# GrafikXxxxxxxYyyyyyyyyyy/StableDiffusion

Hardware: AMD Instinct MI355X
Metric: denoise-loop latents/s (512px, 50-step DDIM, batch 4) (higher is better)
Workload: dtype f16; 1 GPU; SD1.5 512x512, 50-step DDIM, batch 4/GPU, CFG on (UNet batch 8), UNet + VAE decode HIP kernels; global_batch=4, parallelism=dp1

## Files before the change

### include/sd_engine.h

```cpp
#ifndef SD_ENGINE_H
#define SD_ENGINE_H

#include <stdint.h>

#ifdef __cplusplus
extern "C" {
#endif

#define SD_OK 0
#define SD_ERR_INVALID 1
#define SD_ERR_STATE 2
#define SD_ERR_HIP 3
#define SD_ERR_UNSUPPORTED 4

#define SD_DTYPE_F16 0
#define SD_DTYPE_F32 1

#define SD_MAX_BLOCKS 4

typedef struct sd_unet_config {
    int32_t in_channels;
    int32_t out_channels;
    int32_t num_blocks;
    int32_t block_out_channels[SD_MAX_BLOCKS];
// ... 49 lines not shown
int sd_unet_destroy(sd_unet* u);
int sd_unet_num_weights(const sd_unet* u);
int sd_unet_weight_info(const sd_unet* u, int index, const char** key, int64_t* shape4, int* ndim);
int sd_unet_set_weight(sd_unet* u, const char* diffusers_key, const void* data,
                       const int64_t* shape, int ndim, int dtype);
int sd_unet_finalize(sd_unet* u);
int sd_unet_forward(sd_unet* u, const void* sample, const float* timesteps, const void* ehs,
                    int ehs_len, const void* add_text, const float* add_time_ids, void* out,
                    int B, int H, int W, void* stream);
int sd_unet_use_graph(sd_unet* u, int enable);
int sd_unet_text_kv_cache(sd_unet* u, int enable);
int sd_unet_forward_ex(sd_unet* u, const void* sample, const float* timesteps, const void* ehs, int ehs_len,
                       const void* add_text, const float* add_time_ids, const void* image_embeds, int n_img, void* out,
                       int B, int H, int W, void* stream);
int sd_unet_forward_tc(sd_unet* u, const void* sample, const float* timesteps, const void* ehs, int ehs_len,
                       const void* add_text, const float* add_time_ids, const void* image_embeds, int n_img,
                       const float* timestep_cond, int cond_dim, void* out, int B, int H, int W, void* stream);
int sd_unet_set_ip_adapter(sd_unet* u, sd_ip_adapter* adapter);
int sd_unet_set_ip_adapter_scale(sd_unet* u, float scale);
int sd_unet_set_controlnet(sd_unet* u, sd_controlnet* cn);
int sd_unet_forward_cn(sd_unet* u, const void* sample, const float* timesteps, const void* ehs, int ehs_len,
                       const void* add_text, const float* add_time_ids, const void* image_embeds, int n_img,
                       const void* control_image, int n_ctrl, float cond_scale, void* out, int B, int H, int W,
                       void* stream);
int sd_unet_forward_cfg(sd_unet* u, const void* latents, const float* timesteps, const void* ehs, int ehs_len,
                        const void* add_text, const float* add_time_ids, const void* image_embeds, int n_img,
                        float in_scale, int share, void* out, int B, int H, int W, void* stream);
int sd_unet_cfg_share(const sd_unet_config* cfg);
int sd_unet_set_freeu(sd_unet* u, int enable, float s1, float s2, float b1, float b2);
int sd_unet_memory(const sd_unet* u, int64_t* weight_bytes, int64_t* workspace_bytes);

int sd_ip_adapter_create(const sd_unet* u, int image_embed_dim, int num_tokens, sd_ip_adapter** out);
int sd_ip_adapter_destroy(sd_ip_adapter* a);
int sd_ip_adapter_num_weights(const sd_ip_adapter* a);
int sd_ip_adapter_weight_info(const sd_ip_adapter* a, int index, const char** key, int64_t* shape4, int* ndim);
int sd_ip_adapter_set_weight(sd_ip_adapter* a, const char* key, const void* data, const int64_t* shape, int ndim,
                             int dtype);
int sd_ip_adapter_finalize(sd_ip_adapter* a);

int sd_controlnet_create(const sd_unet* u, const sd_unet_config* cn_cfg, int conditioning_channels, sd_controlnet** out);
int sd_controlnet_destroy(sd_controlnet* cn);
int sd_controlnet_num_weights(const sd_controlnet* cn);
int sd_controlnet_weight_info(const sd_controlnet* cn, int index, const char** key, int64_t* shape4, int* ndim);
int sd_controlnet_set_weight(sd_controlnet* cn, const char* key, const void* data, const int64_t* shape, int ndim,
                             int dtype);
int sd_controlnet_finalize(sd_controlnet* cn);

int sd_vae_create(const sd_vae_config* cfg, sd_vae** out);
int sd_vae_destroy(sd_vae* v);
int sd_vae_num_weights(const sd_vae* v);
int sd_vae_weight_info(const sd_vae* v, int index, const char** key, int64_t* shape4, int* ndim);
int sd_vae_set_weight(sd_vae* v, const char* diffusers_key, const void* data,
                      const int64_t* shape, int ndim, int dtype);
int sd_vae_finalize(sd_vae* v);
int sd_vae_decode(sd_vae* v, const void* z, void* img, int B, int h, int w, void* stream);
int sd_vae_encode(sd_vae* v, const void* img, void* moments, int B, int H, int W, void* stream);
int sd_vae_encode_range_shift(sd_vae* v, int shift);
int sd_vae_memory(const sd_vae* v, int64_t* weight_bytes, int64_t* workspace_bytes);

int sd_clip_create(const sd_clip_config* cfg, sd_clip** out);
int sd_clip_destroy(sd_clip* c);
int sd_clip_num_weights(const sd_clip* c);
int sd_clip_weight_info(const sd_clip* c, int index, const char** key, int64_t* shape4, int* ndim);
int sd_clip_set_weight(sd_clip* c, const char* key, const void* data, const int64_t* shape, int ndim, int dtype);
int sd_clip_finalize(sd_clip* c);
int sd_clip_forward(sd_clip* c, const int32_t* input_ids, const int32_t* eos_index, void* hidden_states,
                    void* last_hidden, void* pooled, void* text_embeds, int B, int T, void* stream);
int sd_clip_final_layer_norm(sd_clip* c, const void* x, void* y, int64_t rows, void* stream);
int sd_clip_memory(const sd_clip* c, int64_t* weight_bytes, int64_t* workspace_bytes);

int sd_cfg_duplicate(const void* latents, void* out2b, int64_t n_per_batch, int B, float in_scale,
                     void* stream);
int sd_cfg_ddim_step(const void* noise_pred_2b, void* latents, int64_t n, float guidance_scale,
                     float c_x, float c_eps, void* stream);

int sd_cfg_linear_step(const void* noise_pred_2b, void* latents, float* hist_f32, int64_t n,
                       float guidance_scale, float c_x, float c_eps, float c_hist, float h_x, float h_eps,
                       void* stream);

int sd_cfg_rescale_linear_step(const void* noise_pred_2b, void* latents, float* hist_f32, int B, int64_t n_per_sample,
                               float guidance_scale, float guidance_rescale, float c_x, float c_eps, float c_hist,
                               float h_x, float h_eps, float* factors_out, void* stream);

int sd_lcm_step(const void* model_out, int rows, void* latents, const void* noise, void* denoised, int64_t n,
                float guidance_scale, float d_x, float d_out, float p_den, float p_noise, void* stream);

#define SD_STEP_MAX_SLOTS 4
#define SD_STEP_MAX_WRITES 2
typedef struct sd_step_plan {
    int32_t n_slots;
    int32_t n_writes;
    int32_t write_slot[SD_STEP_MAX_WRITES];
    double out[3+SD_STEP_MAX_SLOTS];
    double write[SD_STEP_MAX_WRITES][3+SD_STEP_MAX_SLOTS];
} sd_step_plan;
int sd_sched_affine_step(const void* model_out, int rows, void* latents, const void* noise, float* bank,
                         int64_t bank_stride, int64_t n, float guidance_scale, const sd_step_plan* plan, void* stream);

int sd_inpaint_blend(void* latents, const void* image_latents, const void* noise, const void* mask,
                     float a, float b, int B, int C, int H, int W, void* stream);

int sd_images_to_uint8(const void* images_nchw_f16, void* out_nhwc_u8, int B, int C, int H, int W, void* stream);

typedef struct sd_prof_entry {
    char kernel[64];
    double flops;
    double bytes;
    double ms;
    int64_t launches;
} sd_prof_entry;
int sd_prof_enable(int on);
int sd_prof_collect(sd_prof_entry* out, int max_entries, int* n_entries);

int sd_probe_mfma(int iters, float* tflops, void* stream);
int sd_probe_copy(int64_t bytes, int iters, float* gbs, void* stream);
int sd_probe_lds_dma(int64_t region_bytes, int passes, int depth, int shared, float* gbs, void* stream);

int sd_igemm_force(int variant, int splits);
int sd_igemm_plan(const int* geom, const int* flags, int64_t* out, char* name);

int sd_op_conv2d(const void* x_nhwc, const void* w_oihw, const void* bias, const void* rowadd,
                 const void* res_nhwc, void* y_nhwc, int N, int H, int W, int Cin, int Cout,
                 int ksize, int stride, int upsample2x, int geglu, void* stream);
int sd_op_conv2d_ex(const void* x_nhwc, const void* w_oihw, const void* bias, const void* rowadd,
                    const void* res_nhwc, void* y_nhwc, int N, int H, int W, int Cin, int Cout, int ksize,
                    int stride, int upsample2x, int geglu, int64_t ldx, int64_t ldres, int64_t ldy, int pad, int act,
                    float acc_scale, float bias_scale, int gn_groups, int* ran, void* stream);
int sd_op_conv3x3_small_cout(const void* x_nhwc, const void* w_oihw, const void* bias, void* y_nchw, int N, int H,
                             int W, int Cin, int Cout, void* stream);
int sd_op_conv2d_groupnorm(const void* x_nhwc, const void* w_oihw, const void* bias, const void* rowadd,
                           const void* res_nhwc, void* y_conv_nhwc, const void* gamma, const void* beta,
                           void* y_gn_nhwc, int N, int H, int W, int Cin, int Cout, int ksize, int stride,
                           int upsample2x, int groups, float eps, int silu, int* stats_from_epilogue, void* stream);
int sd_op_groupnorm_conv2d(const void* x_nhwc, const void* gamma, const void* beta, int groups, float eps, int silu,
                           const void* w_oihw, const void* bias, const void* rowadd, const void* res_nhwc, void* y_nhwc,
                           int N, int H, int W, int Cin, int Cout, int ksize, int iters, float* ms_per_launch, int* fused,
                           void* stream);
int sd_op_unet_conv_in(const void* x_nchw, const void* w_oihw, const void* bias, void* y_nhwc, float* gn_summaries, int groups,
                       int N, int Cin, int H, int W, int Cout, int iters, float* ms_per_launch, void* stream);
int sd_op_unet_conv_out(const void* x_nhwc, const void* gamma, const void* beta, int groups, float eps, int silu,
                        const void* w_oihw, const void* bias, void* y_nchw, int N, int H, int W, int C, int Cout, int iters,
                        float* ms_per_launch, void* stream);
int sd_op_ffn_geglu(const void* x, const void* ln_gamma, const void* ln_beta, float ln_eps, const void* w1, const void* b1,
                    const void* w2, const void* b2, void* y, int M, int C, int iters, float* ms_per_launch, int* fused,
                    void* stream);
int sd_op_linear_rowstats(const void* x, const void* w0, const void* b0, const void* res, void* y1, float* stat, int M,
                          int K, int C, int* parts, int* part_w, int* producer, void* stream);
int sd_op_ln_linear(const void* y1, const float* stat, int parts, int part_w, const void* gamma, const void* beta, float eps,
                    const void* w1, const void* b1, void* y2, int M, int C, int O, int geglu, int rows_scaled, float row_scale,
                    int* consumer, void* stream);
int sd_op_ln_ffn_geglu(const void* x, const float* stat, int parts, int part_w, const void* ln_gamma, const void* ln_beta,
                       float ln_eps, const void* w1, const void* b1, const void* w2, const void* b2, void* y, int M, int C,
                       int* fused, void* stream);
int sd_bench_conv2d(const void* x_nhwc, const void* w_oihw, void* y_nhwc, int N, int H, int W, int Cin,
                    int Cout, int ksize, int stride, int upsample2x, int geglu, int iters,
                    float* ms_per_launch, void* stream);
int sd_op_groupnorm(const void* x_nhwc, const void* gamma, const void* beta, void* y_nhwc,
                    int N, int HW, int C, int groups, float eps, int silu, void* stream);
int sd_op_groupnorm_concat(const void* x_nhwc, int Ca, int Cb, const void* gamma, const void* beta, void* y_nhwc, int N, int HW,
                           int groups, float eps, int silu, void* stream);
int sd_bench_groupnorm(const void* x_nhwc, const void* gamma, const void* beta, void* y_nhwc,
                       int N, int HW, int C, int groups, float eps, int silu, int iters,
                       float* ms_per_launch, void* stream);
int sd_op_timestep_sinusoid(const float* t, float* out, int count, int dim, int flip_sin_to_cos, float freq_shift,
                            void* stream);
int sd_op_timestep_cond_embedding(const float* t, const float* cond, const void* w_f16, float* out, int B, int dim,
                                  int cond_dim, int flip_sin_to_cos, float freq_shift, void* stream);
int sd_op_small_linear(const float* x, const void* w_f16, const float* bias, float* y, int B, int K, int n_out,
                       int silu_in, int silu_out, void* stream);
int sd_op_freeu(void* cat_nhwc, int N, int H, int W, int C1, int C2, float b, float s, void* stream);
int sd_op_layernorm(const void* x, const void* gamma, const void* beta, void* y, int rows, int C,
                    float eps, void* stream);
int sd_op_attention(const void* q, const void* k, const void* v, void* out, int B, int Tq, int Tk,
                    int heads, int d, int ldq, int ldk, int ldv, int ldo, void* stream);
int sd_op_attention_ex(const void* q, const void* k, const void* v, void* out, int B, int Tq, int Tk,
                       int heads, int d, int ldq, int ldk, int ldv, int ldo, int causal, int prescaled,
                       void* stream);
int sd_attention_plan(int B, int Tq, int Tk, int heads, int d, int causal, int prescaled, int* out5);
int sd_op_ip_cross_attention(const void* q, const void* k, const void* v, const void* k_ip, const void* v_ip, void* out,
                             int B, int Tq, int L, int T_ip, int heads, int d, int ldq, int ldk, int ldv, int ldk_ip,
                             int ldv_ip, int ldo, float ip_scale, int prescaled, int iters, float* ms_per_launch,
                             void* stream);

typedef struct sd_cn_problem {
    const void* x; int64_t ldx;
    const void* w;
    const float* bias;
    void* y; int64_t ldy;
    int M, C;
} sd_cn_problem;
int sd_op_controlnet_residuals(const sd_cn_problem* problems, int count, float scale, int mode, int iters,
                               float* ms_per_launch, void* stream);
int sd_op_controlnet_cond_embed(sd_controlnet* cn, const void* image, int n, int H, int W, void* out, int iters,
                                float* ms_per_launch, void* stream);

#ifdef __cplusplus
}
#endif
#endif
```

### stablediffusion_amd/_lib.py

```python
from __future__ import annotations

import ctypes as C
import os

_HERE = os.path.dirname(os.path.abspath(__file__))
LIB_PATH = os.path.join(_HERE, "libsd_engine.so")

SD_MAX_BLOCKS = 4
SD_STEP_MAX_SLOTS = 4
SD_STEP_MAX_WRITES = 2
SD_DTYPE_F16 = 0
SD_DTYPE_F32 = 1


class SdUNetConfig(C.Structure):
    _fields_ = [
        ("in_channels", C.c_int32),
        ("out_channels", C.c_int32),
        ("num_blocks", C.c_int32),
        ("block_out_channels", C.c_int32 * SD_MAX_BLOCKS),
        ("down_block_has_attn", C.c_int32 * SD_MAX_BLOCKS),
        ("up_block_has_attn", C.c_int32 * SD_MAX_BLOCKS),
        ("num_heads", C.c_int32 * SD_MAX_BLOCKS),
        ("transformer_layers", C.c_int32 * SD_MAX_BLOCKS),
# ... 1 lines not shown
        ("cross_attention_dim", C.c_int32),
        ("use_linear_projection", C.c_int32),
        ("norm_num_groups", C.c_int32),
        ("norm_eps", C.c_float),
        ("flip_sin_to_cos", C.c_int32),
        ("freq_shift", C.c_float),
        ("addition_time_embed_dim", C.c_int32),
        ("projection_class_embeddings_input_dim", C.c_int32),
        ("time_cond_proj_dim", C.c_int32),
    ]


class SdVAEConfig(C.Structure):
    _fields_ = [
        ("in_channels", C.c_int32),
        ("out_channels", C.c_int32),
        ("latent_channels", C.c_int32),
        ("num_blocks", C.c_int32),
        ("block_out_channels", C.c_int32 * SD_MAX_BLOCKS),
        ("layers_per_block", C.c_int32),
        ("norm_num_groups", C.c_int32),
    ]


class SdClipConfig(C.Structure):
    _fields_ = [
        ("vocab_size", C.c_int32),
        ("hidden_size", C.c_int32),
        ("intermediate_size", C.c_int32),
        ("num_layers", C.c_int32),
        ("num_heads", C.c_int32),
        ("max_positions", C.c_int32),
        ("hidden_act", C.c_int32),
        ("projection_dim", C.c_int32),
        ("layer_norm_eps", C.c_float),
    ]


class SdProfEntry(C.Structure):
    _fields_ = [("kernel", C.c_char * 64), ("flops", C.c_double), ("bytes", C.c_double),
                ("ms", C.c_double), ("launches", C.c_int64)]


class SdCnProblem(C.Structure):
    _fields_ = [("x", C.c_void_p), ("ldx", C.c_int64), ("w", C.c_void_p), ("bias", C.c_void_p),
                ("y", C.c_void_p), ("ldy", C.c_int64), ("M", C.c_int), ("C", C.c_int)]


class SdStepPlan(C.Structure):
    _fields_ = [("n_slots", C.c_int32), ("n_writes", C.c_int32), ("write_slot", C.c_int32 * SD_STEP_MAX_WRITES),
                ("out", C.c_double * (3 + SD_STEP_MAX_SLOTS)),
                ("write", C.c_double * (3 + SD_STEP_MAX_SLOTS) * SD_STEP_MAX_WRITES)]


def step_plan(plan) -> SdStepPlan:
    if len(plan.writes) > SD_STEP_MAX_WRITES or plan.n_slots > SD_STEP_MAX_SLOTS:
        raise ValueError(f"an affine step has at most {SD_STEP_MAX_WRITES} writes and {SD_STEP_MAX_SLOTS} slots")
    p = SdStepPlan(n_slots=plan.n_slots, n_writes=len(plan.writes))
    p.out[:] = plan.out
    for j, (slot, row) in enumerate(plan.writes):
        p.write_slot[j] = slot
        p.write[j][:] = row
    return p


_P = C.c_void_p
_I = C.c_int
_I64 = C.c_int64
_F = C.c_float
SIGNATURES = {
    "sd_last_error": (C.c_char_p, []),
    "sd_engine_version": (_I, []),
    "sd_engine_arch": (C.c_char_p, []),
    "sd_unet_create": (_I, [C.POINTER(SdUNetConfig), C.POINTER(_P)]),
    "sd_unet_destroy": (_I, [_P]),
    "sd_unet_num_weights": (_I, [_P]),
    "sd_unet_weight_info": (_I, [_P, _I, C.POINTER(C.c_char_p), C.POINTER(_I64), C.POINTER(_I)]),
    "sd_unet_set_weight": (_I, [_P, C.c_char_p, _P, C.POINTER(_I64), _I, _I]),
    "sd_unet_finalize": (_I, [_P]),
    "sd_unet_forward": (_I, [_P, _P, _P, _P, _I, _P, _P, _P, _I, _I, _I, _P]),
    "sd_unet_use_graph": (_I, [_P, _I]),
    "sd_unet_text_kv_cache": (_I, [_P, _I]),
    "sd_unet_memory": (_I, [_P, C.POINTER(_I64), C.POINTER(_I64)]),
    "sd_unet_forward_ex": (_I, [_P, _P, _P, _P, _I, _P, _P, _P, _I, _P, _I, _I, _I, _P]),
    "sd_unet_forward_tc": (_I, [_P, _P, _P, _P, _I, _P, _P, _P, _I, _P, _I, _P, _I, _I, _I, _P]),
    "sd_unet_forward_cfg": (_I, [_P, _P, _P, _P, _I, _P, _P, _P, _I, _F, _I, _P, _I, _I, _I, _P]),
    "sd_unet_cfg_share": (_I, [C.POINTER(SdUNetConfig)]),
    "sd_unet_set_ip_adapter": (_I, [_P, _P]),
    "sd_unet_set_ip_adapter_scale": (_I, [_P, _F]),
    "sd_unet_set_freeu": (_I, [_P, _I, _F, _F, _F, _F]),
    "sd_ip_adapter_create": (_I, [_P, _I, _I, C.POINTER(_P)]),
    "sd_ip_adapter_destroy": (_I, [_P]),
    "sd_ip_adapter_num_weights": (_I, [_P]),
    "sd_ip_adapter_weight_info": (_I, [_P, _I, C.POINTER(C.c_char_p), C.POINTER(_I64), C.POINTER(_I)]),
    "sd_ip_adapter_set_weight": (_I, [_P, C.c_char_p, _P, C.POINTER(_I64), _I, _I]),
    "sd_ip_adapter_finalize": (_I, [_P]),
    "sd_unet_set_controlnet": (_I, [_P, _P]),
    "sd_unet_forward_cn": (_I, [_P, _P, _P, _P, _I, _P, _P, _P, _I, _P, _I, _F, _P, _I, _I, _I, _P]),
    "sd_controlnet_create": (_I, [_P, C.POINTER(SdUNetConfig), _I, C.POINTER(_P)]),
    "sd_controlnet_destroy": (_I, [_P]),
    "sd_controlnet_num_weights": (_I, [_P]),
    "sd_controlnet_weight_info": (_I, [_P, _I, C.POINTER(C.c_char_p), C.POINTER(_I64), C.POINTER(_I)]),
    "sd_controlnet_set_weight": (_I, [_P, C.c_char_p, _P, C.POINTER(_I64), _I, _I]),
    "sd_controlnet_finalize": (_I, [_P]),
    "sd_vae_create": (_I, [C.POINTER(SdVAEConfig), C.POINTER(_P)]),
    "sd_vae_destroy": (_I, [_P]),
    "sd_vae_num_weights": (_I, [_P]),
    "sd_vae_weight_info": (_I, [_P, _I, C.POINTER(C.c_char_p), C.POINTER(_I64), C.POINTER(_I)]),
    "sd_vae_set_weight": (_I, [_P, C.c_char_p, _P, C.POINTER(_I64), _I, _I]),
    "sd_vae_finalize": (_I, [_P]),
    "sd_vae_decode": (_I, [_P, _P, _P, _I, _I, _I, _P]),
    "sd_vae_encode": (_I, [_P, _P, _P, _I, _I, _I, _P]),
    "sd_vae_encode_range_shift": (_I, [_P, _I]),
    "sd_vae_memory": (_I, [_P, C.POINTER(_I64), C.POINTER(_I64)]),
    "sd_clip_create": (_I, [C.POINTER(SdClipConfig), C.POINTER(_P)]),
    "sd_clip_destroy": (_I, [_P]),
    "sd_clip_num_weights": (_I, [_P]),
    "sd_clip_weight_info": (_I, [_P, _I, C.POINTER(C.c_char_p), C.POINTER(_I64), C.POINTER(_I)]),
    "sd_clip_set_weight": (_I, [_P, C.c_char_p, _P, C.POINTER(_I64), _I, _I]),
    "sd_clip_finalize": (_I, [_P]),
    "sd_clip_forward": (_I, [_P, _P, _P, _P, _P, _P, _P, _I, _I, _P]),
    "sd_clip_final_layer_norm": (_I, [_P, _P, _P, _I64, _P]),
    "sd_clip_memory": (_I, [_P, C.POINTER(_I64), C.POINTER(_I64)]),
    "sd_op_attention_ex": (_I, [_P, _P, _P, _P, _I, _I, _I, _I, _I, _I, _I, _I, _I, _I, _I, _P]),
    "sd_cfg_duplicate": (_I, [_P, _P, _I64, _I, _F, _P]),
    "sd_cfg_ddim_step": (_I, [_P, _P, _I64, _F, _F, _F, _P]),
    "sd_inpaint_blend": (_I, [_P, _P, _P, _P, _F, _F, _I, _I, _I, _I, _P]),
    "sd_images_to_uint8": (_I, [_P, _P, _I, _I, _I, _I, _P]),
    "sd_cfg_linear_step": (_I, [_P, _P, _P, _I64, _F, _F, _F, _F, _F, _F, _P]),
    "sd_cfg_rescale_linear_step": (_I, [_P, _P, _P, _I, _I64, _F, _F, _F, _F, _F, _F, _F, _P, _P]),
    "sd_lcm_step": (_I, [_P, _I, _P, _P, _P, _I64, _F, _F, _F, _F, _F, _P]),
    "sd_sched_affine_step": (_I, [_P, _I, _P, _P, _P, _I64, _I64, _F, C.POINTER(SdStepPlan), _P]),
    "sd_igemm_force": (_I, [_I, _I]),
    "sd_igemm_plan": (_I, [C.POINTER(_I), C.POINTER(_I), C.POINTER(_I64), C.c_char_p]),
    "sd_probe_mfma": (_I, [_I, C.POINTER(_F), _P]),
    "sd_probe_lds_dma": (_I, [_I64, _I, _I, _I, C.POINTER(_F), _P]),
    "sd_probe_copy": (_I, [_I64, _I, C.POINTER(_F), _P]),
    "sd_prof_enable": (_I, [_I]),
    "sd_prof_collect": (_I, [C.POINTER(SdProfEntry), _I, C.POINTER(_I)]),
    "sd_op_conv2d": (_I, [_P, _P, _P, _P, _P, _P, _I, _I, _I, _I, _I, _I, _I, _I, _I, _P]),
    "sd_op_conv2d_ex": (_I, [_P, _P, _P, _P, _P, _P, _I, _I, _I, _I, _I, _I, _I, _I, _I, _I64, _I64, _I64, _I, _I, _F, _F, _I,
                             C.POINTER(_I), _P]),
    "sd_op_conv3x3_small_cout": (_I, [_P, _P, _P, _P, _I, _I, _I, _I, _I, _P]),
    "sd_op_conv2d_groupnorm": (_I, [_P, _P, _P, _P, _P, _P, _P, _P, _P, _I, _I, _I, _I, _I, _I, _I, _I, _I, _F, _I,
                                    C.POINTER(_I), _P]),
    "sd_op_groupnorm_conv2d": (_I, [_P, _P, _P, _I, _F, _I, _P, _P, _P, _P, _P, _I, _I, _I, _I, _I, _I, _I, C.POINTER(_F),
                                    C.POINTER(_I), _P]),
    "sd_op_unet_conv_in": (_I, [_P, _P, _P, _P, _P, _I, _I, _I, _I, _I, _I, _I, C.POINTER(_F), _P]),
    "sd_op_unet_conv_out": (_I, [_P, _P, _P, _I, _F, _I, _P, _P, _P, _I, _I, _I, _I, _I, _I, C.POINTER(_F), _P]),
    "sd_op_ffn_geglu": (_I, [_P, _P, _P, _F, _P, _P, _P, _P, _P, _I, _I, _I, C.POINTER(_F), C.POINTER(_I), _P]),
    "sd_op_linear_rowstats": (_I, [_P, _P, _P, _P, _P, _P, _I, _I, _I, C.POINTER(_I), C.POINTER(_I), C.POINTER(_I), _P]),
    "sd_op_ln_linear": (_I, [_P, _P, _I, _I, _P, _P, _F, _P, _P, _P, _I, _I, _I, _I, _I, _F, C.POINTER(_I), _P]),
    "sd_op_ln_ffn_geglu": (_I, [_P, _P, _I, _I, _P, _P, _F, _P, _P, _P, _P, _P, _I, _I, C.POINTER(_I), _P]),
    "sd_bench_conv2d": (_I, [_P, _P, _P, _I, _I, _I, _I, _I, _I, _I, _I, _I, _I, C.POINTER(_F), _P]),
    "sd_op_groupnorm": (_I, [_P, _P, _P, _P, _I, _I, _I, _I, _F, _I, _P]),
    "sd_op_groupnorm_concat": (_I, [_P, _I, _I, _P, _P, _P, _I, _I, _I, _F, _I, _P]),
    "sd_bench_groupnorm": (_I, [_P, _P, _P, _P, _I, _I, _I, _I, _F, _I, _I, C.POINTER(_F), _P]),
    "sd_op_timestep_sinusoid": (_I, [_P, _P, _I, _I, _I, _F, _P]),
    "sd_op_timestep_cond_embedding": (_I, [_P, _P, _P, _P, _I, _I, _I, _I, _F, _P]),
    "sd_op_small_linear": (_I, [_P, _P, _P, _P, _I, _I, _I, _I, _I, _P]),
    "sd_op_freeu": (_I, [_P, _I, _I, _I, _I, _I, _F, _F, _P]),
    "sd_op_layernorm": (_I, [_P, _P, _P, _P, _I, _I, _F, _P]),
    "sd_op_attention": (_I, [_P, _P, _P, _P, _I, _I, _I, _I, _I, _I, _I, _I, _I, _P]),
    "sd_attention_plan": (_I, [_I, _I, _I, _I, _I, _I, _I, C.POINTER(_I)]),
    "sd_op_ip_cross_attention": (_I, [_P, _P, _P, _P, _P, _P, _I, _I, _I, _I, _I, _I, _I, _I, _I, _I, _I, _I, _F, _I, _I,
                                      C.POINTER(_F), _P]),
    "sd_op_controlnet_residuals": (_I, [C.POINTER(SdCnProblem), _I, _F, _I, _I, C.POINTER(_F), _P]),
    "sd_op_controlnet_cond_embed": (_I, [_P, _P, _I, _I, _I, _P, _I, C.POINTER(_F), _P]),
}

_lib = None


class EngineError(RuntimeError):
    pass


def load():
    global _lib
    if _lib is not None:
        return _lib
    if not os.path.exists(LIB_PATH):
        raise EngineError(
            f"{LIB_PATH} not found: build it with `python -m stablediffusion_amd.build` "
            "(hipcc --offload-arch=gfx950). The HIP engine is mandatory; there is no CPU fallback.")
    import torch
    lib = C.CDLL(LIB_PATH)
    for name, (res, args) in SIGNATURES.items():
        fn = getattr(lib, name)
        fn.restype = res
        fn.argtypes = args
    _lib = lib
    return lib


def check(rc: int, what: str = ""):
    if rc != 0:
        msg = load().sd_last_error()
        raise EngineError(f"{what}: error {rc}: {msg.decode() if msg else '?'}")


def require_gpu():
    import torch
    if not torch.cuda.is_available():
        raise EngineError("no HIP device visible: the gfx950 engine cannot run (and nothing else will run in its place)")
```

### stablediffusion_amd/csrc/capi.cpp

```cpp
#include <cmath>
#include <cstdio>
#include <new>

#include "model.h"
#include <cstdlib>

using namespace sd;

struct sd_unet { UNet impl; explicit sd_unet(const sd_unet_config& c) : impl(c) {} };
struct sd_vae { VAE impl; explicit sd_vae(const sd_vae_config& c) : impl(c) {} };
struct sd_clip { CLIP impl; explicit sd_clip(const sd_clip_config& c) : impl(c) {} };
struct sd_controlnet {
    ControlNet impl;
    sd_controlnet(const sd_unet_config& c, int cc) : impl(c, cc) {}
};
struct sd_ip_adapter {
    IPAdapter impl;
    sd_ip_adapter(const sd_unet_config& c, int d, int n) : impl(c, d, n) {}
    ~sd_ip_adapter() { if (impl.attached) impl.attached->set_ip_adapter(nullptr); }
};

namespace {

int weight_info(const WeightStore& ws, int index, const char** key, int64_t* shape4, int* ndim) {
// ... 1227 lines not shown
    auto fused = [&]() {
        return launch_ip_attention(qh, kh, vh, kih, vih, oh, B, Tq, L, T_ip, heads, d, ldq, ldk, ldv, ldk_ip, ldv_ip, ldo,
                                   ip_scale, prescaled, s);
    };
    int rc = fused();
    if (rc || iters <= 0) return rc;
    if (!ms_per_launch) { set_error("sd_op_ip_cross_attention: ms_per_launch required with iters > 0"); return SD_ERR_INVALID; }
    if (!attention_supported(d)) { set_error("sd_op_ip_cross_attention: timing needs a head dim of the text kernel"); return SD_ERR_UNSUPPORTED; }
    half_t* tmp = nullptr;
    SD_HIP_CHECK(hipMalloc(reinterpret_cast<void**>(&tmp), (size_t)B * Tq * heads * d * sizeof(half_t)));
    const long ldt = (long)heads * d;
    auto text = [&]() {
        return launch_attention(qh, kh, vh, oh, B, Tq, L, heads, d, ldq, ldk, ldv, ldo, s, 0, prescaled);
    };
    auto unfused = [&]() {
        int r = text();
        if (!r) r = launch_attention(qh, kih, vih, tmp, B, Tq, T_ip, heads, d, ldq, ldk_ip, ldv_ip, ldt, s, 0, prescaled);
        if (!r) r = launch_axpy_f16(oh, ldo, tmp, ldt, (long)B * Tq, heads * d, ip_scale, s);
        return r;
    };
    hipEvent_t e0 = nullptr, e1 = nullptr;
    if (hipEventCreate(&e0) != hipSuccess || hipEventCreate(&e1) != hipSuccess) rc = SD_ERR_HIP;
    for (int variant = 0; variant < 3 && !rc; ++variant) {
        auto one = [&]() { return variant == 0 ? fused() : variant == 1 ? text() : unfused(); };
        for (int it = 0; it < 2 && !rc; ++it) rc = one();
        if (rc) break;
        (void)hipEventRecord(e0, s);
        for (int it = 0; it < iters && !rc; ++it) rc = one();
        (void)hipEventRecord(e1, s);
        float ms = 0.f;
        hipError_t e = hipEventSynchronize(e1);
        if (e == hipSuccess) e = hipEventElapsedTime(&ms, e0, e1);
        if (e != hipSuccess) { set_error(hipGetErrorString(e)); rc = SD_ERR_HIP; }
        ms_per_launch[variant] = ms / (float)iters;
    }
    if (!rc) rc = fused();
    if (!rc && hipStreamSynchronize(s) != hipSuccess) rc = SD_ERR_HIP;
    if (e0) (void)hipEventDestroy(e0);
    if (e1) (void)hipEventDestroy(e1);
    (void)hipFree(tmp);
    return rc;
}

}

namespace {
template <class F>
int run_op_on_arena(hipStream_t s, int iters, float* ms, F body) {
    Arena arena;
    Ctx dry{&arena, s, true};
    arena.begin(true);
    body(dry);
    if (dry.err) return dry.err;
    if (int rc = arena.reserve(arena.peak() > 0 ? arena.peak() : 256)) return rc;
    auto live = [&]() {
        Ctx c{&arena, s, false};
        arena.begin(false);
        body(c);
        return c.err;
    };
    int rc = live();
    if (!rc && iters > 0) {
        if (!ms) { set_error("ms_per_launch required with iters > 0"); return SD_ERR_INVALID; }
        hipEvent_t e0 = nullptr, e1 = nullptr;
        if (hipEventCreate(&e0) != hipSuccess || hipEventCreate(&e1) != hipSuccess) rc = SD_ERR_HIP;
        if (!rc) rc = live();
        if (!rc) (void)hipEventRecord(e0, s);
        for (int it = 0; it < iters && !rc; ++it) rc = live();
        if (!rc) {
            (void)hipEventRecord(e1, s);
            float t = 0.f;
            hipError_t e = hipEventSynchronize(e1);
            if (e == hipSuccess) e = hipEventElapsedTime(&t, e0, e1);
            if (e != hipSuccess) { set_error(hipGetErrorString(e)); rc = SD_ERR_HIP; }
            *ms = t / (float)iters;
        }
        if (e0) (void)hipEventDestroy(e0);
        if (e1) (void)hipEventDestroy(e1);
    }
    const hipError_t e = hipStreamSynchronize(s);
    if (!rc && e != hipSuccess) { set_error(hipGetErrorString(e)); rc = SD_ERR_HIP; }
    return rc;
}
}

extern "C" {

int sd_op_controlnet_residuals(const sd_cn_problem* problems, int count, float scale, int mode, int iters,
                               float* ms_per_launch, void* stream) {
    if (!problems || count < 1 || count > kCnMaxProblems) { set_error("sd_op_controlnet_residuals: 1..16 problems"); return SD_ERR_INVALID; }
    if (mode != 0 && mode != 1) { set_error("sd_op_controlnet_residuals: mode must be 0 (grouped) or 1 (unfused)"); return SD_ERR_INVALID; }
    hipStream_t s = static_cast<hipStream_t>(stream);
    CnResParams rp;
    rp.scale = scale;
    for (int i = 0; i < count; ++i) {
        const sd_cn_problem& q = problems[i];
        CnResProblem& d = rp.p[rp.count++];
        d.x = static_cast<const half_t*>(q.x); d.ldx = q.ldx; d.w = static_cast<const half_t*>(q.w); d.bias = q.bias;
        d.y = static_cast<half_t*>(q.y); d.ldy = q.ldy; d.M = q.M; d.C = q.C; d.first = rp.total;
        if (q.C <= 0 || q.C % 64 != 0 || q.M <= 0) { set_error("sd_op_controlnet_residuals: C % 64 == 0 and M >= 1 required"); return SD_ERR_UNSUPPORTED; }
        rp.total += cn_residual_tiles(q.M, q.C);
    }
    if (!cn_residual_supported(rp)) { set_error("sd_op_controlnet_residuals: unsupported strides or alignment"); return SD_ERR_UNSUPPORTED; }
    if (mode == 0) return run_op_on_arena(s, iters, ms_per_launch, [&](Ctx& c) { if (!c.dry) c.err = launch_cn_residual(rp, s); });
    std::vector<ConvW> ws((size_t)count);
    std::vector<void*> owned;
    int rc = 0;
    for (int i = 0; i < count && !rc; ++i) {
        const sd_cn_problem& q = problems[i];
        const long rows = ((long)q.C + kWeightRowPad - 1) / kWeightRowPad * kWeightRowPad;
        void *w = nullptr, *b = nullptr;
        if (hipMalloc(&w, (size_t)rows * q.C * sizeof(half_t)) != hipSuccess || hipMalloc(&b, (size_t)rows * sizeof(float)) != hipSuccess) {
            set_error("sd_op_controlnet_residuals: out of device memory"); rc = SD_ERR_HIP;
        }
        if (w) owned.push_back(w);
        if (b) owned.push_back(b);
        if (rc) break;
        if (hipMemsetAsync(w, 0, (size_t)rows * q.C * sizeof(half_t), s) != hipSuccess ||
            hipMemsetAsync(b, 0, (size_t)rows * sizeof(float), s) != hipSuccess ||
            hipMemcpyAsync(w, q.w, (size_t)q.C * q.C * sizeof(half_t), hipMemcpyDeviceToDevice, s) != hipSuccess ||
            hipMemcpyAsync(b, q.bias, (size_t)q.C * sizeof(float), hipMemcpyDeviceToDevice, s) != hipSuccess) {
            set_error("sd_op_controlnet_residuals: copy failed"); rc = SD_ERR_HIP;
        }
        ConvW& cw = ws[(size_t)i];
        cw.w = static_cast<half_t*>(w); cw.bias = static_cast<float*>(b); cw.cin = q.C; cw.cout = q.C; cw.ks = 1; cw.K = q.C;
    }
    if (!rc && scale != 0.f)
        rc = run_op_on_arena(s, iters, ms_per_launch, [&](Ctx& c) {
            for (int i = 0; i < count; ++i) {
                const sd_cn_problem& q = problems[i];
                View y(static_cast<half_t*>(q.y), q.ldy, q.C);
                ConvFuse f;
                f.acc_scale = scale; f.bias_scale = scale;
                op_conv(c, ws[(size_t)i], View(const_cast<half_t*>(static_cast<const half_t*>(q.x)), q.ldx, q.C), 1, q.M, 1,
                        y, 1, 0, nullptr, 0, &y, 0, -1, 0, &f);
            }
        });
    (void)hipStreamSynchronize(s);
    for (void* p : owned) (void)hipFree(p);
    return rc;
}

int sd_op_controlnet_cond_embed(sd_controlnet* cn, const void* image, int n, int H, int W, void* out, int iters,
                                float* ms_per_launch, void* stream) {
    if (!cn || !image || !out) { set_error("null argument"); return SD_ERR_INVALID; }
    if (!cn->impl.finalized) { set_error("sd_op_controlnet_cond_embed: ControlNet not finalized"); return SD_ERR_STATE; }
    if (n < 1 || H < 1 || W < 1) { set_error("sd_op_controlnet_cond_embed: bad shape"); return SD_ERR_INVALID; }
    const int C0 = cn->impl.cfg.block_out_channels[0];
    return run_op_on_arena(static_cast<hipStream_t>(stream), iters, ms_per_launch, [&](Ctx& c) {
        cn->impl.run_cond_embed(c, static_cast<const half_t*>(image), n, H, W, View(static_cast<half_t*>(out), C0, C0));
    });
}

}
```

### stablediffusion_amd/csrc/engine.h

```cpp
#pragma once
#include <map>
#include <string>
#include <unordered_map>
#include <vector>

#include "kernels.h"

namespace sd {

struct View {
    half_t* p = nullptr;
    long ld = 0;
    int C = 0;
    View() {}
    View(half_t* p_, long ld_, int C_) : p(p_), ld(ld_), C(C_) {}
    View slice(int c0, int c) const { return View(p + c0, ld, c); }
};

class Arena {
  public:
    ~Arena();
    int reserve(size_t bytes);
    void begin(bool dry) { dry_ = dry; off_ = 0; if (dry) peak_ = 0; }
    void* alloc(size_t bytes);
    half_t* alloc_h(long n) { return static_cast<half_t*>(alloc((size_t)n * sizeof(half_t))); }
    float* alloc_f(long n) { return static_cast<float*>(alloc((size_t)n * sizeof(float))); }
    size_t mark() const { return off_; }
    void release(size_t m) { off_ = m; }
    size_t peak() const { return peak_; }
    size_t capacity() const { return cap_; }
    bool dry() const { return dry_; }
    bool overflow() const { return overflow_; }

  private:
    char* base_ = nullptr;
    size_t cap_ = 0, off_ = 0, peak_ = 0;
    bool dry_ = false, overflow_ = false;
};

struct ConvW {
    half_t* w = nullptr;
    float* bias = nullptr;
    int cin = 0, cout = 0, ks = 1;
    long K = 0;
    float* wsum = nullptr;
};
struct RowStat {
    float* p = nullptr;
    int parts = 0;
    int width = 0;
};
struct GnStatBuf {
    float* buf = nullptr;
    GnStats st;
};
struct ConvFuse {
    const RowStat* ln_in = nullptr;
    float ln_eps = 0.f;
    RowStat* stat_out = nullptr;
    GnStatBuf* gn_out = nullptr;
    int gn_groups = 0;
    const struct NormW* gn_in = nullptr;
    GnStats gn_in_stats;
    int gn_in_groups = 0;
    float gn_in_eps = 0.f;
    int gn_in_silu = 0;
    float acc_scale = 1.f, bias_scale = 1.f;
};
struct NormW {
    float* gamma = nullptr;
    float* beta = nullptr;
    float* gb = nullptr;
    int C = 0;
};

struct RawTensor {
    std::vector<int64_t> shape;
    half_t* dev = nullptr;
    long numel = 0;
};

class WeightStore {
  public:
    ~WeightStore();
    void declare(const std::string& key, std::vector<int64_t> shape);
    int set(const std::string& key, const void* data, const int64_t* shape, int ndim, int dtype);
    bool complete(std::string* missing) const;
    const RawTensor* raw(const std::string& key) const;
    int pack_conv(const std::string& prefix, ConvW* out, bool has_bias = true);
    int pack_rows(const std::vector<std::string>& weight_keys, const std::vector<std::string>& bias_keys,
                  ConvW* out);
    int pack_geglu(const std::string& prefix, ConvW* out);
    int pack_norm(const std::string& prefix, NormW* out);
    int fold_ln(ConvW* w, const NormW& ln, int rows_scaled, float row_scale);
    void free_raw();
    void* dmalloc(size_t bytes);
    int64_t packed_bytes() const { return packed_bytes_; }

    std::vector<std::string> order;
    std::unordered_map<std::string, RawTensor> tensors;

  private:
    int host_floats(const std::string& key, std::vector<float>* out) const;
    std::vector<void*> owned_;
    int64_t packed_bytes_ = 0;
};

struct Ctx {
    Arena* arena;
    hipStream_t stream;
    bool dry;
    int err = 0;
    static constexpr int kGnPool = 4;
    GnStatBuf gnpool[kGnPool];
    int gn_next = 0;
    int gn_groups = 0;
    View ip_kv;
    int ip_T = 0;
    float ip_scale = 1.f;
};
void ctx_gnpool_init(Ctx& c, int N, long HW_max, int G);
GnStatBuf* ctx_gnbuf(Ctx& c);

struct ProfAgg { double flops = 0, bytes = 0, ms = 0; long launches = 0; };
void prof_enable(bool on);
bool prof_enabled();
void prof_open(hipStream_t s, const char* kernel, double flops, double bytes);
void prof_close(hipStream_t s);
int prof_collect(std::map<std::string, ProfAgg>* out);

void op_conv(Ctx& c, const ConvW& w, View x, int N, int H, int W, View y, int stride = 1, int up = 0,
             const float* rowadd = nullptr, int rowadd_ld = 0, const View* res = nullptr, int geglu = 0,
             int pad = -1, int act = 0, const ConvFuse* fuse = nullptr);
inline long rowstat_floats(long M, int C) { return M * ((C + 63) / 64) * 2; }
inline long gnstat_floats(int N, long HW, int G) { const long t = (HW + 63) / 64; return (long)N * (t > 64 ? t : 64) * G * 2; }
void op_groupnorm(Ctx& c, const NormW& n, View x, View y, int N, long HW, int G, float eps, int silu,
                  const GnStatBuf* pre = nullptr);
void op_gn_conv(Ctx& c, const NormW& n, const ConvW& w, View x, int N, int H, int W, View y, int G, float eps, int silu,
                const GnStatBuf* pre, const float* rowadd = nullptr, int rowadd_ld = 0, const View* res = nullptr,
                const ConvFuse* fuse = nullptr);
void op_layernorm(Ctx& c, const NormW& n, View x, View y, long rows, float eps);
bool op_ffn_fused(Ctx& c, const ConvW& ff1, const ConvW& ff2, View x, const RowStat& x_stat, float ln_eps, long M, View y);
void op_attention(Ctx& c, View q, View k, View v, View out, int B, int Tq, int Tk, int heads, int d, int causal = 0,
                  int prescaled = 0);
void op_ip_attention(Ctx& c, View q, View k, View v, View k_ip, View v_ip, View out, int B, int Tq, int L, int T_ip,
                     int heads, int d, float ip_scale);

}
```

### stablediffusion_amd/csrc/ffn.hip

```cpp
#include <cstdlib>

#include "kernels.h"

namespace sd {
namespace {

constexpr int FF_C = 320, FF_BM = 128, FF_NKS = FF_C / 64, FF_NOS = 2, FF_STAGES = 7;
constexpr int kFfMaxLnParts = 20;

template <int N>
__device__ __forceinline__ void ff_wait_vmcnt() {
    asm volatile("s_waitcnt vmcnt(%0)" ::"n"(N) : "memory");
}

struct FfLds {
    static constexpr int STAGE = 160 * 64 * 2;
    static constexpr int RING = FF_STAGES * STAGE;
    static constexpr int H = FF_BM * 64 * 2;
    static constexpr int AUX = 2 * 256 * 4;
    static constexpr int STAT = FF_BM * 2 * 4;
    static constexpr int TOTAL = RING + H + AUX + STAT;
};

__global__ __launch_bounds__(512) void ffn_fused_kernel(FfnParams p) {
// ... 38 lines not shown
    __amdgpu_buffer_rsrc_t rw2 = __builtin_amdgcn_make_buffer_rsrc(const_cast<half_t*>(p.w2), 0, (int)((long)p.w2_rows * p.hidden * 2), 0x00020000);
    __amdgpu_buffer_rsrc_t raux = __builtin_amdgcn_make_buffer_rsrc(const_cast<float*>(wave == 0 ? p.b1 : p.wsum1), 0, p.w1_rows * 4, 0x00020000);
    const int lrow = lane >> 3;
    const int chunk = (lane & 7) ^ (lrow & 7);
    auto gperm = [](int r) { return r < 32 || r >= 96 ? r : (r < 64 ? r + 32 : r - 32); };
    unsigned w1_off[2], w2_off[3];
#pragma unroll
    for (int j = 0; j < 2; ++j) {
        const int r = (wave * 2 + j) * 8 + lrow;
        w1_off[j] = (unsigned)((((long)gperm(r)) * C + chunk * 8) * 2);
    }
#pragma unroll
    for (int j = 0; j < 3; ++j) {
        const int r = (wave + NW * j) * 8 + lrow;
        const int oc = 160 * (r / 80) + (r % 80);
        w2_off[j] = (unsigned)((((long)oc) * p.hidden + chunk * 8) * 2);
    }

    int s_it = 0, s_q = 0, s_slot = 0;
    auto issue = [&]() {
        half_t* dst = ring + s_slot * STAGE_HALVES;
        const bool live = s_it < NSTEP;
        if (s_q < NKS) {
            if (s_q == 0 && wave < 2 && live && lane < 32)
                __builtin_amdgcn_raw_ptr_buffer_load_lds(raux, (__attribute__((address_space(3))) void*)(sAux + (s_it & 1) * 256 + wave * 128),
                                                         16, (unsigned)((s_it * 128 + lane * 4) * 4), 0, 0, 0);
#pragma unroll
            for (int j = 0; j < 2; ++j)
                __builtin_amdgcn_raw_ptr_buffer_load_lds(rw1, (__attribute__((address_space(3))) void*)(dst + (wave * 2 + j) * 512), 16,
                                                         live ? w1_off[j] + (unsigned)((s_it * 128 * C + s_q * 64) * 2) : kOOB, 0, 0, 0);
        } else {
            const unsigned sb = (unsigned)((((long)(s_q - NKS) * 80) * p.hidden + s_it * 64) * 2);
#pragma unroll
            for (int j = 0; j < 3; ++j)
                if (wave + NW * j < 20)
                    __builtin_amdgcn_raw_ptr_buffer_load_lds(rw2, (__attribute__((address_space(3))) void*)(dst + (wave + NW * j) * 512), 16,
                                                             live ? w2_off[j] + sb : kOOB, 0, 0, 0);
        }
        if (++s_q == NKS + NOS) { s_q = 0; ++s_it; }
        if (++s_slot == STAGES) s_slot = 0;
    };
#pragma unroll
    for (int s = 0; s < LA; ++s) issue();

    f4 acc1[TM][4], acc2[NOS][TM][5];
#pragma unroll
    for (int i = 0; i < TM; ++i) {
#pragma unroll
        for (int j = 0; j < 4; ++j) acc1[i][j] = f4{0.f, 0.f, 0.f, 0.f};
#pragma unroll
        for (int s = 0; s < NOS; ++s)
#pragma unroll
            for (int j = 0; j < 5; ++j) acc2[s][i][j] = f4{0.f, 0.f, 0.f, 0.f};
    }

    int lb[2];
#pragma unroll
    for (int ks = 0; ks < 2; ++ks) lb[ks] = fr * 64 + (((ks * 4 + fq) ^ (fr & 7)) << 3);
    const int rowH = wm * 32 * 64, rowB1 = wn * 64 * 64, rowB2 = wn * 80 * 64;
    int c_slot = 0;
    auto slab_begin = [&]() -> const half_t* {
        ff_wait_vmcnt<2 * (LA - 1)>();
        asm volatile("s_waitcnt lgkmcnt(0)" ::: "memory");
        __builtin_amdgcn_s_barrier();
        issue();
        const half_t* cB = ring + c_slot * STAGE_HALVES;
        if (++c_slot == STAGES) c_slot = 0;
        return cB;
    };

    for (int it = 0; it < NSTEP; ++it) {
        {
#pragma unroll
            for (int q = 0; q < NKS; ++q) {
                const half_t* cB = slab_begin();
#pragma unroll
                for (int ks = 0; ks < 2; ++ks) {
                    h8 fb[4];
#pragma unroll
                    for (int j = 0; j < 4; ++j) fb[j] = *reinterpret_cast<const h8*>(cB + rowB1 + j * 1024 + lb[ks]);
#pragma unroll
                    for (int i = 0; i < TM; ++i)
#pragma unroll
                        for (int j = 0; j < 4; ++j)
                            acc1[i][j] = __builtin_amdgcn_mfma_f32_16x16x32_f16(fb[j], xf[i][q * 2 + ks], acc1[i][j], 0, 0, 0);
                }
            }
            const float* ax = sAux + (it & 1) * 256 + wn * 32 + fq * 4;
#pragma unroll
            for (int jh = 0; jh < 2; ++jh) {
                const f4 bh = *reinterpret_cast<const f4*>(ax + jh * 16), bg = *reinterpret_cast<const f4*>(ax + 64 + jh * 16);
                const f4 wh = *reinterpret_cast<const f4*>(ax + 128 + jh * 16), wg = *reinterpret_cast<const f4*>(ax + 192 + jh * 16);
#pragma unroll
                for (int i = 0; i < TM; ++i) {
                    const float2 mr = *reinterpret_cast<const float2*>(sStat + (wm * 32 + i * 16 + fr) * 2);
                    const f4 hv = (acc1[i][jh] - mr.x * wh) * mr.y + bh;
                    const f4 gv = (acc1[i][jh + 2] - mr.x * wg) * mr.y + bg;
                    h4 o;
#pragma unroll
                    for (int e = 0; e < 4; ++e) o[e] = (half_t)(hv[e] * gelu_erf_f(gv[e]));
                    const int pr = wm * 32 + i * 16 + fr;
                    const int k = wn * 32 + jh * 16 + fq * 4;
                    *reinterpret_cast<h4*>(sH + pr * 64 + (((k >> 3) ^ (pr & 7)) << 3) + (k & 7)) = o;
                    acc1[i][jh] = f4{0.f, 0.f, 0.f, 0.f};
                    acc1[i][jh + 2] = f4{0.f, 0.f, 0.f, 0.f};
                }
            }
        }
        {
#pragma unroll
            for (int s = 0; s < NOS; ++s) {
                const half_t* cB = slab_begin();
#pragma unroll
                for (int ks = 0; ks < 2; ++ks) {
                    h8 fa[TM], fb[5];
#pragma unroll
                    for (int i = 0; i < TM; ++i) fa[i] = *reinterpret_cast<const h8*>(sH + rowH + i * 1024 + lb[ks]);
#pragma unroll
                    for (int j = 0; j < 5; ++j) fb[j] = *reinterpret_cast<const h8*>(cB + rowB2 + j * 1024 + lb[ks]);
#pragma unroll
                    for (int i = 0; i < TM; ++i)
#pragma unroll
                        for (int j = 0; j < 5; ++j)
                            acc2[s][i][j] = __builtin_amdgcn_mfma_f32_16x16x32_f16(fb[j], fa[i], acc2[s][i][j], 0, 0, 0);
                }
            }
        }
    }
    ff_wait_vmcnt<0>();

#pragma unroll
    for (int s = 0; s < NOS; ++s) {
#pragma unroll
        for (int j = 0; j < 5; ++j) {
            const int col = 160 * wn + 80 * s + j * 16 + fq * 4;
            const f4 b2 = *reinterpret_cast<const f4*>(p.b2 + col);
#pragma unroll
            for (int i = 0; i < TM; ++i) {
                const long m = m0 + wm * 32 + i * 16 + fr;
                const f4 v = acc2[s][i][j] + b2;
                const h4 xr = *reinterpret_cast<const h4*>(p.x + m * p.ldx + col);
                h4 o;
#pragma unroll
                for (int e = 0; e < 4; ++e) o[e] = (half_t)((float)(half_t)v[e] + (float)xr[e]);
                *reinterpret_cast<h4*>(p.y + m * p.ldy + col) = o;
            }
        }
    }
#endif
}

}

bool ffn_fused_supported(const FfnParams& p) {
    static const bool off = getenv("SD_NO_FFN_FUSE") != nullptr;
    return !off && p.C == FF_C && p.hidden == 4 * FF_C && p.M % FF_BM == 0 && p.M / FF_BM >= 64 && p.ln_stat && p.ln_parts >= 1 &&
           p.ln_parts <= kFfMaxLnParts && p.w1_rows >= 2 * p.hidden && p.w2_rows >= FF_C &&
           (long)p.M * p.ldx * 2 < (1L << 31) && p.b1 && p.b2 && p.wsum1;
}

int launch_ffn_fused(const FfnParams& p, hipStream_t s) {
    if (!ffn_fused_supported(p)) { set_error("ffn_fused: unsupported problem"); return 1; }
    static_assert(FfLds::TOTAL <= 160 * 1024, "LDS budget");
    static PerDeviceOnce attr_once;
    if (attr_once.first()) {
        SD_HIP_CHECK(hipFuncSetAttribute(reinterpret_cast<const void*>(&ffn_fused_kernel),
                                         hipFuncAttributeMaxDynamicSharedMemorySize, FfLds::TOTAL));
    }
    hipLaunchKernelGGL(ffn_fused_kernel, dim3(p.M / FF_BM), dim3(512), FfLds::TOTAL, s, p);
    SD_HIP_CHECK(hipGetLastError());
    return 0;
}

}
```

### stablediffusion_amd/csrc/igemm2.hip

```cpp
#include <atomic>
#include <cstdlib>
#include <mutex>

#include "kernels.h"

namespace sd {
namespace {

constexpr int BK = 64;
constexpr int kMaxLnParts = 20;
template <int N>
__device__ __forceinline__ void wait_vmcnt() {
    static_assert(N >= 0 && N <= 63, "vmcnt is a 6-bit field");
    asm volatile("s_waitcnt vmcnt(%0)" ::"n"(N) : "memory");
}
template <int PER, int YMAX>
__device__ __forceinline__ void wait_stages(int y) {
    if constexpr (YMAX == 0) {
        wait_vmcnt<0>();
    } else {
        if (y >= YMAX) wait_vmcnt<PER * YMAX>();
        else wait_stages<PER, YMAX - 1>(y);
    }
}
// ... 924 lines not shown
    }
    if constexpr (GN) {
        if (p.gnstat_out) {
            float* sG = reinterpret_cast<float*>(smem + ((BM * LDC * 2 + 15) & ~15));
            gn_part_finish(gsplit, gnv, gp0, gp1, gm0, gq0, gm1, gq1);
            gn_tile_stats<BM, BN, NT>(sG, tid, gm0, gq0, gm1, gq1, n0, p.Cout, cpg, p.gn_groups,
                                      p.gnstat_out + ((long)img * patches + pidx) * p.gn_groups * 2);
        }
    }
#endif
}

bool halo_supported(const IGemmParams& p) {
    return p.KS == 3 && p.stride == 1 && (p.up == 0 || p.up == 1) && p.pad == 1 && !p.geglu && !p.act && p.Cin % 64 == 0 &&
           p.Cout % 8 == 0 && halo_patch_width(p.OH, p.OW) > 0 && p.OH == p.H << p.up && p.OW == p.W << p.up &&
           p.K == 9 * p.Cin;
}

template <int BN, bool GNF, bool KHU>
int launch_halo_t(const IGemmParams& p, float* partial, int splits, hipStream_t s) {
    const int Wt = halo_patch_width(p.OH, p.OW), R = 256 / Wt;
    size_t lds = (size_t)2 * (R + 2) * (Wt + 2) * 128 + (size_t)3 * BN * 128 + (GNF ? 768 : 0);
    const size_t epi = (size_t)256 * (BN + 8) * 2 + 16 + 512 * 16;
    if (lds < epi) lds = epi;
    if (lds > 160 * 1024) { set_error("conv3x3_halo_kernel: LDS budget"); return 1; }
    static size_t attr_by_dev[64] = {};
    static std::mutex attr_mu;
    int dev = 0;
    (void)hipGetDevice(&dev);
    std::lock_guard<std::mutex> attr_lock(attr_mu);
    size_t& attr = attr_by_dev[dev & 63];
    if (lds > attr) {
        SD_HIP_CHECK(hipFuncSetAttribute(reinterpret_cast<const void*>(&conv3x3_halo_kernel<BN, GNF, KHU>),
                                         hipFuncAttributeMaxDynamicSharedMemorySize, (int)lds));
        attr = lds;
    }
    const int tiles = (p.M / 256) * cdiv(p.Cout, BN);
    const int nslab = p.Cin / 64;
    const int per = cdiv(nslab, splits);
    const int eff_splits = cdiv(nslab, per);
    note_splits(eff_splits);
    IGemmParams q = p;
    q.mfast = weights_outweigh_activations(p);
    if (eff_splits > 1) q.gnstat_out = nullptr;
    hipLaunchKernelGGL((conv3x3_halo_kernel<BN, GNF, KHU>), dim3(tiles, eff_splits), dim3(512), lds, s, q, eff_splits > 1 ? partial : nullptr,
                       per);
    SD_HIP_CHECK(hipGetLastError());
    if (eff_splits > 1) return launch_splitk_epilogue(p, partial, eff_splits, s);
    return 0;
}

template <int BN>
int launch_halo(const IGemmParams& p, float* partial, int splits, hipStream_t s) {
    if (p.gni_part) {
        if (p.gni_groups < 1 || p.gni_groups > 32 || 512 % p.gni_groups != 0 || p.Cin % p.gni_groups != 0 || !p.gni_gb) {
            set_error("conv3x3_halo_kernel: fused GroupNorm needs 1..32 groups dividing 512 and the packed affine");
            return 1;
        }
        return launch_halo_t<BN, true, false>(p, partial, splits, s);
    }
    if constexpr (BN == 160) {
        if (p.gnstat_out && splits <= 1) return launch_halo_t<BN, false, false>(p, partial, splits, s);
    }
    return launch_halo_t<BN, false, true>(p, partial, splits, s);
}

template <int BM, int BN, int WM, int WN, int STAGES, bool PW, bool STAG, int BKT>
int launch_v2p(const IGemmParams& p, float* partial, int splits, hipStream_t s) {
    constexpr size_t lds = IGemm2Lds<BM, BN, STAGES, BKT>::TOTAL;
    static_assert(lds <= 160 * 1024, "LDS budget");
    static PerDeviceOnce attr_once;
    if (attr_once.first()) {
        SD_HIP_CHECK(hipFuncSetAttribute(reinterpret_cast<const void*>(&igemm2_kernel<BM, BN, WM, WN, STAGES, PW, STAG, BKT>),
                                         hipFuncAttributeMaxDynamicSharedMemorySize, (int)lds));
    }
    const int tiles = cdiv(p.M, BM) * cdiv(p.Cout, BN);
    const int nk = p.K / BKT;
    const int per = cdiv(nk, splits);
    const int eff_splits = cdiv(nk, per);
    note_splits(eff_splits);
    IGemmParams q = p;
    q.mfast = weights_outweigh_activations(p);
    q.rowstat_parts = cdiv(p.Cout, BN);
    if (p.geglu && !(BN == 128 && WN == 2)) { set_error("igemm2: GEGLU needs a 128-column tile over two wave columns"); return 1; }
    if (eff_splits > 1 && (p.rowstat_out || p.ln_stat)) { set_error("igemm2: row statistics / LayerNorm fold need splits == 1"); return 1; }
    hipLaunchKernelGGL((igemm2_kernel<BM, BN, WM, WN, STAGES, PW, STAG, BKT>), dim3(tiles, eff_splits), dim3(64 * WM * WN), lds, s,
                       q, eff_splits > 1 ? partial : nullptr, per);
    SD_HIP_CHECK(hipGetLastError());
    if (eff_splits > 1) return launch_splitk_epilogue(p, partial, eff_splits, s);
    return 0;
}

template <int BM, int BN, int WM, int WN, int STAGES, bool STAG = false, int BKT = 64>
int launch_v2(const IGemmParams& p, float* partial, int splits, hipStream_t s) {
    if (p.KS == 1 && p.stride == 1 && p.up == 0)
        return launch_v2p<BM, BN, WM, WN, STAGES, true, STAG, BKT>(p, partial, splits, s);
    return launch_v2p<BM, BN, WM, WN, STAGES, false, STAG, BKT>(p, partial, splits, s);
}

std::atomic<int> g_force_variant{-1};
std::atomic<int> g_force_splits{0};

enum class Family { Tile, Halo, Ws, Reg };
struct Variant {
    int id, bm, bn;
    Family family;
    bool geglu;
    bool reg_alt;
    const char* name;
    int (*launch)(const IGemmParams&, float* partial, int splits, hipStream_t);
};
int launch_ws(const IGemmParams& p, float*, int, hipStream_t s) { return launch_wsgemm(p, s); }
int launch_reg(const IGemmParams& p, float*, int, hipStream_t s) { return launch_igemm3(p, weights_outweigh_activations(p), s); }
const Variant kVariants[] = {
    {0, 256, 128, Family::Tile, true, false, "igemm2_kernel<256,128,4,2,3,%s,false,64>", &launch_v2<256, 128, 4, 2, 3>},
    {1, 128, 128, Family::Tile, true, false, "igemm2_kernel<128,128,2,2,2,%s,false,64>", &launch_v2<128, 128, 2, 2, 2>},
    {2, 128, 160, Family::Tile, false, false, "igemm2_kernel<128,160,2,2,2,%s,false,64>", &launch_v2<128, 160, 2, 2, 2>},
    {3, 128, 64, Family::Tile, false, false, "igemm2_kernel<128,64,2,2,2,%s,false,64>", &launch_v2<128, 64, 2, 2, 2>},
    {4, 64, 64, Family::Tile, false, false, "igemm2_kernel<64,64,2,2,2,%s,false,64>", &launch_v2<64, 64, 2, 2, 2>},
    {5, 256, 160, Family::Tile, false, false, "igemm2_kernel<256,160,4,1,3,%s,false,64>", &launch_v2<256, 160, 4, 1, 3>},
    {6, 256, 128, Family::Tile, true, false, "igemm2_kernel<256,128,4,2,3,%s,true,64>", &launch_v2<256, 128, 4, 2, 3, true>},
    {7, 256, 160, Family::Tile, false, false, "igemm2_kernel<256,160,4,2,3,%s,true,64>", &launch_v2<256, 160, 4, 2, 3, true>},
    {8, 128, 64, Family::Tile, false, false, "igemm2_kernel<128,64,2,2,3,%s,false,64>", &launch_v2<128, 64, 2, 2, 3>},
    {9, 128, 160, Family::Tile, false, false, "igemm2_kernel<128,160,2,2,3,%s,false,64>", &launch_v2<128, 160, 2, 2, 3>},
    {10, 256, 160, Family::Halo, false, false, "conv3x3_halo_kernel<160>", &launch_halo<160>},
    {11, 128, 80, Family::Tile, false, true, "igemm2_kernel<128,80,4,1,2,%s,false,64>", &launch_v2<128, 80, 4, 1, 2>},
    {12, 128, 80, Family::Tile, false, true, "igemm2_kernel<128,80,4,1,3,%s,false,64>", &launch_v2<128, 80, 4, 1, 3>},
    {13, 128, 160, Family::Ws, true, false, "wsgemm_kernel<160,false,...>", &launch_ws},
    {14, 128, 128, Family::Ws, true, false, "wsgemm_kernel<128,true,...>", &launch_ws},
    {15, 256, 128, Family::Halo, false, false, "conv3x3_halo_kernel<128>", &launch_halo<128>},
    {16, 128, 80, Family::Tile, false, false, "igemm2_kernel<128,80,4,1,4,%s,false,64>", &launch_v2<128, 80, 4, 1, 4>},
    {17, 128, 80, Family::Tile, false, false, "igemm2_kernel<128,80,4,1,5,%s,false,64>", &launch_v2<128, 80, 4, 1, 5>},
    {18, 128, 80, Family::Reg, false, false, "igemm3_kernel", &launch_reg},
};
constexpr int kNumVariants = sizeof(kVariants) / sizeof(kVariants[0]);
enum : int {
    kT256x128 = 0, kT128x128 = 1, kT128x160 = 2, kT128x64 = 3, kT64x64 = 4,
    kHalo160 = 10, kHalo128 = 15,
    kWsPlain = 13, kWsGeglu = 14,
    kHaloFallback = 7,
    kGegluFallback = kT128x128,
    kWsFallbackGeglu = kT128x128, kWsFallbackPlain = kT128x160,
    kReg = 18, kRegFallback = 12,
};
bool valid_id(int v) { return v >= 0 && v < kNumVariants && kVariants[v].id == v; }
bool is_halo(int v) { return kVariants[v].family == Family::Halo; }
bool is_ws(int v) { return kVariants[v].family == Family::Ws; }

struct TunedEntry { int M, N, K, ks, stride, up, geglu, variant, splits; float us; int alt_variant; float alt_us; };
const TunedEntry kTuned[] = {
#include "igemm2_table.inc"
};

void pick_tile(const IGemmParams& p, int* variant, int* splits) {
    if (g_force_variant.load() >= 0) {
        int v = g_force_variant.load();
        *splits = g_force_splits.load() > 0 ? g_force_splits.load() : 1;
        if (p.geglu && !(valid_id(v) && kVariants[v].geglu)) v = kGegluFallback;
        if (p.geglu || p.act) *splits = 1;
        if (valid_id(v) && is_halo(v) && !halo_supported(p)) v = kHaloFallback;
        *variant = v;
        return;
    }
    for (const TunedEntry& e : kTuned)
        if (!p.act && e.M == p.M && e.N == p.Cout && e.K == p.K && e.ks == p.KS && e.stride == p.stride && e.up == p.up &&
            e.geglu == p.geglu) {
            *variant = is_halo(e.variant) && !halo_supported(p) ? kHaloFallback : e.variant;
            *splits = e.splits;
            return;
        }
    auto tiles_of = [&](int v) { return (long)cdiv(p.M, kVariants[v].bm) * cdiv(p.Cout, kVariants[v].bn); };
    const int narrow = tiles_of(kT128x64) >= 256 ? kT128x64 : kT64x64;
    *splits = 1;
    if (p.act) {
        *variant = tiles_of(kT128x128) >= 256 ? kT128x128 : narrow;
        return;
    }
    const int nk = p.K / BK;
    int v;
    if (p.geglu) v = tiles_of(kT256x128) >= 512 ? kT256x128 : kT128x128;
    else v = p.Cout % 160 == 0 ? kT128x160 : kT128x128;
    if (!p.geglu && tiles_of(v) < 256 && nk <= 40) v = narrow;
    const long tiles = tiles_of(v);
    if (!p.geglu && tiles < 384 && nk >= 24) {
        int sp = (int)((512 + tiles / 2) / tiles);
        if (sp > 8) sp = 8;
        while (sp > 1 && nk / sp < 12) --sp;
        *splits = sp;
    }
    *variant = v;
}

}

void igemm2_force(int variant, int splits) { g_force_variant = variant; g_force_splits = splits; }

bool igemm2_supported(const IGemmParams& p) {
    const long x_bytes = (long)p.N * p.H * p.W * p.ldx * 2;
    const long wrows = ((long)p.Cout + kWeightRowPad - 1) / kWeightRowPad * kWeightRowPad;
    return p.K % BK == 0 && p.Cin % BK == 0 && (p.Cout % 8) == 0 && x_bytes < (1L << 31) &&
           wrows * p.K * 2 < (1L << 31) && (!p.geglu || p.Cout % 128 == 0) && !(p.geglu && p.act);
}

bool igemm2_gn_fusable(const IGemmParams& p, int groups) {
    return igemm2_supported(p) && halo_supported(p) && p.up == 0 && groups >= 1 && groups <= 32 && 512 % groups == 0 &&
           p.Cin % groups == 0;
}

IGemmPlan igemm2_plan(IGemmParams& p, const IGemmRequest& rq) {
    IGemmPlan pl;
    pl.rs_part_w = p.Cout;
    if (!igemm2_supported(p)) {
        snprintf(pl.name, sizeof(pl.name), "%s", igemm_variant(p));
        return pl;
    }
    static const bool ws_on = getenv("SD_NO_WSGEMM") == nullptr;
    static const bool pg_k320 = getenv("SD_PGEMM_K320") != nullptr;
    static const bool g3_auto = getenv("SD_IGEMM3") != nullptr;
    const bool forced = g_force_variant.load() >= 0;
    int v0, sp0;
    pick_tile(p, &v0, &sp0);
    if (!valid_id(v0)) { set_error("igemm2: bad variant"); pl.kind = kKindBadVariant; return pl; }
    int v, sp;
    auto route = [&]() {
        v = v0; sp = sp0;
        if (p.gni_part && !is_halo(v)) {
            v = p.Cout % 160 == 0 ? kHalo160 : kHalo128;
            const long tiles = (long)(p.M / kVariants[v].bm) * cdiv(p.Cout, kVariants[v].bn);
            const int nslab = p.Cin / 64;
            sp = 1;
            while (tiles * sp < 192 && nslab / (sp + 1) >= 4 && sp < 8) ++sp;
        }
        if (p.ln_stat) sp = 1;
        const bool ws_ok = wsgemm_supported(p);
        if (is_ws(v) && !ws_ok) { v = p.geglu ? kWsFallbackGeglu : kWsFallbackPlain; sp = 1; }
        if (!forced && ws_ok && !p.res && ws_on) { v = kWsPlain; sp = 1; }
        if (is_ws(v)) v = p.geglu ? kWsGeglu : kWsPlain;
        if (rq.no_workspace) sp = 1;
    };
    route();
    pl.scales_ok = !p.geglu && !is_ws(v);
    const int G = rq.gn_groups, cpg = G > 0 && p.Cout % G == 0 ? p.Cout / G : 0;
    if (rq.gnstat && !p.geglu && (cpg >= 8 || cpg == 4)) {
        p.gnstat_out = rq.gnstat; p.gn_groups = G;
        route();
        const Variant& t = kVariants[is_halo(v) && !halo_supported(p) ? kHaloFallback : v];
        if (is_ws(v)) pl.gn_rows = 0;
        else if (sp > 1) pl.gn_rows = splitk_gs_rows(p, G);
        else pl.gn_rows = (p.OH * p.OW) % t.bm == 0 && (t.bn % cpg == 0 || p.Cout <= t.bn) ? t.bm : 0;
        pl.gnstats = pl.gn_rows > 0;
        if (!pl.gnstats) { p.gnstat_out = nullptr; p.gn_groups = 0; }
    }
    if (rq.rowstat && !p.geglu) {
        p.rowstat_out = rq.rowstat;
        route();
        const int parts = is_ws(v) ? wsgemm_rowstat_parts(p) : cdiv(p.Cout, kVariants[v].bn);
        pl.rowstats = sp <= 1 && !is_halo(v) && parts <= kMaxLnParts;
        if (pl.rowstats) { pl.rs_parts = parts; pl.rs_part_w = is_ws(v) ? p.Cout / parts : kVariants[v].bn; }
        else p.rowstat_out = nullptr;
    }
    route();
    pl.variant = v;
    pl.splits = sp;
    pl.partial_floats = sp > 1 ? (long)sp * p.M * p.Cout : 0;
    if (p.geglu && (!is_ws(v) || pg_k320) && !forced && pgemm_geglu_supported(p)) pl.kind = kKindPgemmGeglu;
    else if ((v == kReg || (kVariants[v].reg_alt && g3_auto && !forced)) && sp <= 1 && igemm3_supported(p)) pl.kind = kReg;
    else pl.kind = v == kReg ? kRegFallback : v;
    const Variant& t = kVariants[pl.kind == kKindPgemmGeglu ? v : pl.kind];
    pl.bm = t.bm; pl.bn = t.bn;
    if (pl.kind == kKindPgemmGeglu) snprintf(pl.name, sizeof(pl.name), "geglu_persist_kernel");
    else snprintf(pl.name, sizeof(pl.name), t.name, p.KS == 1 && p.stride == 1 && p.up == 0 ? "true" : "false");
    return pl;
}

IGemmLaunchNote igemm2_last_launch() { return t_note; }

int launch_igemm2(const IGemmParams& p, float* partial, hipStream_t s, const IGemmPlan* plan) {
    t_note = IGemmLaunchNote();
    IGemmParams q = p;
    IGemmPlan own;
    if (!plan || (plan->splits > 1 && !partial)) {
        q.rowstat_out = nullptr; q.gnstat_out = nullptr;
        own = igemm2_plan(q, IGemmRequest{p.rowstat_out, p.gnstat_out, p.gn_groups, partial == nullptr});
        plan = &own;
    }
    if (plan->kind == kKindIgemm1) return launch_igemm(q, s);
    if (plan->kind == kKindPgemmGeglu) return launch_pgemm_geglu(q, s);
    if (plan->kind == kKindBadVariant) { set_error("igemm2: bad variant"); return 1; }
    return kVariants[plan->kind].launch(q, partial, plan->splits, s);
}

}
```

### stablediffusion_amd/csrc/kernels.h

```cpp
#pragma once
#include "common.h"

namespace sd {

struct IGemmParams {
    const half_t* x; long ldx;
    const half_t* w;
    const float* bias;
    const float* rowadd; int rowadd_ld;
    const half_t* res; long ldres;
    half_t* y; long ldy;
    int N, H, W, Cin;
    int OH, OW, Cout;
    int KS, stride, pad, up;
    int M, K;
    int geglu;
    int mfast = 0;
    int act = 0;
    float* rowstat_out = nullptr;
    int rowstat_parts = 0;
    const float* ln_stat = nullptr;
    int ln_parts = 0, ln_C = 0, ln_part_w = 0;
    float ln_eps = 0.f;
    const float* ln_wsum = nullptr;
    float* gnstat_out = nullptr;
    int gn_groups = 0;
    const float* gni_part = nullptr;
    int gni_S = 0;
    long gni_rows = 0;
    int gni_groups = 0;
    float gni_eps = 0.f;
    int gni_silu = 0;
    const float* gni_gb = nullptr;
    int dbg_unchecked = 0;
    float acc_scale = 1.f, bias_scale = 1.f;
};
bool igemm2_gn_fusable(const IGemmParams& p, int groups);
int launch_igemm(const IGemmParams& p, hipStream_t s);
const char* igemm_variant(const IGemmParams& p);
bool igemm2_supported(const IGemmParams& p);
void igemm2_force(int variant, int splits);
struct IGemmRequest {
    float* rowstat = nullptr;
    float* gnstat = nullptr;
    int gn_groups = 0;
    bool no_workspace = false;
};
constexpr int kKindPgemmGeglu = 100;
constexpr int kKindIgemm1 = -1;
constexpr int kKindBadVariant = -2;
struct IGemmPlan {
    int kind = kKindIgemm1;
    int variant = -1;
    int splits = 1;
    long partial_floats = 0;
    int bm = 0, bn = 0;
    bool rowstats = false;
    int rs_parts = 1, rs_part_w = 0;
    bool gnstats = false;
    int gn_rows = 0;
    bool scales_ok = false;
    char name[64] = "";
};
IGemmPlan igemm2_plan(IGemmParams& p, const IGemmRequest& rq = IGemmRequest());
int launch_igemm2(const IGemmParams& p, float* partial, hipStream_t s, const IGemmPlan* plan = nullptr);
struct IGemmLaunchNote {
    int splits = 1;
    int reducer = 0;
};
IGemmLaunchNote igemm2_last_launch();
bool igemm3_supported(const IGemmParams& p);
int launch_igemm3(const IGemmParams& p, int mfast, hipStream_t s);
constexpr int kWeightRowPad = 256;
bool wsgemm_supported(const IGemmParams& p);
int wsgemm_rowstat_parts(const IGemmParams& p);
int launch_wsgemm(const IGemmParams& p, hipStream_t s);
bool pgemm_geglu_supported(const IGemmParams& p);
int launch_pgemm_geglu(const IGemmParams& p, hipStream_t s);

struct FfnParams {
    const half_t* x; long ldx;
    half_t* y; long ldy;
    const half_t* w1; const float* b1; const float* wsum1; int w1_rows;
    const half_t* w2; const float* b2; int w2_rows;
    const float* ln_stat; int ln_parts; float ln_eps;
    int M, C, hidden;
    int ln_part_w;
};
bool ffn_fused_supported(const FfnParams& p);
int launch_ffn_fused(const FfnParams& p, hipStream_t s);

long gn_scratch_floats(int N, long HW, int C, int G);
struct GnStats {
    const float* part = nullptr;
    int S = 0;
    long rows = 0;
};
bool gn_wants_stats(long HW, int C, int G);
int launch_groupnorm(const half_t* x, long ldx, const float* gamma, const float* beta,
                     half_t* y, long ldy, int N, long HW, int C, int G, float eps, int silu,
                     float* scratch, hipStream_t s, const GnStats* pre = nullptr);
int launch_gn_stats(const half_t* x, long ldx, int N, long HW, int C, int G, float* scratch, GnStats* st, hipStream_t s);
int launch_gn_finalize(GnStats* st, float* out, int N, long HW, int C, int G, hipStream_t s);
int gn_cat_unit(int Ca, int Cb, int G);
int launch_gn_cat_finalize(const GnStats& sa, int Ga, int Ca, const GnStats& sb, int Gb, int Cb, float* out, int N, long HW, int G,
                           hipStream_t s);
int launch_layernorm(const half_t* x, long ldx, const float* gamma, const float* beta,
                     half_t* y, long ldy, long rows, int C, float eps, hipStream_t s);
int launch_row_stats(const half_t* x, long ldx, float* stat, long rows, int C, hipStream_t s);
int launch_ln_fold(half_t* w, long K, int rows, const float* gamma, const float* beta, const float* bias_in,
                   float* bias, float* wsum, int rows_scaled, float row_scale, hipStream_t s);

int launch_attention(const half_t* q, const half_t* k, const half_t* v, half_t* out,
                     int B, int Tq, int Tk, int heads, int d,
                     long ldq, long ldk, long ldv, long ldo, hipStream_t s, int causal = 0, int prescaled = 0);
bool attention_supported(int d);
struct AttnPlan { int D, QT, KT, PRESC, NWV; };
AttnPlan attention_plan(int B, int Tq, int Tk, int heads, int d, int causal, int prescaled);
int launch_ip_attention(const half_t* q, const half_t* k, const half_t* v, const half_t* kip, const half_t* vip,
                        half_t* out, int B, int Tq, int L, int Tip, int heads, int d, long ldq, long ldk, long ldv,
                        long ldki, long ldvi, long ldo, float ip_scale, int prescaled, hipStream_t s);
bool ip_attention_supported(int d);
int launch_axpy_f16(half_t* y, long ldy, const half_t* x, long ldx, long rows, int cols, float a, hipStream_t s);

constexpr int kCnMaxProblems = 16;
struct CnResProblem {
    const half_t* x = nullptr; long ldx = 0;
    const half_t* w = nullptr;
    const float* bias = nullptr;
    half_t* y = nullptr; long ldy = 0;
    int M = 0, C = 0;
    int first = 0;
};
struct CnResParams {
    CnResProblem p[kCnMaxProblems];
    int count = 0, total = 0;
    float scale = 1.f;
};
int cn_residual_tiles(int M, int C);
bool cn_residual_supported(const CnResParams& p);
int launch_cn_residual(const CnResParams& p, hipStream_t s);
struct CnCondConvParams {
    const half_t* x = nullptr; int nchw = 0;
    const float* w = nullptr; const float* bias = nullptr;
    half_t* y = nullptr;
    int N = 0, IH = 0, IW = 0, Cin = 0, OH = 0, OW = 0, Cout = 0, stride = 1, silu = 1;
};
bool cn_cond_conv_supported(const CnCondConvParams& p);
int launch_cn_cond_conv(const CnCondConvParams& p, hipStream_t s);
int launch_cn_pack_cond(const half_t* w_oihw, float* out, int O, int I, hipStream_t s);

int launch_freeu(half_t* x, long ld, int N, int H, int W, int C1, int C2, float b, float s, hipStream_t st);

int launch_timestep_sinusoid(const float* t, int t_stride, float* out, int count, int dim, int flip, float shift,
                             long out_ld, hipStream_t s);
int launch_timestep_cond(const float* t, const float* cond, const half_t* w, long ldw, float* out, int count, int dim,
                         int cond_dim, int flip, float shift, hipStream_t s);
int launch_small_linear(const float* x, long ldx, const half_t* w, const float* bias, float* y,
                        long ldy, int B, int K, int Nout, int silu_in, int silu_out, hipStream_t s);
int launch_add_f32(float* y, const float* x, long n, int silu, hipStream_t s);
int launch_f16_to_f32(const half_t* x, float* y, long n, hipStream_t s);
int launch_f32_to_f16(const float* x, half_t* y, long n, hipStream_t s);
int launch_im2col_nchw3x3(const half_t* x, half_t* col, int N, int C, int H, int W, int Kpad,
                          hipStream_t s);
int launch_nhwc_to_nchw(const half_t* x, long ldx, half_t* y, int N, long HW, int C, hipStream_t s);
int launch_nchw_to_nhwc(const half_t* x, half_t* y, long ldy, int N, long HW, int C, hipStream_t s);
int launch_pointwise_nchw(const half_t* x, const half_t* w, const float* bias, half_t* y, int N,
                          int Cin, int Cout, long HW, hipStream_t s);
constexpr long kSmallCoutMinPixels = 131072;
int launch_conv3x3_small_cout(const half_t* x, long ldx, const half_t* w, long K, const float* bias, half_t* y_nchw,
                              int N, int H, int W, int Cin, int Cout, hipStream_t s);
struct HeadParams {
    const half_t* x_nchw = nullptr;
    const half_t* w = nullptr; long K = 0;
    const float* bias = nullptr;
    half_t* y = nullptr; long ldy = 0;
    float* gnstat_out = nullptr; int G = 0;
    int N = 0, Cin = 0, H = 0, W = 0, Cout = 0;
};
bool conv_head_supported(const HeadParams& p);
int launch_conv_head(const HeadParams& p, hipStream_t s);
struct TailParams {
    const half_t* x = nullptr; long ldx = 0;
    const float* gn_part = nullptr; int gn_S = 0; long gn_rows = 0;
    int G = 0; float eps = 0.f; const float* gamma = nullptr; const float* beta = nullptr; int silu = 0;
    const half_t* w = nullptr; long K = 0; const float* bias = nullptr;
    half_t* y = nullptr;
    int N = 0, H = 0, W = 0, C = 0, Cout = 0;
};
bool conv_tail_supported(const TailParams& p);
int launch_conv_tail(const TailParams& p, hipStream_t s);
int launch_pack_conv(const half_t* w_oihw, half_t* wp, int O, int I, int KH, int KW, long Kpad,
                     hipStream_t s);
int launch_cfg_duplicate(const half_t* lat, half_t* out, long n_total, float scale, hipStream_t s);
constexpr int kRowDupMax = 8;
struct RowDupSeg {
    const void* src = nullptr;
    void* dst = nullptr;
    long ld_bytes = 0, row_bytes = 0, rows = 0;
};
int launch_row_dup(const RowDupSeg* segs, int count, hipStream_t s);
int launch_scale_copy_f16(const half_t* x, half_t* out, long n, float scale, hipStream_t s);
int launch_dup_f32(const float* x, float* out, long n, hipStream_t s);
int launch_clip_embed(const int* ids, const half_t* tok, const half_t* pos, half_t* out, int B, int T, int H, int vocab,
                      hipStream_t s);
int launch_gather_rows(const half_t* x, long ldx, const int* idx, half_t* out16, float* out32, int B, int T, int H,
                       hipStream_t s);
int launch_inpaint_blend(half_t* lat, const half_t* img, const half_t* noise, const half_t* mask, float a, float b, int B,
                         int C, long HW, hipStream_t s);
int launch_scale_f16(half_t* x, long n, float scale, hipStream_t s);
int launch_image_to_uint8(const half_t* img, unsigned char* out, int B, int C, long HW, hipStream_t s);
int launch_cfg_linear(const half_t* eps2b, half_t* lat, float* hist, long n, float g, float cx, float ce, float ch,
                      float hx, float he, hipStream_t s);
int launch_cfg_ddim(const half_t* eps2b, half_t* lat, long n, float g, float cx, float ce,
                    hipStream_t s);
int launch_lcm_step(const half_t* model_out, int rows, half_t* lat, const half_t* noise, half_t* denoised, long n, float g,
                    float dx, float dout, float pden, float pnoise, hipStream_t s);
constexpr int STEP_SLOTS = 4, STEP_WRITES = 2, STEP_COLS = 3 + STEP_SLOTS;
struct StepRows {
    double out[STEP_COLS];
    double write[STEP_WRITES][STEP_COLS];
    int n_writes;
    int write_slot[STEP_WRITES];
};
int launch_sched_affine_step(const half_t* model_out, int rows, half_t* lat, const half_t* noise, float* bank, long stride,
                             long n, float g, const StepRows& p, hipStream_t s);
int launch_cfg_rescale_linear(const half_t* eps2b, half_t* lat, float* hist, int B, long n, float g, float phi, float cx,
                              float ce, float ch, float hx, float he, float* factors, hipStream_t s);

int probe_mfma(int iters, float* tflops, hipStream_t s);
int probe_copy(long bytes, int iters, float* gbs, hipStream_t s);
int probe_dma(long region_bytes, int passes, int depth, int shared, float* gbs, hipStream_t s);

}
```

### stablediffusion_amd/csrc/misc.hip

```cpp
#include <cstdint>
#include <cstdlib>
#include <map>
#include <mutex>
#include <utility>

#include "kernels.h"

namespace sd {
namespace {

__global__ void sinusoid_kernel(const float* __restrict__ t, int t_stride, float* __restrict__ out, int count,
                                int dim, int flip, float shift, long out_ld) {
    const int half = dim >> 1;
    const int i = blockIdx.x * blockDim.x + threadIdx.x;
    if (i >= count * half) return;
    const int b = i / half, f = i - b * half;
    const float freq = __expf(-9.210340371976184f * (float)f / ((float)half - shift));
    const float ang = t[(long)b * t_stride] * freq;
    float sn, cs;
    sincosf(ang, &sn, &cs);
    float* o = out + (long)b * out_ld;
    if (flip) { o[f] = cs; o[half + f] = sn; } else { o[f] = sn; o[half + f] = cs; }
}

// ... 472 lines not shown
__global__ __launch_bounds__(256) void rs_apply_kernel(const half_t* __restrict__ eps2b, half_t* __restrict__ lat,
                                                       float* __restrict__ hist, const RsStat* __restrict__ part, int parts,
                                                       long n, long total, float g, float phi, float cx, float ce, float ch,
                                                       float hx, float he, float* __restrict__ factors) {
    const int b = blockIdx.y, lane = threadIdx.x & 63;
    RsStat st = {0.f, 0.f, 0.f}, se = {0.f, 0.f, 0.f};
    if (lane < parts) {
        const RsStat* q = part + ((long)b * parts + lane) * 2;
        st = q[0];
        se = q[1];
    }
    st = rs_wave_merge(st);
    se = rs_wave_merge(se);
    const float k = 1.f + phi * (sqrtf(st.m2 / se.m2) - 1.f);
    if (factors && blockIdx.x == 0 && threadIdx.x == 0) factors[b] = k;
    const long base = (long)b * n;
    const half_t* u = eps2b + base;
    const half_t* t = u + total;
    half_t* x = lat + base;
    float* h = hist ? hist + base : nullptr;
    if (VEC) {
        const long i = ((long)blockIdx.x * 256 + threadIdx.x) * 8;
        if (i >= n) return;
        const h8 vu = *reinterpret_cast<const h8*>(u + i);
        const h8 vt = *reinterpret_cast<const h8*>(t + i);
        const h8 vx = *reinterpret_cast<const h8*>(x + i);
        float hv[8], x0[8];
        if (h) {
            const f4 h0 = *reinterpret_cast<const f4*>(h + i), h1 = *reinterpret_cast<const f4*>(h + i + 4);
#pragma unroll
            for (int j = 0; j < 4; ++j) { hv[j] = h0[j]; hv[j + 4] = h1[j]; }
        }
        h8 o;
#pragma unroll
        for (int j = 0; j < 8; ++j) {
            const float e = k * rs_cfg((float)vu[j], (float)vt[j], g);
            const float xf = (float)vx[j];
            float out = rs_axpby(cx, xf, ce, e);
            if (h) {
                out = __builtin_fmaf(ch, hv[j], out);
                x0[j] = rs_axpby(hx, xf, he, e);
            }
            o[j] = (half_t)out;
        }
        *reinterpret_cast<h8*>(x + i) = o;
        if (h) {
            f4 h0, h1;
#pragma unroll
            for (int j = 0; j < 4; ++j) { h0[j] = x0[j]; h1[j] = x0[j + 4]; }
            *reinterpret_cast<f4*>(h + i) = h0;
            *reinterpret_cast<f4*>(h + i + 4) = h1;
        }
    } else {
        const long i = (long)blockIdx.x * 256 + threadIdx.x;
        if (i >= n) return;
        const float e = k * rs_cfg((float)u[i], (float)t[i], g);
        const float xf = (float)x[i];
        float out = rs_axpby(cx, xf, ce, e);
        if (h) {
            out = __builtin_fmaf(ch, h[i], out);
            h[i] = rs_axpby(hx, xf, he, e);
        }
        x[i] = (half_t)out;
    }
}

__global__ void image_to_uint8_kernel(const half_t* __restrict__ img, unsigned char* __restrict__ out, int C, long HW,
                                      long total_px) {
    const long i = (long)blockIdx.x * blockDim.x + threadIdx.x;
    if (i >= total_px) return;
    const long b = i / HW, px = i - b * HW;
    const half_t* src = img + b * C * HW + px;
    unsigned char* dst = out + i * C;
    for (int c = 0; c < C; ++c) {
        half_t v = src[(long)c * HW] * (half_t)0.5f;
        v = v + (half_t)0.5f;
        v = v < (half_t)0.f ? (half_t)0.f : (v > (half_t)1.f ? (half_t)1.f : v);
        v = v * (half_t)255.f;
        dst[c] = (unsigned char)(int)(float)v;
    }
}

__global__ void clip_embed_kernel(const int* __restrict__ ids, const half_t* __restrict__ tok,
                                  const half_t* __restrict__ pos, half_t* __restrict__ out, long rows, int T, int H8,
                                  int vocab) {
    const long i = (long)blockIdx.x * blockDim.x + threadIdx.x;
    if (i >= rows * H8) return;
    const long r = i / H8;
    const int c = (int)(i - r * H8) * 8;
    int id = ids[r];
    id = id < 0 ? 0 : (id >= vocab ? vocab - 1 : id);
    const int t = (int)(r % T);
    const h8 a = *reinterpret_cast<const h8*>(tok + (long)id * H8 * 8 + c);
    const h8 b = *reinterpret_cast<const h8*>(pos + (long)t * H8 * 8 + c);
    h8 o;
#pragma unroll
    for (int e = 0; e < 8; ++e) o[e] = (half_t)((float)a[e] + (float)b[e]);
    *reinterpret_cast<h8*>(out + r * H8 * 8 + c) = o;
}
__global__ void gather_rows_kernel(const half_t* __restrict__ x, long ldx, const int* __restrict__ idx,
                                   half_t* __restrict__ out16, float* __restrict__ out32, int B, int T, int H) {
    const long i = (long)blockIdx.x * blockDim.x + threadIdx.x;
    if (i >= (long)B * H) return;
    const int b = (int)(i / H), c = (int)(i - (long)b * H);
    int t = idx[b];
    t = t < 0 ? 0 : (t >= T ? T - 1 : t);
    const half_t v = x[((long)b * T + t) * ldx + c];
    if (out16) out16[i] = v;
    if (out32) out32[i] = (float)v;
}

__global__ void inpaint_blend_kernel(half_t* __restrict__ lat, const half_t* __restrict__ img,
                                     const half_t* __restrict__ noise, const half_t* __restrict__ mask, float a,
                                     float b, int C, long HW, long n) {
    const long i = (long)blockIdx.x * blockDim.x + threadIdx.x;
    if (i >= n) return;
    const long bc = i / HW, px = i - bc * HW;
    const float m = (float)mask[(bc / C) * HW + px];
    float keep = a * (float)img[i];
    if (noise) keep += b * (float)noise[i];
    lat[i] = (half_t)(m * (float)lat[i] + (1.f - m) * keep);
}

__global__ void scale_f16_kernel(half_t* __restrict__ x, long n, float scale) {
    const long i = (long)blockIdx.x * blockDim.x + threadIdx.x;
    if (i < n) x[i] = (half_t)((float)x[i] * scale);
}

__global__ __launch_bounds__(256) void ln_fold_kernel(half_t* __restrict__ w, long K, int rows,
                                                      const float* __restrict__ gamma, const float* __restrict__ beta,
                                                      const float* __restrict__ bias_in, float* __restrict__ bias,
                                                      float* __restrict__ wsum, int rows_scaled, float row_scale) {
    const int lane = threadIdx.x & 63;
    const int n = blockIdx.x * 4 + (threadIdx.x >> 6);
    if (n >= rows) return;
    const float sc = n < rows_scaled ? row_scale : 1.0f;
    half_t* row = w + (long)n * K;
    float ws = 0.f, wb = 0.f;
    for (long k = lane; k < K; k += 64) {
        const float old = (float)row[k];
        const half_t nw = (half_t)(old * gamma[k] * sc);
        row[k] = nw;
        ws += (float)nw;
        wb += old * beta[k];
    }
#pragma unroll
    for (int off = 32; off > 0; off >>= 1) { ws += __shfl_xor(ws, off); wb += __shfl_xor(wb, off); }
    if (lane == 0) {
        wsum[n] = ws;
        bias[n] = sc * ((bias_in ? bias_in[n] : 0.f) + wb);
    }
}


constexpr int CO_TH = 8, CO_TW = 64;
constexpr int CO_CS = 32;
constexpr int CO_PSTR = CO_CS + 8;
template <int COUT>
__global__ __launch_bounds__(256) void conv3x3_small_cout_kernel(const half_t* __restrict__ x, long ldx,
                                                                 const half_t* __restrict__ w, long K,
                                                                 const float* __restrict__ bias,
                                                                 half_t* __restrict__ y, int N, int H, int W, int Cin,
                                                                 int cout_real) {
    constexpr int HP = (CO_TH + 2) * (CO_TW + 2);
    __shared__ __attribute__((aligned(16))) half_t halo[HP * CO_PSTR];
    __shared__ __attribute__((aligned(16))) half_t wl[9 * (CO_CS / 8) * COUT * 8];
    const int tid = threadIdx.x;
    const int tiles_w = (W + CO_TW - 1) / CO_TW, tiles_h = (H + CO_TH - 1) / CO_TH;
    int b = blockIdx.x;
    const int tw = b % tiles_w; b /= tiles_w;
    const int th = b % tiles_h;
    const int n = b / tiles_h;
    const int oh0 = th * CO_TH, ow0 = tw * CO_TW;
    const int lr = tid / (CO_TW / 2), lc = (tid % (CO_TW / 2)) * 2;
    float acc[2][COUT];
#pragma unroll
    for (int co = 0; co < COUT; ++co) { acc[0][co] = 0.f; acc[1][co] = 0.f; }
    const half_t* xn = x + (long)n * H * W * ldx;
    for (int c0 = 0; c0 < Cin; c0 += CO_CS) {
        __syncthreads();
        for (int i = tid; i < HP * (CO_CS / 8); i += 256) {
            const int hp = i / (CO_CS / 8), ch = i % (CO_CS / 8);
            const int hr = hp / (CO_TW + 2), hc = hp - hr * (CO_TW + 2);
            const int ih = oh0 - 1 + hr, iw = ow0 - 1 + hc;
            h8 v = {0, 0, 0, 0, 0, 0, 0, 0};
            if ((unsigned)ih < (unsigned)H && (unsigned)iw < (unsigned)W)
                v = *reinterpret_cast<const h8*>(xn + ((long)ih * W + iw) * ldx + c0 + ch * 8);
            *reinterpret_cast<h8*>(halo + hp * CO_PSTR + ch * 8) = v;
        }
        for (int i = tid; i < 9 * (CO_CS / 8) * COUT; i += 256) {
            const int co = i % COUT, ch = (i / COUT) % (CO_CS / 8), tap = i / (COUT * (CO_CS / 8));
            *reinterpret_cast<h8*>(wl + i * 8) =
                *reinterpret_cast<const h8*>(w + (long)co * K + ((long)(c0 / 64) * 9 + tap) * 64 + (c0 % 64) + ch * 8);
        }
        __syncthreads();
#pragma unroll
        for (int tap = 0; tap < 9; ++tap) {
            const half_t* px = halo + ((lr + tap / 3) * (CO_TW + 2) + lc + tap % 3) * CO_PSTR;
#pragma unroll
            for (int ch = 0; ch < CO_CS / 8; ++ch) {
                const h8 x0 = *reinterpret_cast<const h8*>(px + ch * 8);
                const h8 x1 = *reinterpret_cast<const h8*>(px + CO_PSTR + ch * 8);
#pragma unroll
                for (int co = 0; co < COUT; ++co) {
                    const h8 wv = *reinterpret_cast<const h8*>(wl + ((tap * (CO_CS / 8) + ch) * COUT + co) * 8);
#pragma unroll
                    for (int e = 0; e < 4; ++e) {
                        const h2 wp = {wv[2 * e], wv[2 * e + 1]};
                        acc[0][co] = __builtin_amdgcn_fdot2(h2{x0[2 * e], x0[2 * e + 1]}, wp, acc[0][co], false);
                        acc[1][co] = __builtin_amdgcn_fdot2(h2{x1[2 * e], x1[2 * e + 1]}, wp, acc[1][co], false);
                    }
                }
            }
        }
    }
    const int oh = oh0 + lr;
#pragma unroll
    for (int p2 = 0; p2 < 2; ++p2) {
        const int ow = ow0 + lc + p2;
        if (oh < H && ow < W) {
#pragma unroll
            for (int co = 0; co < COUT; ++co)
                if (co < cout_real)
                    y[(((long)n * cout_real + co) * H + oh) * W + ow] = (half_t)(acc[p2][co] + (bias ? bias[co] : 0.f));
        }
    }
}

inline dim3 grid1d(long n, int block = 256) { return dim3((unsigned)((n + block - 1) / block)); }

}

int launch_timestep_sinusoid(const float* t, int t_stride, float* out, int count, int dim, int flip, float shift,
                             long out_ld, hipStream_t s) {
    hipLaunchKernelGGL(sinusoid_kernel, grid1d((long)count * (dim / 2)), dim3(256), 0, s, t, t_stride, out, count,
                       dim, flip, shift, out_ld);
    SD_HIP_CHECK(hipGetLastError());
    return 0;
}

int launch_timestep_cond(const float* t, const float* cond, const half_t* w, long ldw, float* out, int count, int dim,
                         int cond_dim, int flip, float shift, hipStream_t s) {
    const long waves = (long)count * (dim / 2);
    if (waves <= 0) return 0;
    const bool vec = ldw % 8 == 0 && (reinterpret_cast<uintptr_t>(w) & 15) == 0;
    const dim3 grid((unsigned)((waves + 3) / 4));
    if (vec)
        hipLaunchKernelGGL(temb_cond_kernel<true>, grid, dim3(256), 0, s, t, cond, w, ldw, out, count, dim, cond_dim, flip, shift);
    else
        hipLaunchKernelGGL(temb_cond_kernel<false>, grid, dim3(256), 0, s, t, cond, w, ldw, out, count, dim, cond_dim, flip, shift);
    SD_HIP_CHECK(hipGetLastError());
    return 0;
}

constexpr int SK_MAXKS = 10;
__global__ __launch_bounds__(256) void skinny_linear_kernel(const float* __restrict__ x, long ldx, const half_t* __restrict__ w,
                                                            const float* __restrict__ bias, float* __restrict__ y, long ldy,
                                                            int B, int K, int Nout, int silu_in, int silu_out) {
    __shared__ float red[2][4][256];
    const int tid = threadIdx.x, lane = tid & 63, wave = tid >> 6;
    const int fr = lane & 15, fq = lane >> 4;
    const int KS = K / 32;
    const int tiles = Nout / 16;
    h8 xh[SK_MAXKS], xl[SK_MAXKS];
#pragma unroll
    for (int j = 0; j < SK_MAXKS; ++j) {
        const int ks = wave + 4 * j;
        h8 hi = {0, 0, 0, 0, 0, 0, 0, 0}, lo = {0, 0, 0, 0, 0, 0, 0, 0};
        if (ks < KS && fr < B) {
            const float* xr = x + (long)fr * ldx + ks * 32 + fq * 8;
            const f4 a = *reinterpret_cast<const f4*>(xr), b = *reinterpret_cast<const f4*>(xr + 4);
#pragma unroll
            for (int e = 0; e < 8; ++e) {
                float v = e < 4 ? a[e] : b[e - 4];
                if (silu_in) v = silu_f(v);
                hi[e] = (half_t)v;
                lo[e] = (half_t)(v - (float)hi[e]);
            }
        }
        xh[j] = hi; xl[j] = lo;
    }
    auto fetch = [&](int t, h8* wf) {
        const int tt = t < tiles ? t : tiles - 1;
        const half_t* wr = w + ((long)tt * 16 + fr) * K + fq * 8;
#pragma unroll
        for (int j = 0; j < SK_MAXKS; ++j) {
            const int ks = wave + 4 * j;
            wf[j] = *reinterpret_cast<const h8*>(wr + (ks < KS ? ks : KS - 1) * 32);
        }
    };
    h8 wcur[SK_MAXKS], wnext[SK_MAXKS];
    int t = blockIdx.x;
    fetch(t, wcur);
    int par = 0;
    for (; t < tiles; t += gridDim.x, par ^= 1) {
        fetch(t + gridDim.x, wnext);
        f4 acc = {0.f, 0.f, 0.f, 0.f};
#pragma unroll
        for (int j = 0; j < SK_MAXKS; ++j) {
            if (wave + 4 * j < KS) {
                acc = __builtin_amdgcn_mfma_f32_16x16x32_f16(wcur[j], xh[j], acc, 0, 0, 0);
                acc = __builtin_amdgcn_mfma_f32_16x16x32_f16(wcur[j], xl[j], acc, 0, 0, 0);
            }
        }
#pragma unroll
        for (int e = 0; e < 4; ++e) red[par][wave][(fq * 4 + e) * 16 + fr] = acc[e];
// ... 101 lines not shown
        }
        p.src[k] = static_cast<const uint4*>(g.src);
        p.dst[k] = static_cast<uint4*>(g.dst);
        p.ld16[k] = g.ld_bytes / 16;
        p.w16[k] = g.row_bytes / 16;
        p.units[k] = g.rows * p.w16[k];
        p.first[k] = blocks;
        const long nb = (p.units[k] + RD_UNITS - 1) / RD_UNITS;
        if (nb + blocks > 0x7fffffffL) { set_error("row_dup: too large"); return 1; }
        blocks += (int)nb;
        ++k;
    }
    if (k == 0) return 0;
    p.first[k] = blocks;
    p.count = k;
    hipLaunchKernelGGL(row_dup_kernel, dim3((unsigned)blocks), dim3(256), 0, s, p);
    SD_HIP_CHECK(hipGetLastError());
    return 0;
}
int launch_scale_copy_f16(const half_t* x, half_t* out, long n, float scale, hipStream_t s) {
    if (n <= 0) return 0;
    hipLaunchKernelGGL(scale_copy_f16_kernel, grid1d(n), dim3(256), 0, s, x, out, n, scale);
    SD_HIP_CHECK(hipGetLastError());
    return 0;
}
int launch_dup_f32(const float* x, float* out, long n, hipStream_t s) {
    if (n <= 0) return 0;
    hipLaunchKernelGGL(dup_f32_kernel, grid1d(n), dim3(256), 0, s, x, out, n);
    SD_HIP_CHECK(hipGetLastError());
    return 0;
}
int launch_cfg_ddim(const half_t* eps2b, half_t* lat, long n, float g, float cx, float ce, hipStream_t s) {
    hipLaunchKernelGGL(cfg_ddim_kernel, grid1d(n), dim3(256), 0, s, eps2b, lat, n, g, cx, ce);
    SD_HIP_CHECK(hipGetLastError());
    return 0;
}
int launch_cfg_linear(const half_t* eps2b, half_t* lat, float* hist, long n, float g, float cx, float ce, float ch,
                      float hx, float he, hipStream_t s) {
    hipLaunchKernelGGL(cfg_linear_kernel, grid1d(n), dim3(256), 0, s, eps2b, lat, hist, n, g, cx, ce, ch, hx, he);
    SD_HIP_CHECK(hipGetLastError());
    return 0;
}
int launch_lcm_step(const half_t* model_out, int rows, half_t* lat, const half_t* noise, half_t* denoised, long n, float g,
                    float dx, float dout, float pden, float pnoise, hipStream_t s) {
    const bool vec = n % 8 == 0 && ((reinterpret_cast<uintptr_t>(model_out) | reinterpret_cast<uintptr_t>(lat) |
                                     reinterpret_cast<uintptr_t>(noise) | reinterpret_cast<uintptr_t>(denoised)) & 15) == 0;
    const dim3 grid = grid1d(vec ? n / 8 : n);
#define SD_LCM_LAUNCH(R, V) \
    hipLaunchKernelGGL((lcm_step_kernel<R, V>), grid, dim3(256), 0, s, model_out, lat, noise, denoised, n, g, dx, dout, pden, pnoise)
    if (rows == 2) { if (vec) SD_LCM_LAUNCH(2, true); else SD_LCM_LAUNCH(2, false); }
    else { if (vec) SD_LCM_LAUNCH(1, true); else SD_LCM_LAUNCH(1, false); }
#undef SD_LCM_LAUNCH
    SD_HIP_CHECK(hipGetLastError());
    return 0;
}
int launch_sched_affine_step(const half_t* model_out, int rows, half_t* lat, const half_t* noise, float* bank, long stride,
                             long n, float g, const StepRows& p, hipStream_t s) {
    unsigned use = 0;
    for (int k = 0; k < STEP_COLS; ++k) {
        bool any = p.out[k] != 0.0;
        for (int w = 0; w < p.n_writes; ++w) any = any || p.write[w][k] != 0.0;
        if (any) use |= 1u << k;
    }
    const bool vec = n % 8 == 0 && stride % 4 == 0 &&
                     ((reinterpret_cast<uintptr_t>(model_out) | reinterpret_cast<uintptr_t>(lat) |
                       reinterpret_cast<uintptr_t>(noise) | reinterpret_cast<uintptr_t>(bank)) & 15) == 0;
    const dim3 grid = grid1d(vec ? n / 8 : n);
#define SD_STEP_LAUNCH(R, V) \
    hipLaunchKernelGGL((sched_affine_kernel<R, V>), grid, dim3(256), 0, s, model_out, lat, noise, bank, stride, n, g, p, use)
    if (rows == 2) { if (vec) SD_STEP_LAUNCH(2, true); else SD_STEP_LAUNCH(2, false); }
    else { if (vec) SD_STEP_LAUNCH(1, true); else SD_STEP_LAUNCH(1, false); }
#undef SD_STEP_LAUNCH
    SD_HIP_CHECK(hipGetLastError());
    return 0;
}
static RsStat* rs_workspace(int B, hipStream_t s) {
    struct Buf { RsStat* p = nullptr; int B = 0; };
    static std::mutex mu;
    static std::map<std::pair<int, hipStream_t>, Buf> bufs;
    int dev = 0;
    if (hipGetDevice(&dev) != hipSuccess) return nullptr;
    std::lock_guard<std::mutex> lock(mu);
    Buf& b = bufs[{dev, s}];
    if (b.B < B) {
        if (b.p) (void)hipFree(b.p);
        b.p = nullptr;
        b.B = 0;
        if (hipMalloc(reinterpret_cast<void**>(&b.p), (size_t)B * RS_MAX_PARTS * 2 * sizeof(RsStat)) != hipSuccess) {
            b.p = nullptr;
            return nullptr;
        }
        b.B = B;
    }
    return b.p;
}
int launch_cfg_rescale_linear(const half_t* eps2b, half_t* lat, float* hist, int B, long n, float g, float phi, float cx,
                              float ce, float ch, float hx, float he, float* factors, hipStream_t s) {
    RsStat* part = rs_workspace(B, s);
    if (!part) { set_error("cfg_rescale_linear: no device memory for the chunk summaries"); return 1; }
    const long total = (long)B * n;
    const bool vec = n % 8 == 0 && ((reinterpret_cast<uintptr_t>(eps2b) | reinterpret_cast<uintptr_t>(lat) |
                                     reinterpret_cast<uintptr_t>(hist)) & 15) == 0;
    long parts = (n + RS_MIN_CHUNK - 1) / RS_MIN_CHUNK;
    if (parts > RS_MAX_PARTS) parts = RS_MAX_PARTS;
    long chunk = (n + parts - 1) / parts;
    chunk = (chunk + 7) / 8 * 8;
    parts = (n + chunk - 1) / chunk;
    const long per_block = vec ? 256 * 8 : 256;
    const long blocks = (n + per_block - 1) / per_block;
    if (blocks > 0x7fffffffL) { set_error("cfg_rescale_linear: sample too large"); return 1; }
    const dim3 gs((unsigned)parts, (unsigned)B), ga((unsigned)blocks, (unsigned)B);
    if (vec) {
        hipLaunchKernelGGL(rs_stats_kernel<true>, gs, dim3(256), 0, s, eps2b, part, n, chunk, total, g);
        hipLaunchKernelGGL(rs_apply_kernel<true>, ga, dim3(256), 0, s, eps2b, lat, hist, part, (int)parts, n, total, g, phi, cx,
                           ce, ch, hx, he, factors);
    } else {
        hipLaunchKernelGGL(rs_stats_kernel<false>, gs, dim3(256), 0, s, eps2b, part, n, chunk, total, g);
        hipLaunchKernelGGL(rs_apply_kernel<false>, ga, dim3(256), 0, s, eps2b, lat, hist, part, (int)parts, n, total, g, phi, cx,
                           ce, ch, hx, he, factors);
    }
    SD_HIP_CHECK(hipGetLastError());
    return 0;
}
int launch_clip_embed(const int* ids, const half_t* tok, const half_t* pos, half_t* out, int B, int T, int H, int vocab,
                      hipStream_t s) {
    if (H % 8 != 0) { set_error("clip_embed: hidden size must be a multiple of 8"); return 1; }
    const long n = (long)B * T * (H / 8);
    hipLaunchKernelGGL(clip_embed_kernel, grid1d(n), dim3(256), 0, s, ids, tok, pos, out, (long)B * T, T, H / 8, vocab);
    SD_HIP_CHECK(hipGetLastError());
    return 0;
}
int launch_gather_rows(const half_t* x, long ldx, const int* idx, half_t* out16, float* out32, int B, int T, int H,
                       hipStream_t s) {
    hipLaunchKernelGGL(gather_rows_kernel, grid1d((long)B * H), dim3(256), 0, s, x, ldx, idx, out16, out32, B, T, H);
    SD_HIP_CHECK(hipGetLastError());
    return 0;
}
int launch_inpaint_blend(half_t* lat, const half_t* img, const half_t* noise, const half_t* mask, float a, float b, int B,
                         int C, long HW, hipStream_t s) {
    const long n = (long)B * C * HW;
    if (n == 0) return 0;
    hipLaunchKernelGGL(inpaint_blend_kernel, grid1d(n), dim3(256), 0, s, lat, img, noise, mask, a, b, C, HW, n);
    SD_HIP_CHECK(hipGetLastError());
    return 0;
}
int launch_ln_fold(half_t* w, long K, int rows, const float* gamma, const float* beta, const float* bias_in,
                   float* bias, float* wsum, int rows_scaled, float row_scale, hipStream_t s) {
    if (rows <= 0) return 0;
    hipLaunchKernelGGL(ln_fold_kernel, dim3((rows + 3) / 4), dim3(256), 0, s, w, K, rows, gamma, beta, bias_in, bias, wsum,
                       rows_scaled, row_scale);
    SD_HIP_CHECK(hipGetLastError());
    return 0;
}
int launch_scale_f16(half_t* x, long n, float scale, hipStream_t s) {
    if (n <= 0) return 0;
    hipLaunchKernelGGL(scale_f16_kernel, grid1d(n), dim3(256), 0, s, x, n, scale);
    SD_HIP_CHECK(hipGetLastError());
    return 0;
}
int launch_image_to_uint8(const half_t* img, unsigned char* out, int B, int C, long HW, hipStream_t s) {
    const long total = (long)B * HW;
    if (total == 0) return 0;
    hipLaunchKernelGGL(image_to_uint8_kernel, grid1d(total), dim3(256), 0, s, img, out, C, HW, total);
    SD_HIP_CHECK(hipGetLastError());
    return 0;
}

}
```

### stablediffusion_amd/csrc/model.h

```cpp
#pragma once
#include "../../include/sd_engine.h"
#include "engine.h"

#include <functional>

namespace sd {

const std::string& last_error();

struct Resnet {
    NormW n1, n2;
    ConvW c1, c2, sc;
    bool has_sc = false;
    int temb_off = -1;
    int cin = 0, cout = 0;
};
struct TBlock {
    NormW ln1, ln2, ln3;
    ConvW qkv, out1, q2, out2, ff1, ff2;
    int kv_off = 0;
    int ip_kv_off = 0;
    bool fold = false;
};
struct Xformer {
    NormW gn;
    ConvW pin, pout;
    std::vector<TBlock> blocks;
    int C = 0, heads = 1;
};
struct VaeAttn {
    NormW gn;
    ConvW qkv, out;
    int C = 0;
};

struct CfgShare {
    std::vector<RowDupSeg> segs;
};

void run_resnet(Ctx& c, const Resnet& r, View x, int N, int H, int W, View out, int G, float eps,
                const float* tproj, int tproj_ld, const GnStatBuf* x_stats = nullptr, GnStatBuf** out_stats = nullptr,
                float stream_scale = 1.f, GnStatBuf* out_buf = nullptr, int out_groups = 0);
void run_xformer(Ctx& c, const Xformer& t, View x, int N, int H, int W, View out, int G, View text_kv, int L,
                 const GnStatBuf* x_stats = nullptr, GnStatBuf** out_stats = nullptr, GnStatBuf* out_buf = nullptr,
                 int out_groups = 0, const CfgShare* share = nullptr);

struct UNet;

std::vector<std::pair<std::string, int>> unet_xattn_sites(const sd_unet_config& cfg, bool mid_last);

struct IPAdapter {
    IPAdapter(const sd_unet_config& c, int image_embed_dim, int num_tokens);
    int finalize();

    sd_unet_config cfg;
    int d_img = 0, n_tok = 0;
    WeightStore ws;
    bool finalized = false;
    ConvW proj;
    NormW norm;
    ConvW kv_all;
    int kv_total = 0;
    UNet* attached = nullptr;
};

struct Encoder {
    explicit Encoder(const sd_unet_config& c) : cfg(c) {}

    sd_unet_config cfg;
    WeightStore ws;
    ConvW conv_in, te1, te2, ae1, ae2, temb_stack;
    ConvW tcp;
    ConvW kv_all;
    std::vector<std::string> kv_keys;
    std::vector<std::vector<Resnet>> down_res;
    std::vector<std::vector<Xformer>> down_att;
    std::vector<ConvW> down_ds;
    Resnet mid_r0, mid_r1;
    Xformer mid_att;
    int temb_total = 0;
    int kv_total = 0;

    int num_skips() const;
    using SkipDst = std::function<View(int si)>;
    using SkipStat = std::function<GnStatBuf*(int si, long HW, int C)>;

  protected:
    void declare_encoder();
    int pack_encoder(std::vector<std::string>* tw, std::vector<std::string>* tb);
    int pack_resnet(const std::string& p, Resnet* r, std::vector<std::string>* tw, std::vector<std::string>* tb);
    int pack_xformer(const std::string& p, Xformer* x, int heads, int depth);
    int run_temb(Ctx& c, const float* timesteps, const half_t* add_text, const float* add_time_ids, int B, float** tproj,
                 int rows_alloc = 0, const float* tcond = nullptr);
    void run_conv_in(Ctx& c, const half_t* sample, int B, int H, int W, View y0, GnStatBuf* gb, const View* res,
                     GnStatBuf** xs);
    View run_down(Ctx& c, View x, GnStatBuf*& xs, int B, int& h, int& w, View text_kv, int L, const float* tproj,
                  const SkipDst& dst, const SkipStat& stat, const CfgShare* share = nullptr);
    void run_mid(Ctx& c, View x, GnStatBuf* xs, int B, int h, int w, View text_kv, int L, const float* tproj, View dst);
};

struct ControlNet : Encoder {
    ControlNet(const sd_unet_config& c, int conditioning_channels);
    ~ControlNet();
    int finalize();

    int cond_channels = 3;
    bool finalized = false;
    static constexpr int kCondLayers = 7;
    float* cond_w[kCondLayers] = {};
    float* cond_b[kCondLayers] = {};
    int cond_cin[kCondLayers] = {}, cond_cout[kCondLayers] = {}, cond_stride[kCondLayers] = {};
    ConvW cond_out;
    std::vector<ConvW> zero;
    ConvW zero_mid;
    UNet* attached = nullptr;

    void run_cond_embed(Ctx& c, const half_t* image, int n, int H, int W, View out);
    int run(Ctx& c, const half_t* sample, const float* timesteps, View text_kv, int L, const half_t* add_text,
            const float* add_time_ids, int B, int H, int W, View emb, const std::vector<View>& sites, View mid);
};

bool unet_cfg_share_eligible(const sd_unet_config& cfg);

struct CfgIn {
    const half_t* latents = nullptr;
    float in_scale = 1.f;
};

struct UNet : Encoder {
    explicit UNet(const sd_unet_config& c);
    int finalize();
    int forward_cfg(const half_t* latents, const float* timesteps, const half_t* ehs, int L, const half_t* add_text,
                    const float* add_time_ids, const half_t* image_embeds, int n_img, float in_scale, bool share,
                    half_t* out, int B, int H, int W, hipStream_t stream);
    bool cfg_share_active(bool share) const;
    char* cfg_slab = nullptr;
    size_t cfg_cap = 0;
    int forward(const half_t* sample, const float* timesteps, const half_t* ehs, int L,
                const half_t* add_text, const float* add_time_ids, half_t* out, int B, int H, int W,
                hipStream_t stream, const half_t* image_embeds = nullptr, int n_img = 0,
                const half_t* control = nullptr, int n_ctrl = 0, float cn_scale = 0.f, const CfgIn* cfg_in = nullptr,
                const float* tcond = nullptr);
    void set_ip_adapter(IPAdapter* a);
    void set_controlnet(ControlNet* n);

    Arena arena;
    bool finalized = false;
    long planned_key = -1;
    long planned_cn = -1;

    bool graph_enabled = false;
    hipStream_t gstream = nullptr;
    hipEvent_t ev_in = nullptr, ev_out = nullptr;
    hipGraphExec_t gexec = nullptr;
    long graph_key = -1;
    char* io_slab = nullptr;
    size_t io_cap = 0;
    int forward_graph(const half_t* sample, const float* timesteps, const half_t* ehs, int L, const half_t* add_text,
                      const float* add_time_ids, half_t* out, int B, int H, int W, hipStream_t stream,
                      const float* tcond = nullptr);
    ~UNet();

    bool kv_cache_on = false, kv_valid = false;
    half_t* kv_cache = nullptr;
    size_t kv_cap = 0;
    const half_t* kv_src = nullptr;
    int kv_B = 0, kv_L = 0;

    IPAdapter* ip = nullptr;
    float ip_scale = 1.f;
    bool ipkv_valid = false;
    half_t* ipkv_cache = nullptr;
    size_t ipkv_cap = 0;
    const half_t* ipkv_src = nullptr;
    int ipkv_B = 0, ipkv_n = 0;

    ControlNet* cn = nullptr;
    bool cond_valid = false, cnkv_valid = false;
    half_t* cond_cache = nullptr;
    size_t cond_cap = 0;
    const half_t* cond_src = nullptr;
    int cond_B = 0, cond_n = 0, cond_H = 0, cond_W = 0;
    half_t* cnkv_cache = nullptr;
    size_t cnkv_cap = 0;
    const half_t* cnkv_src = nullptr;
    int cnkv_B = 0, cnkv_L = 0;

    bool freeu_on = false;
    float freeu_s1 = 1.f, freeu_s2 = 1.f, freeu_b1 = 1.f, freeu_b2 = 1.f;

    ConvW conv_out;
    NormW norm_out;
    std::vector<std::vector<Resnet>> up_res;
    std::vector<std::vector<Xformer>> up_att;
    std::vector<ConvW> up_us;

  private:
    int run(Ctx& c, const half_t* sample, const float* timesteps, const half_t* ehs, int L,
// ... 75 lines not shown
```

### stablediffusion_amd/csrc/runtime.cpp

```cpp
#include "engine.h"

#include <atomic>
#include <cstdio>
#include <mutex>
#include <cstdlib>
#include <cstring>

namespace sd {

static thread_local std::string g_last_error;
void set_error(const std::string& msg) { g_last_error = msg; }
const std::string& last_error() { return g_last_error; }

Arena::~Arena() {
    if (base_) (void)hipFree(base_);
}

int Arena::reserve(size_t bytes) {
    if (bytes <= cap_) return 0;
    if (base_) { (void)hipFree(base_); base_ = nullptr; cap_ = 0; }
    SD_HIP_CHECK(hipMalloc(reinterpret_cast<void**>(&base_), bytes));
    cap_ = bytes;
    return 0;
}
// ... 88 lines not shown
    if (!t) { set_error("missing weight: " + key); return 2; }
    std::vector<half_t> h((size_t)t->numel);
    SD_HIP_CHECK(hipMemcpy(h.data(), t->dev, (size_t)t->numel * sizeof(half_t), hipMemcpyDeviceToHost));
    out->resize((size_t)t->numel);
    for (long i = 0; i < t->numel; ++i) (*out)[(size_t)i] = (float)h[(size_t)i];
    return 0;
}

static long round_up(long a, long b) { return (a + b - 1) / b * b; }

static int upload_bias(WeightStore* ws, const std::vector<float>& host, int cout, float** dst) {
    const long padded = round_up(cout, kWeightRowPad);
    std::vector<float> buf((size_t)padded, 0.f);
    std::memcpy(buf.data(), host.data(), (size_t)cout * sizeof(float));
    *dst = static_cast<float*>(ws->dmalloc((size_t)padded * sizeof(float)));
    if (!*dst) { set_error("hipMalloc failed (bias)"); return 3; }
    SD_HIP_CHECK(hipMemcpy(*dst, buf.data(), (size_t)padded * sizeof(float), hipMemcpyHostToDevice));
    return 0;
}

int WeightStore::pack_conv(const std::string& prefix, ConvW* out, bool has_bias) {
    const RawTensor* w = raw(prefix + ".weight");
    if (!w) { set_error("missing weight: " + prefix + ".weight"); return 2; }
    const int O = (int)w->shape[0], I = (int)w->shape[1];
    const int KH = w->shape.size() == 4 ? (int)w->shape[2] : 1;
    const int KW = w->shape.size() == 4 ? (int)w->shape[3] : 1;
    const long K = round_up((long)KH * KW * I, 64);
    const long rows = round_up(O, kWeightRowPad);
    out->cin = I; out->cout = O; out->ks = KH; out->K = K;
    out->w = static_cast<half_t*>(dmalloc((size_t)rows * K * sizeof(half_t)));
    if (!out->w) { set_error("hipMalloc failed (weights)"); return 3; }
    SD_HIP_CHECK(hipMemsetAsync(out->w, 0, (size_t)rows * K * sizeof(half_t), 0));
    int rc = launch_pack_conv(w->dev, out->w, O, I, KH, KW, K, 0);
    if (rc) return rc;
    out->bias = nullptr;
    if (has_bias) {
        std::vector<float> b;
        rc = host_floats(prefix + ".bias", &b);
        if (rc) return rc;
        rc = upload_bias(this, b, O, &out->bias);
        if (rc) return rc;
    }
    return 0;
}

int WeightStore::pack_rows(const std::vector<std::string>& wkeys, const std::vector<std::string>& bkeys,
                           ConvW* out) {
    long total = 0;
    int I = -1;
    for (const auto& k : wkeys) {
        const RawTensor* w = raw(k);
        if (!w) { set_error("missing weight: " + k); return 2; }
        if (I < 0) I = (int)w->shape[1];
        if ((int)w->shape[1] != I) { set_error("pack_rows: inner dims differ at " + k); return 1; }
        total += w->shape[0];
    }
    if (I % 64 != 0) { set_error("pack_rows: inner dim must be a multiple of 64"); return 1; }
    const long rows = round_up(total, kWeightRowPad);
    out->cin = I; out->cout = (int)total; out->ks = 1; out->K = I;
    out->w = static_cast<half_t*>(dmalloc((size_t)rows * I * sizeof(half_t)));
    if (!out->w) { set_error("hipMalloc failed (weights)"); return 3; }
    SD_HIP_CHECK(hipMemsetAsync(out->w, 0, (size_t)rows * I * sizeof(half_t), 0));
    long r = 0;
    for (const auto& k : wkeys) {
        const RawTensor* w = raw(k);
        SD_HIP_CHECK(hipMemcpyAsync(out->w + r * I, w->dev, (size_t)w->numel * sizeof(half_t),
                                    hipMemcpyDeviceToDevice, 0));
        r += w->shape[0];
    }
    out->bias = nullptr;
    if (!bkeys.empty()) {
        std::vector<float> all;
        for (const auto& k : bkeys) {
            std::vector<float> b;
            int rc = host_floats(k, &b);
            if (rc) return rc;
            all.insert(all.end(), b.begin(), b.end());
        }
        if ((long)all.size() != total) { set_error("pack_rows: bias length mismatch"); return 1; }
        int rc = upload_bias(this, all, (int)total, &out->bias);
        if (rc) return rc;
    }
    return 0;
}

int WeightStore::pack_geglu(const std::string& prefix, ConvW* out) {
    const RawTensor* w = raw(prefix + ".weight");
    if (!w) { set_error("missing weight: " + prefix + ".weight"); return 2; }
    const long O = w->shape[0], I = w->shape[1];
    const long half_rows = O / 2;
    if (half_rows % 64 != 0 || I % 64 != 0) { set_error("pack_geglu: dims must be multiples of 64"); return 1; }
    const long rows = round_up(O, kWeightRowPad);
    out->cin = (int)I; out->cout = (int)O; out->ks = 1; out->K = I;
    out->w = static_cast<half_t*>(dmalloc((size_t)rows * I * sizeof(half_t)));
    if (!out->w) { set_error("hipMalloc failed (weights)"); return 3; }
    SD_HIP_CHECK(hipMemsetAsync(out->w, 0, (size_t)rows * I * sizeof(half_t), 0));
    std::vector<float> b, bp((size_t)O);
    int rc = host_floats(prefix + ".bias", &b);
    if (rc) return rc;
    for (long blk = 0; blk < half_rows / 64; ++blk) {
        SD_HIP_CHECK(hipMemcpyAsync(out->w + (blk * 128) * I, w->dev + (blk * 64) * I,
                                    (size_t)64 * I * sizeof(half_t), hipMemcpyDeviceToDevice, 0));
        SD_HIP_CHECK(hipMemcpyAsync(out->w + (blk * 128 + 64) * I, w->dev + (half_rows + blk * 64) * I,
                                    (size_t)64 * I * sizeof(half_t), hipMemcpyDeviceToDevice, 0));
        for (int e = 0; e < 64; ++e) {
            bp[(size_t)(blk * 128 + e)] = b[(size_t)(blk * 64 + e)];
            bp[(size_t)(blk * 128 + 64 + e)] = b[(size_t)(half_rows + blk * 64 + e)];
        }
    }
    return upload_bias(this, bp, (int)O, &out->bias);
}

int WeightStore::pack_norm(const std::string& prefix, NormW* out) {
    std::vector<float> g, b;
    int rc = host_floats(prefix + ".weight", &g);
    if (rc) return rc;
    rc = host_floats(prefix + ".bias", &b);
    if (rc) return rc;
    out->C = (int)g.size();
    out->gamma = static_cast<float*>(dmalloc(g.size() * sizeof(float)));
    out->beta = static_cast<float*>(dmalloc(b.size() * sizeof(float)));
    if (!out->gamma || !out->beta) { set_error("hipMalloc failed (norm)"); return 3; }
    SD_HIP_CHECK(hipMemcpy(out->gamma, g.data(), g.size() * sizeof(float), hipMemcpyHostToDevice));
    SD_HIP_CHECK(hipMemcpy(out->beta, b.data(), b.size() * sizeof(float), hipMemcpyHostToDevice));
    out->gb = nullptr;
    if (g.size() % 64 == 0) {
        std::vector<float> gb(2 * g.size());
        for (size_t blk = 0; blk < g.size() / 64; ++blk)
            for (int e = 0; e < 64; ++e) {
                gb[blk * 128 + e] = g[blk * 64 + e];
                gb[blk * 128 + 64 + e] = b[blk * 64 + e];
            }
        out->gb = static_cast<float*>(dmalloc(gb.size() * sizeof(float)));
        if (!out->gb) { set_error("hipMalloc failed (norm)"); return 3; }
        SD_HIP_CHECK(hipMemcpy(out->gb, gb.data(), gb.size() * sizeof(float), hipMemcpyHostToDevice));
    }
    return 0;
}

int WeightStore::fold_ln(ConvW* w, const NormW& ln, int rows_scaled, float row_scale) {
    if (ln.C != w->K || w->ks != 1) { set_error("fold_ln: LayerNorm width must equal the linear's K"); return 1; }
    const long padded = round_up(w->cout, kWeightRowPad);
    float* nb = static_cast<float*>(dmalloc((size_t)padded * sizeof(float)));
    w->wsum = static_cast<float*>(dmalloc((size_t)padded * sizeof(float)));
    if (!nb || !w->wsum) { set_error("hipMalloc failed (fold_ln)"); return 3; }
    SD_HIP_CHECK(hipMemsetAsync(nb, 0, (size_t)padded * sizeof(float), 0));
    SD_HIP_CHECK(hipMemsetAsync(w->wsum, 0, (size_t)padded * sizeof(float), 0));
    int rc = launch_ln_fold(w->w, w->K, w->cout, ln.gamma, ln.beta, w->bias, nb, w->wsum, rows_scaled, row_scale, 0);
    if (rc) return rc;
    w->bias = nb;
    return 0;
}

namespace {
struct ProfRec { std::string name; double flops, bytes; hipEvent_t a, b; };
std::atomic<bool> g_prof_on{false};
std::mutex g_prof_mu;
std::vector<ProfRec> g_prof;
}
void prof_enable(bool on) { g_prof_on = on; }
bool prof_enabled() { return g_prof_on; }
void prof_open(hipStream_t s, const char* kernel, double flops, double bytes) {
    if (!g_prof_on) return;
    ProfRec r{kernel, flops, bytes, nullptr, nullptr};
    if (hipEventCreate(&r.a) != hipSuccess || hipEventCreate(&r.b) != hipSuccess) return;
    (void)hipEventRecord(r.a, s);
    std::lock_guard<std::mutex> lk(g_prof_mu);
    g_prof.push_back(r);
}
void prof_close(hipStream_t s) {
    if (!g_prof_on) return;
    std::lock_guard<std::mutex> lk(g_prof_mu);
    if (g_prof.empty()) return;
    (void)hipEventRecord(g_prof.back().b, s);
}
int prof_collect(std::map<std::string, ProfAgg>* out) {
    SD_HIP_CHECK(hipDeviceSynchronize());
    std::lock_guard<std::mutex> lk(g_prof_mu);
    for (auto& r : g_prof) {
        float ms = 0.f;
        if (hipEventElapsedTime(&ms, r.a, r.b) == hipSuccess) {
            ProfAgg& a = (*out)[r.name];
            a.flops += r.flops; a.bytes += r.bytes; a.ms += ms; a.launches += 1;
        }
        (void)hipEventDestroy(r.a); (void)hipEventDestroy(r.b);
    }
    g_prof.clear();
    return 0;
}

void ctx_gnpool_init(Ctx& c, int N, long HW_max, int G) {
    static const bool off = getenv("SD_NO_GN_EPILOGUE") != nullptr;
    c.gn_groups = G;
    c.gn_next = 0;
    for (int i = 0; i < Ctx::kGnPool; ++i) {
        c.gnpool[i].buf = off ? nullptr : c.arena->alloc_f(gnstat_floats(N, HW_max, G));
        c.gnpool[i].st = GnStats();
    }
}

GnStatBuf* ctx_gnbuf(Ctx& c) {
    if (!c.gnpool[0].buf) return nullptr;
    GnStatBuf* b = &c.gnpool[c.gn_next];
    c.gn_next = (c.gn_next + 1) % Ctx::kGnPool;
    b->st = GnStats();
    return b;
}

void op_conv(Ctx& c, const ConvW& w, View x, int N, int H, int W, View y, int stride, int up,
             const float* rowadd, int rowadd_ld, const View* res, int geglu, int pad, int act, const ConvFuse* fuse) {
    const RowStat* ln_in = fuse ? fuse->ln_in : nullptr;
    const float ln_eps = fuse ? fuse->ln_eps : 0.f;
    RowStat* stat_out = fuse ? fuse->stat_out : nullptr;
    GnStatBuf* gn_out = fuse ? fuse->gn_out : nullptr;
    IGemmParams p;
    p.x = x.p; p.ldx = x.ld;
    p.w = w.w; p.bias = w.bias;
    p.rowadd = rowadd; p.rowadd_ld = rowadd_ld;
    p.res = res ? res->p : nullptr; p.ldres = res ? res->ld : 0;
    p.y = y.p; p.ldy = y.ld;
    p.N = N; p.H = H; p.W = W; p.Cin = (w.ks == 1) ? (int)w.K : w.cin;
    p.KS = w.ks; p.stride = stride; p.up = up;
    p.pad = pad >= 0 ? pad : (w.ks == 3 ? 1 : 0);
    const int IH = H << up, IW = W << up;
    if (stride == 1) {
        p.OH = IH; p.OW = IW;
    } else if (p.pad == 0) {
        p.OH = (IH + 1 - w.ks) / stride + 1; p.OW = (IW + 1 - w.ks) / stride + 1;
    } else {
        p.OH = (IH + 2 * p.pad - w.ks) / stride + 1; p.OW = (IW + 2 * p.pad - w.ks) / stride + 1;
    }
    p.Cout = w.cout;
    p.M = N * p.OH * p.OW;
    p.K = (int)w.K;
    p.geglu = geglu;
    p.act = act;
    if (ln_in) {
        if (!w.wsum) { set_error("op_conv: LayerNorm statistics passed to a linear without folded weights"); c.err = 1; return; }
        p.ln_stat = ln_in->p; p.ln_parts = ln_in->parts; p.ln_part_w = ln_in->width; p.ln_C = (int)w.K; p.ln_eps = ln_eps; p.ln_wsum = w.wsum;
    }
    if (fuse && fuse->gn_in) {
        p.gni_part = fuse->gn_in_stats.part; p.gni_S = fuse->gn_in_stats.S; p.gni_rows = fuse->gn_in_stats.rows;
        p.gni_groups = fuse->gn_in_groups; p.gni_eps = fuse->gn_in_eps; p.gni_silu = fuse->gn_in_silu;
        p.gni_gb = fuse->gn_in->gb;
        if (c.dry) p.gni_part = reinterpret_cast<const float*>(8);
    }
    if (fuse && (fuse->acc_scale != 1.f || fuse->bias_scale != 1.f)) { p.acc_scale = fuse->acc_scale; p.bias_scale = fuse->bias_scale; }
    const IGemmPlan plan = igemm2_plan(p, IGemmRequest{stat_out ? stat_out->p : nullptr, gn_out ? gn_out->buf : nullptr,
                                                       fuse ? fuse->gn_groups : 0});
    const bool v2 = plan.kind != kKindIgemm1;
    if ((p.acc_scale != 1.f || p.bias_scale != 1.f) && !plan.scales_ok) { set_error("op_conv: output scaling needs the LDS-DMA kernels (not GEGLU / weight-stationary)"); c.err = 1; return; }
    if (ln_in && !v2) { set_error("op_conv: the LayerNorm fold needs the LDS-DMA kernel"); c.err = 1; return; }
    if (act && !v2) { set_error("op_conv: activation epilogue needs the LDS-DMA kernel (Cin % 64, Cout % 8)"); c.err = 1; return; }
    if (gn_out) {
        gn_out->st = GnStats();
        if (plan.gnstats) { gn_out->st.part = gn_out->buf; gn_out->st.rows = plan.gn_rows; gn_out->st.S = p.OH * p.OW / plan.gn_rows; }
    }
    const bool own_stats = plan.rowstats;
    if (stat_out) { stat_out->parts = plan.rs_parts; stat_out->width = plan.rs_part_w; }
    float* partial = plan.partial_floats > 0 ? c.arena->alloc_f(plan.partial_floats) : nullptr;
    if (c.dry || c.err) return;
    if (prof_enabled()) {
        const double kreal = (double)w.ks * w.ks * w.cin;
        const double in_px = (double)N * H * W;
        const char* name = plan.name;
        static const bool by_shape = getenv("SD_PROF_SHAPES") != nullptr;
        char nbuf[64];
        if (v2 && by_shape) {
            snprintf(nbuf, sizeof(nbuf), "%s%d/k%d %dx%dx%d ks%d%s%s%s%s%s%s", plan.kind == kKindPgemmGeglu ? "pg" : "v", plan.variant,
                     plan.splits, p.M, p.Cout, p.K, p.KS, res ? " res" : "", geglu ? " geglu" : "", p.ln_stat ? " ln" : "",
                     p.rowstat_out ? " rs" : "", p.gnstat_out ? " gs" : "", p.gni_part ? " gn" : "");
            name = nbuf;
        }
        prof_open(c.stream, name, 2.0 * p.M * w.cout * kreal,
                  2.0 * (in_px * (w.ks == 1 ? (double)w.K : w.cin) + (double)w.cout * w.K +
                         (double)p.M * (geglu ? w.cout / 2 : w.cout) * (res ? 2 : 1)));
    }
    c.err = launch_igemm2(p, partial, c.stream, &plan);
    prof_close(c.stream);
    if (stat_out && !own_stats && !c.err) {
        prof_open(c.stream, "row_stats_kernel", 0.0, 2.0 * p.M * w.cout);
        c.err = launch_row_stats(y.p, y.ld, stat_out->p, p.M, w.cout, c.stream);
        prof_close(c.stream);
    }
}

void op_groupnorm(Ctx& c, const NormW& n, View x, View y, int N, long HW, int G, float eps, int silu,
                  const GnStatBuf* pre) {
    float* scratch = c.arena->alloc_f(gn_scratch_floats(N, HW, n.C, G));
    if (c.dry || c.err) return;
    const GnStats* st = (pre && pre->st.part && gn_wants_stats(HW, n.C, G)) ? &pre->st : nullptr;
    const bool own_pass = gn_wants_stats(HW, n.C, G) && !st;
    const char* gname = own_pass ? "groupnorm(stats+apply)" : "groupnorm(apply)";
    static thread_local char gbuf[64];
    static const bool gn_by_shape = getenv("SD_PROF_SHAPES") != nullptr;
    if (gn_by_shape && prof_enabled()) {
        snprintf(gbuf, sizeof(gbuf), "gn%s %ldx%d%s", own_pass ? "(stats+apply)" : (st ? "(apply)" : "(fused)"), (long)N * HW, n.C, silu ? " silu" : "");
        gname = gbuf;
    }
    prof_open(c.stream, gname, 0.0, (own_pass ? 6.0 : 4.0) * N * HW * n.C);
    c.err = launch_groupnorm(x.p, x.ld, n.gamma, n.beta, y.p, y.ld, N, HW, n.C, G, eps, silu, scratch, c.stream, st);
    prof_close(c.stream);
}

void op_gn_conv(Ctx& c, const NormW& n, const ConvW& w, View x, int N, int H, int W, View y, int G, float eps, int silu,
                const GnStatBuf* pre, const float* rowadd, int rowadd_ld, const View* res, const ConvFuse* fuse) {
    static const bool off = getenv("SD_GN_FUSE") == nullptr || getenv("SD_NO_GN_FUSE") != nullptr;
    const long HW = (long)H * W;
    IGemmParams q;
    q.x = x.p; q.ldx = x.ld; q.N = N; q.H = H; q.W = W; q.Cin = (w.ks == 1) ? (int)w.K : w.cin;
    q.KS = w.ks; q.stride = 1; q.up = 0; q.pad = w.ks == 3 ? 1 : 0; q.OH = H; q.OW = W; q.Cout = w.cout;
    q.M = N * H * W; q.K = (int)w.K;
    const bool fused = !off && n.gb && n.C == q.Cin && igemm2_gn_fusable(q, G);
    if (!fused) {
        const size_t mk = c.arena->mark();
        View hn(c.arena->alloc_h((long)N * HW * n.C), n.C, n.C);
        op_groupnorm(c, n, x, hn, N, HW, G, eps, silu, pre);
        op_conv(c, w, hn, N, H, W, y, 1, 0, rowadd, rowadd_ld, res, 0, -1, 0, fuse);
        c.arena->release(mk);
        return;
    }
    const size_t mk = c.arena->mark();
    ConvFuse f = fuse ? *fuse : ConvFuse();
    f.gn_in = &n; f.gn_in_groups = G; f.gn_in_eps = eps; f.gn_in_silu = silu;
    float* scratch = c.arena->alloc_f(gn_scratch_floats(N, HW, n.C, G) + (long)N * G * 2);
    if (pre && pre->st.part) {
        f.gn_in_stats = pre->st;
        if (f.gn_in_stats.S > 64 && !c.dry && !c.err) {
            prof_open(c.stream, "gn_finalize_kernel", 0.0, 8.0 * N * f.gn_in_stats.S * G);
            c.err = launch_gn_finalize(&f.gn_in_stats, scratch, N, HW, n.C, G, c.stream);
            prof_close(c.stream);
        }
    } else if (!c.dry && !c.err) {
        static thread_local char gbuf[64];
        static const bool by_shape = getenv("SD_PROF_SHAPES") != nullptr;
        const char* name = "groupnorm(stats)";
        if (by_shape && prof_enabled()) { snprintf(gbuf, sizeof(gbuf), "gn(stats) %ldx%d", (long)N * HW, n.C); name = gbuf; }
        prof_open(c.stream, name, 0.0, 2.0 * N * HW * n.C);
        c.err = launch_gn_stats(x.p, x.ld, N, HW, n.C, G, scratch, &f.gn_in_stats, c.stream);
        prof_close(c.stream);
    }
    op_conv(c, w, x, N, H, W, y, 1, 0, rowadd, rowadd_ld, res, 0, -1, 0, &f);
    c.arena->release(mk);
}

bool op_ffn_fused(Ctx& c, const ConvW& ff1, const ConvW& ff2, View x, const RowStat& x_stat, float ln_eps, long M, View y) {
    FfnParams p;
    p.x = x.p; p.ldx = x.ld; p.y = y.p; p.ldy = y.ld;
    p.w1 = ff1.w; p.b1 = ff1.bias; p.wsum1 = ff1.wsum;
    p.w1_rows = (int)(((long)ff1.cout + kWeightRowPad - 1) / kWeightRowPad * kWeightRowPad);
    p.w2 = ff2.w; p.b2 = ff2.bias;
    p.w2_rows = (int)(((long)ff2.cout + kWeightRowPad - 1) / kWeightRowPad * kWeightRowPad);
    p.ln_stat = x_stat.p; p.ln_parts = x_stat.parts; p.ln_part_w = x_stat.width; p.ln_eps = ln_eps;
    p.M = (int)M; p.C = (int)ff1.K; p.hidden = (int)ff2.K;
    if (c.dry) p.ln_stat = reinterpret_cast<const float*>(8);
    if (ff1.ks != 1 || ff2.ks != 1 || ff2.cout != ff1.K || ff1.cout != 2 * ff2.K || x.C != p.C || !ff1.wsum) return false;
    if (c.dry ? !(p.C == 320 && p.hidden == 1280 && M % 128 == 0 && M / 128 >= 64 && !getenv("SD_NO_FFN_FUSE")) : !ffn_fused_supported(p))
        return false;
    if (c.dry || c.err) return true;
    prof_open(c.stream, "ffn_fused_kernel", 2.0 * M * ((double)ff1.cout * ff1.K + (double)ff2.cout * ff2.K),
              2.0 * ((double)M * p.C * 2 + (double)ff1.cout * ff1.K + (double)ff2.cout * ff2.K));
    c.err = launch_ffn_fused(p, c.stream);
    prof_close(c.stream);
    return true;
}

void op_layernorm(Ctx& c, const NormW& n, View x, View y, long rows, float eps) {
    if (c.dry || c.err) return;
    prof_open(c.stream, "layernorm_kernel", 0.0, 4.0 * rows * n.C);
    c.err = launch_layernorm(x.p, x.ld, n.gamma, n.beta, y.p, y.ld, rows, n.C, eps, c.stream);
    prof_close(c.stream);
}

void op_attention(Ctx& c, View q, View k, View v, View out, int B, int Tq, int Tk, int heads, int d, int causal,
                  int prescaled) {
    if (c.dry || c.err) return;
    if (prof_enabled()) {
        static thread_local char name[32];
        snprintf(name, sizeof(name), "attn_kernel<%d>", d);
        prof_open(c.stream, name, 4.0 * B * heads * (double)Tq * Tk * d,
                  2.0 * B * heads * d * (2.0 * Tq + 2.0 * Tk));
    }
    c.err = launch_attention(q.p, k.p, v.p, out.p, B, Tq, Tk, heads, d, q.ld, k.ld, v.ld, out.ld, c.stream, causal, prescaled);
    prof_close(c.stream);
}

void op_ip_attention(Ctx& c, View q, View k, View v, View k_ip, View v_ip, View out, int B, int Tq, int L, int T_ip,
                     int heads, int d, float ip_scale) {
    if (c.dry || c.err) return;
    if (prof_enabled()) {
        static thread_local char name[32];
        snprintf(name, sizeof(name), "ip_xattn_kernel<%d>", d);
        prof_open(c.stream, name, 4.0 * B * heads * (double)Tq * (L + T_ip) * d,
                  2.0 * B * heads * d * (2.0 * Tq + 2.0 * L + 2.0 * T_ip));
    }
    c.err = launch_ip_attention(q.p, k.p, v.p, k_ip.p, v_ip.p, out.p, B, Tq, L, T_ip, heads, d, q.ld, k.ld, v.ld, k_ip.ld,
                                v_ip.ld, out.ld, ip_scale, 1, c.stream);
    prof_close(c.stream);
}

}
```

### stablediffusion_amd/csrc/unet.cpp

```cpp
#include <algorithm>
#include <vector>

#include "model.h"
#include <cmath>
#include <cstdlib>

namespace sd {

void declare_resnet(WeightStore& ws, const std::string& p, int cin, int cout, int temb) {
    ws.declare(p + ".norm1.weight", {cin});
    ws.declare(p + ".norm1.bias", {cin});
    ws.declare(p + ".conv1.weight", {cout, cin, 3, 3});
    ws.declare(p + ".conv1.bias", {cout});
    if (temb) {
        ws.declare(p + ".time_emb_proj.weight", {cout, temb});
        ws.declare(p + ".time_emb_proj.bias", {cout});
    }
    ws.declare(p + ".norm2.weight", {cout});
    ws.declare(p + ".norm2.bias", {cout});
    ws.declare(p + ".conv2.weight", {cout, cout, 3, 3});
    ws.declare(p + ".conv2.bias", {cout});
    if (cin != cout) {
        ws.declare(p + ".conv_shortcut.weight", {cout, cin, 1, 1});
        ws.declare(p + ".conv_shortcut.bias", {cout});
    }
}

namespace {

void declare_xformer(WeightStore& ws, const std::string& p, int c, int depth, int ctx, bool linear) {
    ws.declare(p + ".norm.weight", {c});
    ws.declare(p + ".norm.bias", {c});
    if (linear) ws.declare(p + ".proj_in.weight", {c, c}); else ws.declare(p + ".proj_in.weight", {c, c, 1, 1});
    ws.declare(p + ".proj_in.bias", {c});
    for (int d = 0; d < depth; ++d) {
        const std::string b = p + ".transformer_blocks." + std::to_string(d);
        ws.declare(b + ".norm1.weight", {c});
        ws.declare(b + ".norm1.bias", {c});
        ws.declare(b + ".attn1.to_q.weight", {c, c});
        ws.declare(b + ".attn1.to_k.weight", {c, c});
        ws.declare(b + ".attn1.to_v.weight", {c, c});
        ws.declare(b + ".attn1.to_out.0.weight", {c, c});
        ws.declare(b + ".attn1.to_out.0.bias", {c});
        ws.declare(b + ".norm2.weight", {c});
        ws.declare(b + ".norm2.bias", {c});
        ws.declare(b + ".attn2.to_q.weight", {c, c});
        ws.declare(b + ".attn2.to_k.weight", {c, ctx});
        ws.declare(b + ".attn2.to_v.weight", {c, ctx});
        ws.declare(b + ".attn2.to_out.0.weight", {c, c});
        ws.declare(b + ".attn2.to_out.0.bias", {c});
        ws.declare(b + ".norm3.weight", {c});
        ws.declare(b + ".norm3.bias", {c});
        ws.declare(b + ".ff.net.0.proj.weight", {8 * c, c});
        ws.declare(b + ".ff.net.0.proj.bias", {8 * c});
        ws.declare(b + ".ff.net.2.weight", {c, 4 * c});
        ws.declare(b + ".ff.net.2.bias", {c});
    }
    if (linear) ws.declare(p + ".proj_out.weight", {c, c}); else ws.declare(p + ".proj_out.weight", {c, c, 1, 1});
    ws.declare(p + ".proj_out.bias", {c});
}

}

void Encoder::declare_encoder() {
    const int nb = cfg.num_blocks;
    const int* boc = cfg.block_out_channels;
    const int temb = boc[0] * 4;
    const int ctx = cfg.cross_attention_dim;
    const bool lin = cfg.use_linear_projection != 0;
    ws.declare("conv_in.weight", {boc[0], cfg.in_channels, 3, 3});
    ws.declare("conv_in.bias", {boc[0]});
    ws.declare("time_embedding.linear_1.weight", {temb, boc[0]});
    ws.declare("time_embedding.linear_1.bias", {temb});
    ws.declare("time_embedding.linear_2.weight", {temb, temb});
    ws.declare("time_embedding.linear_2.bias", {temb});
    if (cfg.time_cond_proj_dim > 0) ws.declare("time_embedding.cond_proj.weight", {boc[0], cfg.time_cond_proj_dim});
    if (cfg.addition_time_embed_dim > 0) {
        ws.declare("add_embedding.linear_1.weight", {temb, cfg.projection_class_embeddings_input_dim});
        ws.declare("add_embedding.linear_1.bias", {temb});
        ws.declare("add_embedding.linear_2.weight", {temb, temb});
        ws.declare("add_embedding.linear_2.bias", {temb});
    }
    int out_ch = boc[0];
    for (int i = 0; i < nb; ++i) {
        const int in_ch = out_ch;
        out_ch = boc[i];
        for (int j = 0; j < cfg.layers_per_block; ++j) {
            const std::string p = "down_blocks." + std::to_string(i);
            declare_resnet(ws, p + ".resnets." + std::to_string(j), j == 0 ? in_ch : out_ch, out_ch, temb);
            if (cfg.down_block_has_attn[i])
                declare_xformer(ws, p + ".attentions." + std::to_string(j), out_ch, cfg.transformer_layers[i], ctx, lin);
        }
        if (i != nb - 1) {
            ws.declare("down_blocks." + std::to_string(i) + ".downsamplers.0.conv.weight", {out_ch, out_ch, 3, 3});
            ws.declare("down_blocks." + std::to_string(i) + ".downsamplers.0.conv.bias", {out_ch});
        }
    }
    const int mid = boc[nb - 1];
    declare_resnet(ws, "mid_block.resnets.0", mid, mid, temb);
    declare_xformer(ws, "mid_block.attentions.0", mid, cfg.transformer_layers[nb - 1], ctx, lin);
    declare_resnet(ws, "mid_block.resnets.1", mid, mid, temb);
}

UNet::UNet(const sd_unet_config& c) : Encoder(c) {
    declare_encoder();
    const int nb = cfg.num_blocks;
    const int* boc = cfg.block_out_channels;
    const int temb = boc[0] * 4;
    const int ctx = cfg.cross_attention_dim;
    const bool lin = cfg.use_linear_projection != 0;
    int out_ch;
    out_ch = boc[nb - 1];
    for (int i = 0; i < nb; ++i) {
        const int prev = out_ch;
        out_ch = boc[nb - 1 - i];
        const int in_ch = boc[nb - 1 - (i + 1 < nb ? i + 1 : nb - 1)];
        const std::string p = "up_blocks." + std::to_string(i);
        for (int j = 0; j < cfg.layers_per_block + 1; ++j) {
            const int skip = (j == cfg.layers_per_block) ? in_ch : out_ch;
            const int rin = (j == 0) ? prev : out_ch;
            declare_resnet(ws, p + ".resnets." + std::to_string(j), rin + skip, out_ch, temb);
            if (cfg.up_block_has_attn[i])
                declare_xformer(ws, p + ".attentions." + std::to_string(j), out_ch,
                                cfg.transformer_layers[nb - 1 - i], ctx, lin);
        }
        if (i != nb - 1) {
            ws.declare(p + ".upsamplers.0.conv.weight", {out_ch, out_ch, 3, 3});
            ws.declare(p + ".upsamplers.0.conv.bias", {out_ch});
        }
    }
    ws.declare("conv_norm_out.weight", {boc[0]});
    ws.declare("conv_norm_out.bias", {boc[0]});
    ws.declare("conv_out.weight", {cfg.out_channels, boc[0], 3, 3});
    ws.declare("conv_out.bias", {cfg.out_channels});
}

int Encoder::pack_resnet(const std::string& p, Resnet* r, std::vector<std::string>* tw, std::vector<std::string>* tb) {
    int rc;
    if ((rc = ws.pack_norm(p + ".norm1", &r->n1))) return rc;
    if ((rc = ws.pack_conv(p + ".conv1", &r->c1))) return rc;
    if ((rc = ws.pack_norm(p + ".norm2", &r->n2))) return rc;
    if ((rc = ws.pack_conv(p + ".conv2", &r->c2))) return rc;
    r->cin = r->c1.cin; r->cout = r->c1.cout;
    r->has_sc = ws.raw(p + ".conv_shortcut.weight") != nullptr;
    if (r->has_sc && (rc = ws.pack_conv(p + ".conv_shortcut", &r->sc))) return rc;
    if (tw) {
        r->temb_off = temb_total;
        temb_total += r->cout;
        tw->push_back(p + ".time_emb_proj.weight");
        tb->push_back(p + ".time_emb_proj.bias");
    }
    return 0;
}

int Encoder::pack_xformer(const std::string& p, Xformer* x, int heads, int depth) {
    int rc;
    if ((rc = ws.pack_norm(p + ".norm", &x->gn))) return rc;
    if ((rc = ws.pack_conv(p + ".proj_in", &x->pin))) return rc;
    if ((rc = ws.pack_conv(p + ".proj_out", &x->pout))) return rc;
    x->C = x->pin.cout;
    x->heads = heads;
    x->blocks.resize((size_t)depth);
    for (int d = 0; d < depth; ++d) {
        TBlock& b = x->blocks[(size_t)d];
        const std::string q = p + ".transformer_blocks." + std::to_string(d);
        if ((rc = ws.pack_norm(q + ".norm1", &b.ln1))) return rc;
        if ((rc = ws.pack_norm(q + ".norm2", &b.ln2))) return rc;
        if ((rc = ws.pack_norm(q + ".norm3", &b.ln3))) return rc;
        if ((rc = ws.pack_rows({q + ".attn1.to_q.weight", q + ".attn1.to_k.weight", q + ".attn1.to_v.weight"}, {}, &b.qkv))) return rc;
        if ((rc = ws.pack_conv(q + ".attn1.to_out.0", &b.out1))) return rc;
        if ((rc = ws.pack_conv(q + ".attn2.to_q", &b.q2, false))) return rc;
        const float qs = 1.4426950408889634f / sqrtf((float)(x->C / heads));
        b.kv_off = kv_total;
        b.ip_kv_off = kv_total;
        kv_total += 2 * x->C;
        kv_keys.push_back(q + ".attn2.to_k.weight");
        kv_keys.push_back(q + ".attn2.to_v.weight");
        if ((rc = ws.pack_conv(q + ".attn2.to_out.0", &b.out2))) return rc;
        if ((rc = ws.pack_geglu(q + ".ff.net.0.proj", &b.ff1))) return rc;
        if ((rc = ws.pack_conv(q + ".ff.net.2", &b.ff2))) return rc;
        static const bool no_fold = getenv("SD_NO_LN_FOLD") != nullptr;
        b.fold = !no_fold;
        if (b.fold) {
            if ((rc = ws.fold_ln(&b.qkv, b.ln1, x->C, qs))) return rc;
            if ((rc = ws.fold_ln(&b.q2, b.ln2, x->C, qs))) return rc;
            if ((rc = ws.fold_ln(&b.ff1, b.ln3, 0, 1.0f))) return rc;
        } else {
            if ((rc = launch_scale_f16(b.qkv.w, (long)x->C * b.qkv.K, qs, 0))) return rc;
            if ((rc = launch_scale_f16(b.q2.w, (long)x->C * b.q2.K, qs, 0))) return rc;
        }
    }
    return 0;
}

int Encoder::pack_encoder(std::vector<std::string>* tw, std::vector<std::string>* tb) {
    const int nb = cfg.num_blocks;
    int rc;
    if ((rc = ws.pack_conv("conv_in", &conv_in))) return rc;
    if ((rc = ws.pack_conv("time_embedding.linear_1", &te1))) return rc;
    if ((rc = ws.pack_conv("time_embedding.linear_2", &te2))) return rc;
    if (cfg.time_cond_proj_dim > 0 && (rc = ws.pack_conv("time_embedding.cond_proj", &tcp, false))) return rc;
    if (cfg.addition_time_embed_dim > 0) {
        if ((rc = ws.pack_conv("add_embedding.linear_1", &ae1))) return rc;
        if ((rc = ws.pack_conv("add_embedding.linear_2", &ae2))) return rc;
    }
    down_res.assign((size_t)nb, {}); down_att.assign((size_t)nb, {}); down_ds.assign((size_t)nb, ConvW());
    for (int i = 0; i < nb; ++i) {
        const std::string p = "down_blocks." + std::to_string(i);
        down_res[i].resize((size_t)cfg.layers_per_block);
        if (cfg.down_block_has_attn[i]) down_att[i].resize((size_t)cfg.layers_per_block);
        for (int j = 0; j < cfg.layers_per_block; ++j) {
            if ((rc = pack_resnet(p + ".resnets." + std::to_string(j), &down_res[i][j], tw, tb))) return rc;
            if (cfg.down_block_has_attn[i] &&
                (rc = pack_xformer(p + ".attentions." + std::to_string(j), &down_att[i][j], cfg.num_heads[i],
                                   cfg.transformer_layers[i]))) return rc;
        }
        if (i != nb - 1 && (rc = ws.pack_conv(p + ".downsamplers.0.conv", &down_ds[i]))) return rc;
    }
    if ((rc = pack_resnet("mid_block.resnets.0", &mid_r0, tw, tb))) return rc;
    if ((rc = pack_xformer("mid_block.attentions.0", &mid_att, cfg.num_heads[nb - 1], cfg.transformer_layers[nb - 1]))) return rc;
    if ((rc = pack_resnet("mid_block.resnets.1", &mid_r1, tw, tb))) return rc;
    return 0;
}

int UNet::finalize() {
    if (finalized) return 0;
    std::string missing;
    if (!ws.complete(&missing)) { set_error("finalize: weight not set: " + missing); return 2; }
    const int nb = cfg.num_blocks;
    int rc;
    std::vector<std::string> tw, tb;
    temb_total = 0;
    kv_total = 0;
    kv_keys.clear();
    if ((rc = pack_encoder(&tw, &tb))) return rc;
    up_res.assign((size_t)nb, {}); up_att.assign((size_t)nb, {}); up_us.assign((size_t)nb, ConvW());
    for (int i = 0; i < nb; ++i) {
        const std::string p = "up_blocks." + std::to_string(i);
        up_res[i].resize((size_t)cfg.layers_per_block + 1);
        if (cfg.up_block_has_attn[i]) up_att[i].resize((size_t)cfg.layers_per_block + 1);
        for (int j = 0; j < cfg.layers_per_block + 1; ++j) {
            if ((rc = pack_resnet(p + ".resnets." + std::to_string(j), &up_res[i][j], &tw, &tb))) return rc;
            if (cfg.up_block_has_attn[i] &&
                (rc = pack_xformer(p + ".attentions." + std::to_string(j), &up_att[i][j], cfg.num_heads[nb - 1 - i],
                                   cfg.transformer_layers[nb - 1 - i]))) return rc;
        }
        if (i != nb - 1 && (rc = ws.pack_conv(p + ".upsamplers.0.conv", &up_us[i]))) return rc;
    }
    if ((rc = ws.pack_norm("conv_norm_out", &norm_out))) return rc;
    if ((rc = ws.pack_conv("conv_out", &conv_out))) return rc;
    if ((rc = ws.pack_rows(tw, tb, &temb_stack))) return rc;
    if (!kv_keys.empty() && (rc = ws.pack_rows(kv_keys, {}, &kv_all))) return rc;
    kv_keys.clear();
    SD_HIP_CHECK(hipDeviceSynchronize());
    ws.free_raw();
    finalized = true;
    return 0;
}

std::vector<std::pair<std::string, int>> unet_xattn_sites(const sd_unet_config& cfg, bool mid_last) {
    const int nb = cfg.num_blocks;
    const int* boc = cfg.block_out_channels;
    std::vector<std::pair<std::string, int>> down, up, mid;
    auto add = [](std::vector<std::pair<std::string, int>>& v, const std::string& p, int depth, int C) {
        for (int k = 0; k < depth; ++k) v.emplace_back(p + ".transformer_blocks." + std::to_string(k), C);
    };
    for (int i = 0; i < nb; ++i)
        if (cfg.down_block_has_attn[i])
            for (int j = 0; j < cfg.layers_per_block; ++j)
                add(down, "down_blocks." + std::to_string(i) + ".attentions." + std::to_string(j), cfg.transformer_layers[i], boc[i]);
    add(mid, "mid_block.attentions.0", cfg.transformer_layers[nb - 1], boc[nb - 1]);
    for (int i = 0; i < nb; ++i)
        if (cfg.up_block_has_attn[i])
            for (int j = 0; j < cfg.layers_per_block + 1; ++j)
                add(up, "up_blocks." + std::to_string(i) + ".attentions." + std::to_string(j),
                    cfg.transformer_layers[nb - 1 - i], boc[nb - 1 - i]);
    std::vector<std::pair<std::string, int>> all = down;
    const auto& second = mid_last ? up : mid;
    const auto& third = mid_last ? mid : up;
    all.insert(all.end(), second.begin(), second.end());
    all.insert(all.end(), third.begin(), third.end());
    return all;
}

namespace {
const char* kIpProj = "encoder_hid_proj.image_projection_layers.0";
}

IPAdapter::IPAdapter(const sd_unet_config& c, int image_embed_dim, int num_tokens)
    : cfg(c), d_img(image_embed_dim), n_tok(num_tokens) {
    const int ctx = cfg.cross_attention_dim;
    const std::string p = kIpProj;
    ws.declare(p + ".image_embeds.weight", {(int64_t)n_tok * ctx, d_img});
    ws.declare(p + ".image_embeds.bias", {(int64_t)n_tok * ctx});
    ws.declare(p + ".norm.weight", {ctx});
    ws.declare(p + ".norm.bias", {ctx});
    for (const auto& site : unet_xattn_sites(cfg, true)) {
        ws.declare(site.first + ".attn2.processor.to_k_ip.0.weight", {site.second, ctx});
        ws.declare(site.first + ".attn2.processor.to_v_ip.0.weight", {site.second, ctx});
    }
}

int IPAdapter::finalize() {
    if (finalized) return 0;
    std::string missing;
    if (!ws.complete(&missing)) { set_error("ip adapter finalize: weight not set: " + missing); return 2; }
    const std::string p = kIpProj;
    int rc;
    if ((rc = ws.pack_conv(p + ".image_embeds", &proj))) return rc;
    if ((rc = ws.pack_norm(p + ".norm", &norm))) return rc;
    std::vector<std::string> keys;
    kv_total = 0;
    for (const auto& site : unet_xattn_sites(cfg, false)) {
        keys.push_back(site.first + ".attn2.processor.to_k_ip.0.weight");
        keys.push_back(site.first + ".attn2.processor.to_v_ip.0.weight");
        kv_total += 2 * site.second;
    }
    if ((rc = ws.pack_rows(keys, {}, &kv_all))) return rc;
    SD_HIP_CHECK(hipDeviceSynchronize());
    ws.free_raw();
    finalized = true;
    return 0;
}

void UNet::set_ip_adapter(IPAdapter* a) {
    if (ip == a) return;
    if (ip) ip->attached = nullptr;
    if (a) {
        if (a->attached && a->attached != this) a->attached->set_ip_adapter(nullptr);
        a->attached = this;
    }
    ip = a;
    ipkv_valid = false;
    planned_key = -1;
}

void run_resnet(Ctx& c, const Resnet& r, View x, int N, int H, int W, View out, int G, float eps,
                const float* tproj, int tproj_ld, const GnStatBuf* x_stats, GnStatBuf** out_stats, float stream_scale,
                GnStatBuf* out_buf, int out_groups) {
    Arena& a = *c.arena;
    const size_t mk = a.mark();
    const long M = (long)N * H * W;
    const float s = stream_scale, eps_s = eps * s * s;
    View h2(a.alloc_h(M * r.cout), r.cout, r.cout);
    const long HW = (long)H * W;
    ConvFuse f1;
    f1.gn_out = gn_wants_stats(HW, r.cout, G) ? ctx_gnbuf(c) : nullptr;
    f1.gn_groups = G;
    f1.acc_scale = s; f1.bias_scale = s;
    op_gn_conv(c, r.n1, r.c1, x, N, H, W, h2, G, eps_s, 1, x_stats, tproj ? tproj + r.temb_off : nullptr, tproj_ld, nullptr, &f1);
    View res = x;
    if (r.has_sc) {
        res = View(a.alloc_h(M * r.cout), r.cout, r.cout);
        ConvFuse fs;
        fs.bias_scale = s;
        op_conv(c, r.sc, x, N, H, W, res, 1, 0, nullptr, 0, nullptr, 0, -1, 0, s != 1.f ? &fs : nullptr);
    }
    ConvFuse f2;
    f2.gn_out = (out_stats && gn_wants_stats(HW, r.cout, G)) ? (out_buf ? out_buf : ctx_gnbuf(c)) : nullptr;
    f2.gn_groups = out_groups > 0 ? out_groups : G;
    f2.acc_scale = s; f2.bias_scale = s;
    op_gn_conv(c, r.n2, r.c2, h2, N, H, W, out, G, eps_s, 1, f1.gn_out, nullptr, 0, &res, &f2);
    if (out_stats) *out_stats = f2.gn_out;
    a.release(mk);
}

void run_xformer(Ctx& c, const Xformer& t, View x, int N, int H, int W, View out, int G, View text_kv, int L,
                 const GnStatBuf* x_stats, GnStatBuf** out_stats, GnStatBuf* out_buf, int out_groups, const CfgShare* share) {
    Arena& a = *c.arena;
    const size_t mk = a.mark();
    const int C = t.C;
    const int T = H * W;
    const long M = (long)N * T;
    const int d = C / t.heads;
    const bool fold = !t.blocks.empty() && t.blocks[0].fold;
    int Np = share ? N / 2 : N;
    long Mp = (long)Np * T;
    View hn(a.alloc_h(M * C), C, C);
    op_groupnorm(c, t.gn, x, hn, Np, T, G, 1e-6f, 0, x_stats);
    View cur(a.alloc_h(M * C), C, C), nxt(a.alloc_h(M * C), C, C);
    RowStat st_cur, st_t2, st_t3;
    if (fold) {
        st_cur.p = a.alloc_f(rowstat_floats(M, C));
        st_t2.p = a.alloc_f(rowstat_floats(M, C));
        st_t3.p = a.alloc_f(rowstat_floats(M, C));
    }
    ConvFuse f_cur, f_t2, f_t3, f_ln1, f_ln2, f_ln3;
    f_cur.stat_out = &st_cur; f_t2.stat_out = &st_t2; f_t3.stat_out = &st_t3;
    f_ln1.ln_in = &st_cur; f_ln2.ln_in = &st_t2; f_ln3.ln_in = &st_t3;
    f_ln1.ln_eps = f_ln2.ln_eps = f_ln3.ln_eps = 1e-5f;
    op_conv(c, t.pin, hn, Np, H, W, cur, 1, 0, nullptr, 0, nullptr, 0, -1, 0, fold ? &f_cur : nullptr);
    for (size_t bi = 0; bi < t.blocks.size(); ++bi) {
        const TBlock& b = t.blocks[bi];
        const bool more = bi + 1 < t.blocks.size();
        const size_t mb = a.mark();
        View n(fold ? nullptr : a.alloc_h(M * C), C, C);
        View qkv(a.alloc_h(M * 3 * C), 3 * C, 3 * C);
        if (fold) {
            op_conv(c, b.qkv, cur, Np, H, W, qkv, 1, 0, nullptr, 0, nullptr, 0, -1, 0, &f_ln1);
        } else {
            op_layernorm(c, b.ln1, cur, n, Mp, 1e-5f);
            op_conv(c, b.qkv, n, Np, H, W, qkv);
        }
        View att(a.alloc_h(M * C), C, C);
        op_attention(c, qkv.slice(0, C), qkv.slice(C, C), qkv.slice(2 * C, C), att, Np, T, T, t.heads, d, 0, 1);
        View t2(a.alloc_h(M * C), C, C);
        op_conv(c, b.out1, att, Np, H, W, t2, 1, 0, nullptr, 0, &cur, 0, -1, 0, fold ? &f_t2 : nullptr);
        View q(a.alloc_h(M * C), C, C);
        if (fold) {
            op_conv(c, b.q2, t2, Np, H, W, q, 1, 0, nullptr, 0, nullptr, 0, -1, 0, &f_ln2);
        } else {
            op_layernorm(c, b.ln2, t2, n, Mp, 1e-5f);
            op_conv(c, b.q2, n, Np, H, W, q);
        }
        if (Np != N) {
            std::vector<RowDupSeg> segs = share->segs;
            for (const View& v : {q, t2, x}) {
                RowDupSeg g;
                g.src = v.p; g.dst = v.p + Mp * v.ld;
                g.ld_bytes = v.ld * 2; g.row_bytes = (long)v.C * 2; g.rows = Mp;
                segs.push_back(g);
            }
            if (!c.dry && !c.err) {
                double bytes = 0;
                for (const RowDupSeg& g : segs) bytes += 2.0 * g.rows * g.row_bytes;
                prof_open(c.stream, "row_dup_kernel", 0.0, bytes);
                c.err = launch_row_dup(segs.data(), (int)segs.size(), c.stream);
                prof_close(c.stream);
            }
            Np = N; Mp = M;
        }
        if (c.ip_kv.p && c.ip_scale != 0.f)
            op_ip_attention(c, q, text_kv.slice(b.kv_off, C), text_kv.slice(b.kv_off + C, C), c.ip_kv.slice(b.ip_kv_off, C),
                            c.ip_kv.slice(b.ip_kv_off + C, C), att, N, T, L, c.ip_T, t.heads, d, c.ip_scale);
        else
            op_attention(c, q, text_kv.slice(b.kv_off, C), text_kv.slice(b.kv_off + C, C), att, N, T, L, t.heads, d, 0, 1);
        View t3(a.alloc_h(M * C), C, C);
        op_conv(c, b.out2, att, N, H, W, t3, 1, 0, nullptr, 0, &t2, 0, -1, 0, fold ? &f_t3 : nullptr);
        if (!(fold && !more && op_ffn_fused(c, b.ff1, b.ff2, t3, st_t3, 1e-5f, M, nxt))) {
            View g(a.alloc_h(M * 4 * C), 4 * C, 4 * C);
            if (fold) {
                op_conv(c, b.ff1, t3, N, H, W, g, 1, 0, nullptr, 0, nullptr, 1, -1, 0, &f_ln3);
            } else {
                op_layernorm(c, b.ln3, t3, n, M, 1e-5f);
                op_conv(c, b.ff1, n, N, H, W, g, 1, 0, nullptr, 0, nullptr, 1);
            }
            op_conv(c, b.ff2, g, N, H, W, nxt, 1, 0, nullptr, 0, &t3, 0, -1, 0, (fold && more) ? &f_cur : nullptr);
        }
        a.release(mb);
        View tmp = cur; cur = nxt; nxt = tmp;
    }
    ConvFuse fo;
    fo.gn_out = (out_stats && gn_wants_stats(T, C, G)) ? (out_buf ? out_buf : ctx_gnbuf(c)) : nullptr;
    fo.gn_groups = out_groups > 0 ? out_groups : G;
    op_conv(c, t.pout, cur, N, H, W, out, 1, 0, nullptr, 0, &x, 0, -1, 0, &fo);
    if (out_stats) *out_stats = fo.gn_out;
    a.release(mk);
}

int Encoder::run_temb(Ctx& c, const float* timesteps, const half_t* add_text, const float* add_time_ids, int B,
                      float** tproj_out, int rows_alloc, const float* tcond) {
    Arena& a = *c.arena;
    const int* boc = cfg.block_out_channels;
    const int temb = boc[0] * 4;
    hipStream_t s = c.stream;
    const bool go = !c.dry;
    float* sinus = a.alloc_f((long)B * boc[0]);
    float* e1 = a.alloc_f((long)B * temb);
    float* emb = a.alloc_f((long)B * temb);
    float* tproj = a.alloc_f((long)std::max(B, rows_alloc) * temb_total);
    *tproj_out = tproj;
    if (go && !c.err)
        c.err = tcond ? launch_timestep_cond(timesteps, tcond, tcp.w, tcp.K, sinus, B, boc[0], cfg.time_cond_proj_dim,
                                             cfg.flip_sin_to_cos, cfg.freq_shift, s)
                      : launch_timestep_sinusoid(timesteps, 1, sinus, B, boc[0], cfg.flip_sin_to_cos, cfg.freq_shift, boc[0], s);
    if (go && !c.err) c.err = launch_small_linear(sinus, boc[0], te1.w, te1.bias, e1, temb, B, boc[0], temb, 0, 1, s);
    const bool aug_path = cfg.addition_time_embed_dim > 0;
    if (go && !c.err) c.err = launch_small_linear(e1, temb, te2.w, te2.bias, emb, temb, B, temb, temb, 0, aug_path ? 0 : 1, s);
    if (aug_path) {
        const int ad = cfg.addition_time_embed_dim;
        const int pin = cfg.projection_class_embeddings_input_dim;
        const int tdim = pin - 6 * ad;
        if (!add_text || !add_time_ids) { set_error("unet: add_text / add_time_ids required for text_time conditioning"); return 1; }
        float* addin = a.alloc_f((long)B * pin);
        float* a1 = a.alloc_f((long)B * temb);
        float* aug = a.alloc_f((long)B * temb);
        float* txt = a.alloc_f((long)B * tdim);
        if (go && !c.err) c.err = launch_f16_to_f32(add_text, txt, (long)B * tdim, s);
        if (go && !c.err) {
            hipError_t e = hipMemcpy2DAsync(addin, (size_t)pin * 4, txt, (size_t)tdim * 4, (size_t)tdim * 4, (size_t)B,
                                            hipMemcpyDeviceToDevice, s);
            if (e != hipSuccess) { set_error(hipGetErrorString(e)); c.err = 3; }
        }
        if (go && !c.err) {
            for (int j = 0; j < 6 && !c.err; ++j)
                c.err = launch_timestep_sinusoid(add_time_ids + j, 6, addin + tdim + j * ad, B, ad,
                                                         cfg.flip_sin_to_cos, cfg.freq_shift, pin, s);
        }
        if (go && !c.err) c.err = launch_small_linear(addin, pin, ae1.w, ae1.bias, a1, temb, B, pin, temb, 0, 1, s);
        if (go && !c.err) c.err = launch_small_linear(a1, temb, ae2.w, ae2.bias, aug, temb, B, temb, temb, 0, 0, s);
        if (go && !c.err) c.err = launch_add_f32(emb, aug, (long)B * temb, 1, s);
    }
    if (go && !c.err) c.err = launch_small_linear(emb, temb, temb_stack.w, temb_stack.bias, tproj, temb_total, B, temb, temb_total, 0, 0, s);

    return c.err;
}

void Encoder::run_conv_in(Ctx& c, const half_t* sample, int B, int H, int W, View y0, GnStatBuf* gb, const View* res,
                          GnStatBuf** xs) {
    Arena& a = *c.arena;
    const int* boc = cfg.block_out_channels;
    const int G = cfg.norm_num_groups;
    hipStream_t s = c.stream;
    const bool go = !c.dry;
    const size_t mk = a.mark();
    const long M = (long)B * H * W;
    HeadParams hp;
    hp.x_nchw = sample; hp.w = conv_in.w; hp.K = conv_in.K; hp.bias = conv_in.bias; hp.y = y0.p; hp.ldy = y0.ld;
    hp.gnstat_out = (gb && gb->buf) ? gb->buf : nullptr; hp.G = G;
    hp.N = B; hp.Cin = cfg.in_channels; hp.H = H; hp.W = W; hp.Cout = boc[0];
    if (!res && conv_head_supported(hp)) {
        if (gb) {
            gb->st = GnStats();
            if (hp.gnstat_out) { gb->st.part = gb->buf; gb->st.rows = 128; gb->st.S = (int)((long)H * W / 128); }
        }
        if (go && !c.err) {
            prof_open(s, "conv_head_kernel", 2.0 * M * boc[0] * 9.0 * cfg.in_channels, 2.0 * M * (boc[0] + cfg.in_channels));
            c.err = launch_conv_head(hp, s);
            prof_close(s);
        }
        *xs = gb;
    } else {
        half_t* col = a.alloc_h(M * conv_in.K);
        if (go && !c.err) c.err = launch_im2col_nchw3x3(sample, col, B, cfg.in_channels, H, W, (int)conv_in.K, s);
        ConvW pw = conv_in; pw.ks = 1;
        ConvFuse f;
        f.gn_out = gb;
        f.gn_groups = G;
        op_conv(c, pw, View(col, conv_in.K, (int)conv_in.K), B, H, W, y0, 1, 0, nullptr, 0, res, 0, -1, 0, &f);
        *xs = f.gn_out;
    }
    a.release(mk);
}

View Encoder::run_down(Ctx& c, View x, GnStatBuf*& xs, int B, int& h, int& w, View text_kv, int L, const float* tproj,
                       const SkipDst& skip_view, const SkipStat& skip_stat, const CfgShare* share) {
    Arena& a = *c.arena;
    const int nb = cfg.num_blocks;
    const int G = cfg.norm_num_groups;
    const float eps = cfg.norm_eps;
    int skip_i = 1;
    for (int i = 0; i < nb; ++i) {
        for (int j = 0; j < cfg.layers_per_block; ++j) {
            const Resnet& r = down_res[i][j];
            if (cfg.down_block_has_attn[i]) {
                const size_t mk = a.mark();
                View tmp(a.alloc_h((long)B * h * w * r.cout), r.cout, r.cout);
                GnStatBuf* rs = nullptr;
                const CfgShare* sh = (i == 0 && j == 0) ? share : nullptr;
                run_resnet(c, r, x, sh ? B / 2 : B, h, w, tmp, G, eps, tproj, temb_total, xs, &rs);
                View dst = skip_view(skip_i);
                run_xformer(c, down_att[i][j], tmp, B, h, w, dst, G, text_kv, L, rs, &xs, skip_stat(skip_i, (long)h * w, r.cout),
                            0, sh);
                a.release(mk);
                x = dst;
            } else {
                View dst = skip_view(skip_i);
                run_resnet(c, r, x, B, h, w, dst, G, eps, tproj, temb_total, xs, &xs, 1.f, skip_stat(skip_i, (long)h * w, r.cout));
                x = dst;
            }
            ++skip_i;
        }
        if (i != nb - 1) {
            ConvFuse f;
            f.gn_out = skip_stat(skip_i, (long)(h / 2) * (w / 2), down_ds[i].cout);
            View dst = skip_view(skip_i++);
            f.gn_groups = G;
            op_conv(c, down_ds[i], x, B, h, w, dst, 2, 0, nullptr, 0, nullptr, 0, -1, 0, &f);
            xs = f.gn_out;
            h /= 2; w /= 2;
            x = dst;
        }
    }

    return x;
}

void Encoder::run_mid(Ctx& c, View x, GnStatBuf* xs, int B, int h, int w, View text_kv, int L, const float* tproj,
                      View dst) {
    Arena& a = *c.arena;
    const int nb = cfg.num_blocks;
    const int* boc = cfg.block_out_channels;
    const int G = cfg.norm_num_groups;
    const float eps = cfg.norm_eps;
    const int C = boc[nb - 1];
    const long M = (long)B * h * w;
    View m0(a.alloc_h(M * C), C, C), m1(a.alloc_h(M * C), C, C);
    GnStatBuf *s0 = nullptr, *s1 = nullptr;
    run_resnet(c, mid_r0, x, B, h, w, m0, G, eps, tproj, temb_total, xs, &s0);
    run_xformer(c, mid_att, m0, B, h, w, m1, G, text_kv, L, s0, &s1);
    run_resnet(c, mid_r1, m1, B, h, w, dst, G, eps, tproj, temb_total, s1);
}

int Encoder::num_skips() const { return 1 + cfg.num_blocks * cfg.layers_per_block + (cfg.num_blocks - 1); }

int UNet::run(Ctx& c, const half_t* sample, const float* timesteps, const half_t* ehs, int L,
              const half_t* add_text, const float* add_time_ids, half_t* out, int B, int H, int W,
              const half_t* image_embeds, int n_img, const half_t* control, int n_ctrl, float cn_scale, const CfgIn* cfg_in,
              const float* tcond) {
    Arena& a = *c.arena;
// ... 506 lines not shown
```

### stablediffusion_amd/shapes.py

```python
from __future__ import annotations

from dataclasses import dataclass
from typing import List

from .config import UNetConfig, VAEConfig


@dataclass(frozen=True)
class ConvShape:
    N: int
    H: int
    W: int
    Cin: int
    Cout: int
    ks: int = 1
    stride: int = 1
    up: int = 0
    geglu: int = 0
    tag: str = ""

    @property
    def out_hw(self):
        ih, iw = self.H << self.up, self.W << self.up
        if self.stride == 1:
            return ih, iw
        pad = 1 if self.ks == 3 else 0
        return (ih + 2 * pad - self.ks) // self.stride + 1, (iw + 2 * pad - self.ks) // self.stride + 1

    @property
    def M(self):
        oh, ow = self.out_hw
        return self.N * oh * ow

    @property
    def K(self):
        return self.ks * self.ks * self.Cin

    @property
    def flops(self):
        return 2.0 * self.M * self.Cout * self.K

    def key(self):
        return (self.N, self.H, self.W, self.Cin, self.Cout, self.ks, self.stride, self.up, self.geglu)


def _resnet(out, N, h, w, cin, cout):
    out.append(ConvShape(N, h, w, cin, cout, 3, tag="res.conv1"))
    out.append(ConvShape(N, h, w, cout, cout, 3, tag="res.conv2"))
    if cin != cout:
        out.append(ConvShape(N, h, w, cin, cout, 1, tag="res.shortcut"))


def _xformer(out, N, h, w, C, depth, L, ctx):
    out.append(ConvShape(N, h, w, C, C, 1, tag="proj_in"))
    for _ in range(depth):
        out.append(ConvShape(N, h, w, C, 3 * C, 1, tag="attn1.qkv"))
        out.append(ConvShape(N, h, w, C, C, 1, tag="attn1.out"))
        out.append(ConvShape(N, h, w, C, C, 1, tag="attn2.q"))
        out.append(ConvShape(N, L, 1, ctx, 2 * C, 1, tag="attn2.kv"))
        out.append(ConvShape(N, h, w, C, C, 1, tag="attn2.out"))
        out.append(ConvShape(N, h, w, C, 8 * C, 1, geglu=1, tag="ff.geglu"))
        out.append(ConvShape(N, h, w, 4 * C, C, 1, tag="ff.out"))
    out.append(ConvShape(N, h, w, C, C, 1, tag="proj_out"))


def unet_convs(cfg: UNetConfig, B: int, H: int, W: int, L: int = 77) -> List[ConvShape]:
    out: List[ConvShape] = []
    boc = cfg.block_out_channels
    nb = len(boc)
    ctx = cfg.cross_attention_dim
    h, w = H, W
    out.append(ConvShape(B, h, w, 64, boc[0], 1, tag="conv_in(im2col K=64)"))
    ch = boc[0]
    for i, bt in enumerate(cfg.down_block_types):
        cin, ch = ch, boc[i]
        for j in range(cfg.layers_per_block):
            _resnet(out, B, h, w, cin if j == 0 else ch, ch)
            if bt == "CrossAttnDownBlock2D":
                _xformer(out, B, h, w, ch, cfg.transformer_layers_per_block[i], L, ctx)
        if i != nb - 1:
            out.append(ConvShape(B, h, w, ch, ch, 3, stride=2, tag="downsample"))
            h, w = h // 2, w // 2
    _resnet(out, B, h, w, ch, ch)
    _xformer(out, B, h, w, ch, cfg.transformer_layers_per_block[-1], L, ctx)
    _resnet(out, B, h, w, ch, ch)
    rev = list(reversed(boc))
    rdepth = list(reversed(cfg.transformer_layers_per_block))
    ch = rev[0]
    for i, bt in enumerate(cfg.up_block_types):
        prev, ch = ch, rev[i]
        cin = rev[min(i + 1, nb - 1)]
        for j in range(cfg.layers_per_block + 1):
            skip = cin if j == cfg.layers_per_block else ch
            rin = prev if j == 0 else ch
            _resnet(out, B, h, w, rin + skip, ch)
            if bt == "CrossAttnUpBlock2D":
                _xformer(out, B, h, w, ch, rdepth[i], L, ctx)
        if i != nb - 1:
            out.append(ConvShape(B, h, w, ch, ch, 3, up=1, tag="upsample"))
            h, w = h * 2, w * 2
    out.append(ConvShape(B, h, w, boc[0], cfg.out_channels, 3, tag="conv_out"))
    return out


def unet_attention_flops(cfg: UNetConfig, B: int, H: int, W: int, L: int = 77) -> float:
    boc = cfg.block_out_channels
    nb = len(boc)
    total = 0.0
    h, w = H, W

    def add(C, depth):
        nonlocal total
        T = h * w
        total += depth * (4.0 * B * T * T * C + 4.0 * B * T * L * C)

    for i, bt in enumerate(cfg.down_block_types):
        if bt == "CrossAttnDownBlock2D":
            for _ in range(cfg.layers_per_block):
                add(boc[i], cfg.transformer_layers_per_block[i])
        if i != nb - 1:
            h, w = h // 2, w // 2
    add(boc[-1], cfg.transformer_layers_per_block[-1])
    rev = list(reversed(boc))
    rdepth = list(reversed(cfg.transformer_layers_per_block))
    for i, bt in enumerate(cfg.up_block_types):
        if bt == "CrossAttnUpBlock2D":
            for _ in range(cfg.layers_per_block + 1):
                add(rev[i], rdepth[i])
        if i != nb - 1:
            h, w = h * 2, w * 2
    return total


def vae_decoder_convs(cfg: VAEConfig, B: int, h: int, w: int) -> List[ConvShape]:
    out: List[ConvShape] = []
    boc = cfg.block_out_channels
    top = boc[-1]
    out.append(ConvShape(B, h, w, 64, top, 1, tag="conv_in(im2col K=64)"))
    _resnet(out, B, h, w, top, top)
    out.append(ConvShape(B, h, w, top, 3 * top, 1, tag="mid.qkv"))
    out.append(ConvShape(B, h, w, top, top, 1, tag="mid.attn_out"))
    _resnet(out, B, h, w, top, top)
    ch = top
    rev = list(reversed(boc))
    for i in range(len(boc)):
        prev, ch = ch, rev[i]
        for j in range(cfg.layers_per_block + 1):
            _resnet(out, B, h, w, prev if j == 0 else ch, ch)
        if i != len(boc) - 1:
            out.append(ConvShape(B, h, w, ch, ch, 3, up=1, tag="upsample"))
            h, w = h * 2, w * 2
    out.append(ConvShape(B, h, w, boc[0], cfg.out_channels, 3, tag="conv_out"))
    return out
```

Before: 7.865 latents/s.

## Fold transformer proj_out into last FFN down-projection via concatenated-K GEMM

For transformer blocks whose FFN is not handled by the fused FFN kernel (C != 320), the last block's ff.net.2 and proj_out are algebraically folded. proj_out(ff2(g) + t3) + x becomes one GEMM over [g, t3] with K = hidden + C, using precomputed weights Wpo·W2 and Wpo, so the separate proj_out GEMM launch and the intermediate activation round-trip are removed. Layout is arranged so GEGLU output and t3 sit adjacent in one buffer. Tuned tile hints are passed for the new shape. The trade-off is fp16 rounding of the folded weights (computed with compensated summation) and a larger-K GEMM.

```diff
diff --git a/include/sd_engine.h b/include/sd_engine.h
--- a/include/sd_engine.h
+++ b/include/sd_engine.h
@@ -225,6 +225,12 @@
 int sd_op_ln_ffn_geglu(const void* x, const float* stat, int parts, int part_w, const void* ln_gamma, const void* ln_beta,
                        float ln_eps, const void* w1, const void* b1, const void* w2, const void* b2, void* y, int M, int C,
                        int* fused, void* stream);
+int sd_op_fold_linear(const void* w_outer, const void* b_outer, const void* w_inner, const void* b_inner, void* w_folded,
+                      float* b_folded, int O, int J, int K, void* stream);
+int sd_op_ffn_geglu_proj_out(const void* x_in, const void* t3, const void* ln_gamma, const void* ln_beta, float ln_eps,
+                             const void* w1, const void* b1, const void* w2, const void* b2, const void* w_po,
+                             const void* b_po, void* y, float* gn_summaries, int* gn_rows, int M, int C, int imgs, int* fused,
+                             void* stream);
 int sd_bench_conv2d(const void* x_nhwc, const void* w_oihw, void* y_nhwc, int N, int H, int W, int Cin,
                     int Cout, int ksize, int stride, int upsample2x, int geglu, int iters,
                     float* ms_per_launch, void* stream);
diff --git a/stablediffusion_amd/_lib.py b/stablediffusion_amd/_lib.py
--- a/stablediffusion_amd/_lib.py
+++ b/stablediffusion_amd/_lib.py
@@ -177,6 +177,9 @@
     "sd_op_linear_rowstats": (_I, [_P, _P, _P, _P, _P, _P, _I, _I, _I, C.POINTER(_I), C.POINTER(_I), C.POINTER(_I), _P]),
     "sd_op_ln_linear": (_I, [_P, _P, _I, _I, _P, _P, _F, _P, _P, _P, _I, _I, _I, _I, _I, _F, C.POINTER(_I), _P]),
     "sd_op_ln_ffn_geglu": (_I, [_P, _P, _I, _I, _P, _P, _F, _P, _P, _P, _P, _P, _I, _I, C.POINTER(_I), _P]),
+    "sd_op_fold_linear": (_I, [_P, _P, _P, _P, _P, _P, _I, _I, _I, _P]),
+    "sd_op_ffn_geglu_proj_out": (_I, [_P, _P, _P, _P, _F, _P, _P, _P, _P, _P, _P, _P, _P, C.POINTER(_I), _I, _I, _I,
+                                      C.POINTER(_I), _P]),
     "sd_bench_conv2d": (_I, [_P, _P, _P, _I, _I, _I, _I, _I, _I, _I, _I, _I, _I, C.POINTER(_F), _P]),
     "sd_op_groupnorm": (_I, [_P, _P, _P, _P, _I, _I, _I, _I, _F, _I, _P]),
     "sd_op_groupnorm_concat": (_I, [_P, _I, _I, _P, _P, _P, _I, _I, _I, _F, _I, _P]),
diff --git a/stablediffusion_amd/csrc/capi.cpp b/stablediffusion_amd/csrc/capi.cpp
--- a/stablediffusion_amd/csrc/capi.cpp
+++ b/stablediffusion_amd/csrc/capi.cpp
@@ -1403,4 +1403,89 @@
     });
 }
 
-}
+int sd_op_fold_linear(const void* w_outer, const void* b_outer, const void* w_inner, const void* b_inner, void* w_folded,
+                      float* b_folded, int O, int J, int K, void* stream) {
+    if (!w_outer || !b_outer || !w_inner || !b_inner || !w_folded || !b_folded || O < 1 || J < 1 || K < 1 || (K + J) % 64 != 0) {
+        set_error("sd_op_fold_linear: bad arguments (K + J must be a multiple of 64)"); return SD_ERR_INVALID;
+    }
+    hipStream_t s = static_cast<hipStream_t>(stream);
+    SD_HIP_CHECK(hipStreamSynchronize(s));
+    WeightStore ws;
+    const int64_t so[2] = {O, J}, si[2] = {J, K}, sbo[1] = {O}, sbi[1] = {J};
+    ws.declare("o.weight", {O, J}); ws.declare("o.bias", {O});
+    ws.declare("i.weight", {J, K}); ws.declare("i.bias", {J});
+    int rc;
+    if ((rc = ws.set("o.weight", w_outer, so, 2, 0)) || (rc = ws.set("o.bias", b_outer, sbo, 1, 1)) ||
+        (rc = ws.set("i.weight", w_inner, si, 2, 0)) || (rc = ws.set("i.bias", b_inner, sbi, 1, 1))) return rc;
+    ConvW f;
+    if ((rc = ws.fold_linear("o", "i", &f))) return rc;
+    SD_HIP_CHECK(hipMemcpy(w_folded, f.w, (size_t)O * f.K * sizeof(half_t), hipMemcpyDeviceToDevice));
+    SD_HIP_CHECK(hipMemcpy(b_folded, f.bias, (size_t)O * sizeof(float), hipMemcpyDeviceToDevice));
+    SD_HIP_CHECK(hipDeviceSynchronize());
+    return SD_OK;
+}
+
+int sd_op_ffn_geglu_proj_out(const void* x_in, const void* t3, const void* ln_gamma, const void* ln_beta, float ln_eps,
+                             const void* w1, const void* b1, const void* w2, const void* b2, const void* w_po,
+                             const void* b_po, void* y, float* gn_summaries, int* gn_rows, int M, int C, int imgs, int* fused,
+                             void* stream) {
+    if (!x_in || !t3 || !ln_gamma || !ln_beta || !w1 || !b1 || !w2 || !b2 || !w_po || !b_po || !y || M < 1 || C < 64 ||
+        C % 64 != 0 || imgs < 1 || M % imgs != 0 || ln_eps != 1e-5f) {
+        set_error("sd_op_ffn_geglu_proj_out: bad arguments (C % 64, M % imgs, ln_eps = 1e-5: the transformer's)"); return SD_ERR_INVALID;
+    }
+    hipStream_t s = static_cast<hipStream_t>(stream);
+    SD_HIP_CHECK(hipStreamSynchronize(s));
+    const int G = 32;
+    WeightStore ws;
+    const int64_t C8 = 8L * C, C4 = 4L * C;
+    const int64_t s1[2] = {C8, C}, s2[2] = {C, C4}, so[2] = {C, C}, sc[1] = {C}, s8[1] = {C8};
+    ws.declare("norm3.weight", {C}); ws.declare("norm3.bias", {C});
+    ws.declare("ff.net.0.proj.weight", {C8, C}); ws.declare("ff.net.0.proj.bias", {C8});
+    ws.declare("ff.net.2.weight", {C, C4}); ws.declare("ff.net.2.bias", {C});
+    ws.declare("proj_out.weight", {C, C}); ws.declare("proj_out.bias", {C});
+    int rc;
+    if ((rc = ws.set("norm3.weight", ln_gamma, sc, 1, 1)) || (rc = ws.set("norm3.bias", ln_beta, sc, 1, 1)) ||
+        (rc = ws.set("ff.net.0.proj.weight", w1, s1, 2, 0)) || (rc = ws.set("ff.net.0.proj.bias", b1, s8, 1, 1)) ||
+        (rc = ws.set("ff.net.2.weight", w2, s2, 2, 0)) || (rc = ws.set("ff.net.2.bias", b2, sc, 1, 1)) ||
+        (rc = ws.set("proj_out.weight", w_po, so, 2, 0)) || (rc = ws.set("proj_out.bias", b_po, sc, 1, 1))) return rc;
+    Xformer t;
+    t.C = C;
+    t.blocks.resize(1);
+    TBlock& b = t.blocks[0];
+    if ((rc = ws.pack_norm("norm3", &b.ln3)) || (rc = ws.pack_geglu("ff.net.0.proj", &b.ff1))) return rc;
+    b.fold = true;
+    if ((rc = ws.fold_ln(&b.ff1, b.ln3, 0, 1.0f)) || (rc = pack_xformer_tail(ws, "proj_out", "ff.net.2", &t, &b))) return rc;
+    SD_HIP_CHECK(hipDeviceSynchronize());
+    const long HW = M / imgs;
+    if (gn_summaries && (!gn_rows || !gn_wants_stats(HW, C, G))) {
+        set_error("sd_op_ffn_geglu_proj_out: summaries need gn_rows and a map the GroupNorm takes summaries for"); return SD_ERR_INVALID;
+    }
+    bool ran_fused = false;
+    GnStatBuf gb;
+    rc = run_op_on_arena(s, 0, nullptr, [&](Ctx& c) {
+        Arena& a = *c.arena;
+        RowStat st;
+        st.p = a.alloc_f(rowstat_floats(M, C));
+        st.parts = 1; st.width = C;
+        View t3v = xformer_tail_t3(a, t, M);
+        View nxt(a.alloc_h((long)M * C), C, C);
+        if (!c.dry) {
+            hipError_t e = hipMemcpy2DAsync(t3v.p, (size_t)t3v.ld * 2, t3, (size_t)C * 2, (size_t)C * 2, (size_t)M,
+                                            hipMemcpyDeviceToDevice, s);
+            if (e != hipSuccess) { set_error(hipGetErrorString(e)); c.err = SD_ERR_HIP; return; }
+            c.err = launch_row_stats(t3v.p, t3v.ld, st.p, M, C, s);
+        }
+        gb = GnStatBuf();
+        gb.buf = gn_summaries;
+        ConvFuse fo;
+        fo.gn_out = gn_summaries ? &gb : nullptr;
+        fo.gn_groups = G;
+        View x(const_cast<half_t*>(static_cast<const half_t*>(x_in)), C, C);
+        ran_fused = run_xformer_tail(c, t, t3v, st, View(), nxt, x, imgs, (int)HW, 1, View(static_cast<half_t*>(y), C, C), fo);
+    });
+    if (fused) *fused = ran_fused ? 1 : 0;
+    if (gn_rows) *gn_rows = gb.st.part ? (int)gb.st.rows : 0;
+    return rc;
+}
+
+}
diff --git a/stablediffusion_amd/csrc/engine.h b/stablediffusion_amd/csrc/engine.h
--- a/stablediffusion_amd/csrc/engine.h
+++ b/stablediffusion_amd/csrc/engine.h
@@ -66,6 +66,7 @@
     float gn_in_eps = 0.f;
     int gn_in_silu = 0;
     float acc_scale = 1.f, bias_scale = 1.f;
+    int tile_variant = -1, tile_splits = 0;
 };
 struct NormW {
     float* gamma = nullptr;
@@ -93,6 +94,7 @@
     int pack_geglu(const std::string& prefix, ConvW* out);
     int pack_norm(const std::string& prefix, NormW* out);
     int fold_ln(ConvW* w, const NormW& ln, int rows_scaled, float row_scale);
+    int fold_linear(const std::string& outer, const std::string& inner, ConvW* out);
     void free_raw();
     void* dmalloc(size_t bytes);
     int64_t packed_bytes() const { return packed_bytes_; }
diff --git a/stablediffusion_amd/csrc/ffn.hip b/stablediffusion_amd/csrc/ffn.hip
--- a/stablediffusion_amd/csrc/ffn.hip
+++ b/stablediffusion_amd/csrc/ffn.hip
@@ -214,9 +214,13 @@
 
 }
 
+bool ffn_fused_width(int C, int hidden) {
+    static const bool off = getenv("SD_NO_FFN_FUSE") != nullptr;
+    return !off && C == FF_C && hidden == 4 * FF_C;
+}
+
 bool ffn_fused_supported(const FfnParams& p) {
-    static const bool off = getenv("SD_NO_FFN_FUSE") != nullptr;
-    return !off && p.C == FF_C && p.hidden == 4 * FF_C && p.M % FF_BM == 0 && p.M / FF_BM >= 64 && p.ln_stat && p.ln_parts >= 1 &&
+    return ffn_fused_width(p.C, p.hidden) && p.M % FF_BM == 0 && p.M / FF_BM >= 64 && p.ln_stat && p.ln_parts >= 1 &&
            p.ln_parts <= kFfMaxLnParts && p.w1_rows >= 2 * p.hidden && p.w2_rows >= FF_C &&
            (long)p.M * p.ldx * 2 < (1L << 31) && p.b1 && p.b2 && p.wsum1;
 }
diff --git a/stablediffusion_amd/csrc/igemm2.hip b/stablediffusion_amd/csrc/igemm2.hip
--- a/stablediffusion_amd/csrc/igemm2.hip
+++ b/stablediffusion_amd/csrc/igemm2.hip
@@ -1100,10 +1100,12 @@
 #include "igemm2_table.inc"
 };
 
-void pick_tile(const IGemmParams& p, int* variant, int* splits) {
-    if (g_force_variant.load() >= 0) {
-        int v = g_force_variant.load();
-        *splits = g_force_splits.load() > 0 ? g_force_splits.load() : 1;
+void pick_tile(const IGemmParams& p, int* variant, int* splits, int hint_variant = -1, int hint_splits = 0) {
+    const bool force = g_force_variant.load() >= 0;
+    if (force || valid_id(hint_variant)) {
+        int v = force ? g_force_variant.load() : hint_variant;
+        const int sp = force ? g_force_splits.load() : hint_splits;
+        *splits = sp > 0 ? sp : 1;
         if (p.geglu && !(valid_id(v) && kVariants[v].geglu)) v = kGegluFallback;
         if (p.geglu || p.act) *splits = 1;
         if (valid_id(v) && is_halo(v) && !halo_supported(p)) v = kHaloFallback;
@@ -1143,6 +1145,16 @@
 
 void igemm2_force(int variant, int splits) { g_force_variant = variant; g_force_splits = splits; }
 
+bool igemm2_tuned_pointwise(int M, int N, int K, int* variant, int* splits) {
+    for (const TunedEntry& e : kTuned)
+        if (e.M == M && e.N == N && e.K == K && e.ks == 1 && e.stride == 1 && e.up == 0 && !e.geglu) {
+            *variant = e.variant;
+            *splits = e.splits;
+            return true;
+        }
+    return false;
+}
+
 bool igemm2_supported(const IGemmParams& p) {
     const long x_bytes = (long)p.N * p.H * p.W * p.ldx * 2;
     const long wrows = ((long)p.Cout + kWeightRowPad - 1) / kWeightRowPad * kWeightRowPad;
@@ -1167,7 +1179,7 @@
     static const bool g3_auto = getenv("SD_IGEMM3") != nullptr;
     const bool forced = g_force_variant.load() >= 0;
     int v0, sp0;
-    pick_tile(p, &v0, &sp0);
+    pick_tile(p, &v0, &sp0, rq.hint_variant, rq.hint_splits);
     if (!valid_id(v0)) { set_error("igemm2: bad variant"); pl.kind = kKindBadVariant; return pl; }
     int v, sp;
     auto route = [&]() {
diff --git a/stablediffusion_amd/csrc/kernels.h b/stablediffusion_amd/csrc/kernels.h
--- a/stablediffusion_amd/csrc/kernels.h
+++ b/stablediffusion_amd/csrc/kernels.h
@@ -45,7 +45,9 @@
     float* gnstat = nullptr;
     int gn_groups = 0;
     bool no_workspace = false;
-};
+    int hint_variant = -1, hint_splits = 0;
+};
+bool igemm2_tuned_pointwise(int M, int N, int K, int* variant, int* splits);
 constexpr int kKindPgemmGeglu = 100;
 constexpr int kKindIgemm1 = -1;
 constexpr int kKindBadVariant = -2;
@@ -88,6 +90,7 @@
     int ln_part_w;
 };
 bool ffn_fused_supported(const FfnParams& p);
+bool ffn_fused_width(int C, int hidden);
 int launch_ffn_fused(const FfnParams& p, hipStream_t s);
 
 long gn_scratch_floats(int N, long HW, int C, int G);
@@ -110,6 +113,8 @@
 int launch_row_stats(const half_t* x, long ldx, float* stat, long rows, int C, hipStream_t s);
 int launch_ln_fold(half_t* w, long K, int rows, const float* gamma, const float* beta, const float* bias_in,
                    float* bias, float* wsum, int rows_scaled, float row_scale, hipStream_t s);
+
+int launch_fold_linear(const half_t* wo, const half_t* wi, half_t* wp, int O, int J, int K, long Kp, hipStream_t s);
 
 int launch_attention(const half_t* q, const half_t* k, const half_t* v, half_t* out,
                      int B, int Tq, int Tk, int heads, int d,
diff --git a/stablediffusion_amd/csrc/misc.hip b/stablediffusion_amd/csrc/misc.hip
--- a/stablediffusion_amd/csrc/misc.hip
+++ b/stablediffusion_amd/csrc/misc.hip
@@ -648,6 +648,22 @@
     }
 }
 
+
+__global__ __launch_bounds__(256) void fold_linear_kernel(const half_t* __restrict__ wo, const half_t* __restrict__ wi,
+                                                          half_t* __restrict__ wp, int J, int K, long Kp) {
+    const long k = (long)blockIdx.x * 256 + threadIdx.x;
+    const long n = blockIdx.y;
+    if (k >= (long)K + J) return;
+    if (k >= K) { wp[n * Kp + k] = wo[n * J + (k - K)]; return; }
+    float s = 0.f, c = 0.f;
+    for (int j = 0; j < J; ++j) {
+        const float y = fmaf((float)wo[n * J + j], (float)wi[(long)j * K + k], -c);
+        const float t = s + y;
+        c = (t - s) - y;
+        s = t;
+    }
+    wp[n * Kp + k] = (half_t)s;
+}
 
 constexpr int CO_TH = 8, CO_TW = 64;
 constexpr int CO_CS = 32;
@@ -1055,6 +1071,12 @@
     SD_HIP_CHECK(hipGetLastError());
     return 0;
 }
+int launch_fold_linear(const half_t* wo, const half_t* wi, half_t* wp, int O, int J, int K, long Kp, hipStream_t s) {
+    if (O <= 0 || J <= 0 || K <= 0 || O > 65535 || Kp < (long)K + J) { set_error("fold_linear: bad shape"); return 1; }
+    hipLaunchKernelGGL(fold_linear_kernel, dim3((unsigned)((K + J + 255) / 256), (unsigned)O), dim3(256), 0, s, wo, wi, wp, J, K, Kp);
+    SD_HIP_CHECK(hipGetLastError());
+    return 0;
+}
 int launch_scale_f16(half_t* x, long n, float scale, hipStream_t s) {
     if (n <= 0) return 0;
     hipLaunchKernelGGL(scale_f16_kernel, grid1d(n), dim3(256), 0, s, x, n, scale);
diff --git a/stablediffusion_amd/csrc/model.h b/stablediffusion_amd/csrc/model.h
--- a/stablediffusion_amd/csrc/model.h
+++ b/stablediffusion_amd/csrc/model.h
@@ -27,6 +27,8 @@
     ConvW pin, pout;
     std::vector<TBlock> blocks;
     int C = 0, heads = 1;
+    bool pout_fold = false;
+    ConvW ff2p;
 };
 struct VaeAttn {
     NormW gn;
@@ -44,6 +46,11 @@
 void run_xformer(Ctx& c, const Xformer& t, View x, int N, int H, int W, View out, int G, View text_kv, int L,
                  const GnStatBuf* x_stats = nullptr, GnStatBuf** out_stats = nullptr, GnStatBuf* out_buf = nullptr,
                  int out_groups = 0, const CfgShare* share = nullptr);
+
+int pack_xformer_tail(WeightStore& ws, const std::string& proj_out, const std::string& ff2, Xformer* x, TBlock* last);
+View xformer_tail_t3(Arena& a, const Xformer& t, long M);
+bool run_xformer_tail(Ctx& c, const Xformer& t, View t3, const RowStat& st_t3, View n, View nxt, View x, int N, int H, int W,
+                      View out, const ConvFuse& fo);
 
 struct UNet;
 
diff --git a/stablediffusion_amd/csrc/runtime.cpp b/stablediffusion_amd/csrc/runtime.cpp
--- a/stablediffusion_amd/csrc/runtime.cpp
+++ b/stablediffusion_amd/csrc/runtime.cpp
@@ -264,6 +264,37 @@
     return 0;
 }
 
+int WeightStore::fold_linear(const std::string& outer, const std::string& inner, ConvW* out) {
+    const RawTensor* wo = raw(outer + ".weight");
+    const RawTensor* wi = raw(inner + ".weight");
+    if (!wo || !wi) { set_error("missing weight: " + (wo ? inner : outer) + ".weight"); return 2; }
+    for (size_t d = 2; d < wo->shape.size(); ++d)
+        if (wo->shape[d] != 1) { set_error("fold_linear: " + outer + " is not pointwise"); return 1; }
+    if (wi->shape.size() != 2 || wo->shape.size() < 2 || wo->shape[1] != wi->shape[0]) {
+        set_error("fold_linear: " + outer + " does not take the output of " + inner); return 1;
+    }
+    const int O = (int)wo->shape[0], J = (int)wo->shape[1], Ki = (int)wi->shape[1];
+    const long K = round_up((long)Ki + J, 64);
+    const long rows = round_up(O, kWeightRowPad);
+    out->cin = Ki + J; out->cout = O; out->ks = 1; out->K = K;
+    out->w = static_cast<half_t*>(dmalloc((size_t)rows * K * sizeof(half_t)));
+    if (!out->w) { set_error("hipMalloc failed (weights)"); return 3; }
+    SD_HIP_CHECK(hipMemsetAsync(out->w, 0, (size_t)rows * K * sizeof(half_t), 0));
+    int rc = launch_fold_linear(wo->dev, wi->dev, out->w, O, J, Ki, K, 0);
+    if (rc) return rc;
+    std::vector<float> wof, bi, bo, b((size_t)O);
+    if ((rc = host_floats(outer + ".weight", &wof))) return rc;
+    if ((rc = host_floats(inner + ".bias", &bi))) return rc;
+    if ((rc = host_floats(outer + ".bias", &bo))) return rc;
+    if ((long)bi.size() != J || (long)bo.size() != O) { set_error("fold_linear: bias length mismatch"); return 1; }
+    for (int n = 0; n < O; ++n) {
+        double acc = bo[(size_t)n];
+        for (int j = 0; j < J; ++j) acc += (double)wof[(size_t)n * J + j] * bi[(size_t)j];
+        b[(size_t)n] = (float)acc;
+    }
+    return upload_bias(this, b, O, &out->bias);
+}
+
 namespace {
 struct ProfRec { std::string name; double flops, bytes; hipEvent_t a, b; };
 std::atomic<bool> g_prof_on{false};
@@ -358,8 +389,9 @@
         if (c.dry) p.gni_part = reinterpret_cast<const float*>(8);
     }
     if (fuse && (fuse->acc_scale != 1.f || fuse->bias_scale != 1.f)) { p.acc_scale = fuse->acc_scale; p.bias_scale = fuse->bias_scale; }
-    const IGemmPlan plan = igemm2_plan(p, IGemmRequest{stat_out ? stat_out->p : nullptr, gn_out ? gn_out->buf : nullptr,
-                                                       fuse ? fuse->gn_groups : 0});
+    IGemmRequest rq{stat_out ? stat_out->p : nullptr, gn_out ? gn_out->buf : nullptr, fuse ? fuse->gn_groups : 0};
+    if (fuse) { rq.hint_variant = fuse->tile_variant; rq.hint_splits = fuse->tile_splits; }
+    const IGemmPlan plan = igemm2_plan(p, rq);
     const bool v2 = plan.kind != kKindIgemm1;
     if ((p.acc_scale != 1.f || p.bias_scale != 1.f) && !plan.scales_ok) { set_error("op_conv: output scaling needs the LDS-DMA kernels (not GEGLU / weight-stationary)"); c.err = 1; return; }
     if (ln_in && !v2) { set_error("op_conv: the LayerNorm fold needs the LDS-DMA kernel"); c.err = 1; return; }
@@ -467,7 +499,7 @@
     p.M = (int)M; p.C = (int)ff1.K; p.hidden = (int)ff2.K;
     if (c.dry) p.ln_stat = reinterpret_cast<const float*>(8);
     if (ff1.ks != 1 || ff2.ks != 1 || ff2.cout != ff1.K || ff1.cout != 2 * ff2.K || x.C != p.C || !ff1.wsum) return false;
-    if (c.dry ? !(p.C == 320 && p.hidden == 1280 && M % 128 == 0 && M / 128 >= 64 && !getenv("SD_NO_FFN_FUSE")) : !ffn_fused_supported(p))
+    if (c.dry ? !(ffn_fused_width(p.C, p.hidden) && M % 128 == 0 && M / 128 >= 64) : !ffn_fused_supported(p))
         return false;
     if (c.dry || c.err) return true;
     prof_open(c.stream, "ffn_fused_kernel", 2.0 * M * ((double)ff1.cout * ff1.K + (double)ff2.cout * ff2.K),
diff --git a/stablediffusion_amd/csrc/unet.cpp b/stablediffusion_amd/csrc/unet.cpp
--- a/stablediffusion_amd/csrc/unet.cpp
+++ b/stablediffusion_amd/csrc/unet.cpp
@@ -157,7 +157,7 @@
     int rc;
     if ((rc = ws.pack_norm(p + ".norm", &x->gn))) return rc;
     if ((rc = ws.pack_conv(p + ".proj_in", &x->pin))) return rc;
-    if ((rc = ws.pack_conv(p + ".proj_out", &x->pout))) return rc;
+    if (depth == 0 && (rc = ws.pack_conv(p + ".proj_out", &x->pout))) return rc;
     x->C = x->pin.cout;
     x->heads = heads;
     x->blocks.resize((size_t)depth);
@@ -178,7 +178,8 @@
         kv_keys.push_back(q + ".attn2.to_v.weight");
         if ((rc = ws.pack_conv(q + ".attn2.to_out.0", &b.out2))) return rc;
         if ((rc = ws.pack_geglu(q + ".ff.net.0.proj", &b.ff1))) return rc;
-        if ((rc = ws.pack_conv(q + ".ff.net.2", &b.ff2))) return rc;
+        const bool last = d + 1 == depth;
+        if (!last && (rc = ws.pack_conv(q + ".ff.net.2", &b.ff2))) return rc;
         static const bool no_fold = getenv("SD_NO_LN_FOLD") != nullptr;
         b.fold = !no_fold;
         if (b.fold) {
@@ -189,8 +190,23 @@
             if ((rc = launch_scale_f16(b.qkv.w, (long)x->C * b.qkv.K, qs, 0))) return rc;
             if ((rc = launch_scale_f16(b.q2.w, (long)x->C * b.q2.K, qs, 0))) return rc;
         }
+        if (last && (rc = pack_xformer_tail(ws, p + ".proj_out", q + ".ff.net.2", x, &b))) return rc;
     }
     return 0;
+}
+
+int pack_xformer_tail(WeightStore& ws, const std::string& proj_out, const std::string& ff2, Xformer* x, TBlock* last) {
+    static const bool off = getenv("SD_NO_POUT_FOLD") != nullptr;
+    const RawTensor* w2 = ws.raw(ff2 + ".weight");
+    const RawTensor* wo = ws.raw(proj_out + ".weight");
+    const int C = x->C;
+    const long hidden = w2 && w2->shape.size() == 2 ? w2->shape[1] : 0;
+    x->pout_fold = !off && last->fold && w2 && wo && hidden > 0 && w2->shape[0] == C && wo->shape[0] == C && wo->shape[1] == C &&
+                   (hidden + C) % 64 == 0 && last->ff1.cout == 2 * hidden && !ffn_fused_width(C, (int)hidden);
+    if (x->pout_fold) return ws.fold_linear(proj_out, ff2, &x->ff2p);
+    int rc;
+    if ((rc = ws.pack_conv(ff2, &last->ff2))) return rc;
+    return ws.pack_conv(proj_out, &x->pout);
 }
 
 int Encoder::pack_encoder(std::vector<std::string>* tw, std::vector<std::string>* tb) {
@@ -390,6 +406,9 @@
     f_ln1.ln_in = &st_cur; f_ln2.ln_in = &st_t2; f_ln3.ln_in = &st_t3;
     f_ln1.ln_eps = f_ln2.ln_eps = f_ln3.ln_eps = 1e-5f;
     op_conv(c, t.pin, hn, Np, H, W, cur, 1, 0, nullptr, 0, nullptr, 0, -1, 0, fold ? &f_cur : nullptr);
+    ConvFuse fo;
+    fo.gn_out = (out_stats && gn_wants_stats(T, C, G)) ? (out_buf ? out_buf : ctx_gnbuf(c)) : nullptr;
+    fo.gn_groups = out_groups > 0 ? out_groups : G;
     for (size_t bi = 0; bi < t.blocks.size(); ++bi) {
         const TBlock& b = t.blocks[bi];
         const bool more = bi + 1 < t.blocks.size();
@@ -435,9 +454,9 @@
                             c.ip_kv.slice(b.ip_kv_off + C, C), att, N, T, L, c.ip_T, t.heads, d, c.ip_scale);
         else
             op_attention(c, q, text_kv.slice(b.kv_off, C), text_kv.slice(b.kv_off + C, C), att, N, T, L, t.heads, d, 0, 1);
-        View t3(a.alloc_h(M * C), C, C);
+        View t3 = more ? View(a.alloc_h(M * C), C, C) : xformer_tail_t3(a, t, M);
         op_conv(c, b.out2, att, N, H, W, t3, 1, 0, nullptr, 0, &t2, 0, -1, 0, fold ? &f_t3 : nullptr);
-        if (!(fold && !more && op_ffn_fused(c, b.ff1, b.ff2, t3, st_t3, 1e-5f, M, nxt))) {
+        if (more) {
             View g(a.alloc_h(M * 4 * C), 4 * C, 4 * C);
             if (fold) {
                 op_conv(c, b.ff1, t3, N, H, W, g, 1, 0, nullptr, 0, nullptr, 1, -1, 0, &f_ln3);
@@ -445,17 +464,59 @@
                 op_layernorm(c, b.ln3, t3, n, M, 1e-5f);
                 op_conv(c, b.ff1, n, N, H, W, g, 1, 0, nullptr, 0, nullptr, 1);
             }
-            op_conv(c, b.ff2, g, N, H, W, nxt, 1, 0, nullptr, 0, &t3, 0, -1, 0, (fold && more) ? &f_cur : nullptr);
+            op_conv(c, b.ff2, g, N, H, W, nxt, 1, 0, nullptr, 0, &t3, 0, -1, 0, fold ? &f_cur : nullptr);
+        } else {
+            run_xformer_tail(c, t, t3, st_t3, n, nxt, x, N, H, W, out, fo);
         }
         a.release(mb);
         View tmp = cur; cur = nxt; nxt = tmp;
     }
-    ConvFuse fo;
-    fo.gn_out = (out_stats && gn_wants_stats(T, C, G)) ? (out_buf ? out_buf : ctx_gnbuf(c)) : nullptr;
-    fo.gn_groups = out_groups > 0 ? out_groups : G;
-    op_conv(c, t.pout, cur, N, H, W, out, 1, 0, nullptr, 0, &x, 0, -1, 0, &fo);
+    if (t.blocks.empty()) op_conv(c, t.pout, cur, N, H, W, out, 1, 0, nullptr, 0, &x, 0, -1, 0, &fo);
     if (out_stats) *out_stats = fo.gn_out;
     a.release(mk);
+}
+
+View xformer_tail_t3(Arena& a, const Xformer& t, long M) {
+    if (!t.pout_fold) return View(a.alloc_h(M * t.C), t.C, t.C);
+    const long ld = t.ff2p.cin;
+    return View(a.alloc_h(M * ld) + (ld - t.C), ld, t.C);
+}
+
+bool run_xformer_tail(Ctx& c, const Xformer& t, View t3, const RowStat& st_t3, View n, View nxt, View x, int N, int H, int W,
+                      View out, const ConvFuse& fo) {
+    Arena& a = *c.arena;
+    const TBlock& b = t.blocks.back();
+    const int C = t.C;
+    const long M = (long)N * H * W;
+    const int hidden = b.ff1.cout / 2;
+    ConvFuse f_ln3;
+    f_ln3.ln_in = &st_t3; f_ln3.ln_eps = 1e-5f;
+    if (t.pout_fold) {
+        if (t3.ld != hidden + C || t.ff2p.cin != hidden + C) { set_error("run_xformer_tail: t3 is not xformer_tail_t3's view"); c.err = 1; return false; }
+        View gt(t3.p - hidden, t3.ld, hidden + C);
+        op_conv(c, b.ff1, t3, N, H, W, gt.slice(0, hidden), 1, 0, nullptr, 0, nullptr, 1, -1, 0, &f_ln3);
+        ConvFuse f = fo;
+        int v, sp;
+        if (igemm2_tuned_pointwise((int)M, C, hidden, &v, &sp)) { f.tile_variant = v; f.tile_splits = sp; }
+        op_conv(c, t.ff2p, gt, N, H, W, out, 1, 0, nullptr, 0, &x, 0, -1, 0, &f);
+        return false;
+    }
+    const bool fold = b.fold;
+    const bool fused = fold && op_ffn_fused(c, b.ff1, b.ff2, t3, st_t3, 1e-5f, M, nxt);
+    if (!fused) {
+        const size_t mk = a.mark();
+        View g(a.alloc_h(M * hidden), hidden, hidden);
+        if (fold) {
+            op_conv(c, b.ff1, t3, N, H, W, g, 1, 0, nullptr, 0, nullptr, 1, -1, 0, &f_ln3);
+        } else {
+            op_layernorm(c, b.ln3, t3, n, M, 1e-5f);
+            op_conv(c, b.ff1, n, N, H, W, g, 1, 0, nullptr, 0, nullptr, 1);
+        }
+        op_conv(c, b.ff2, g, N, H, W, nxt, 1, 0, nullptr, 0, &t3, 0, -1, 0, nullptr);
+        a.release(mk);
+    }
+    op_conv(c, t.pout, nxt, N, H, W, out, 1, 0, nullptr, 0, &x, 0, -1, 0, &fo);
+    return fused;
 }
 
 int Encoder::run_temb(Ctx& c, const float* timesteps, const half_t* add_text, const float* add_time_ids, int B,
diff --git a/stablediffusion_amd/shapes.py b/stablediffusion_amd/shapes.py
--- a/stablediffusion_amd/shapes.py
+++ b/stablediffusion_amd/shapes.py
@@ -62,6 +62,8 @@
         out.append(ConvShape(N, h, w, C, 8 * C, 1, geglu=1, tag="ff.geglu"))
         out.append(ConvShape(N, h, w, 4 * C, C, 1, tag="ff.out"))
     out.append(ConvShape(N, h, w, C, C, 1, tag="proj_out"))
+    if C != 320:
+        out.append(ConvShape(N, h, w, 5 * C, C, 1, tag="ff.out+proj_out"))
 
 
 def unet_convs(cfg: UNetConfig, B: int, H: int, W: int, L: int = 77) -> List[ConvShape]:
```

New measurement: 7.963 latents/s, median of 6. 1.01x the previous value.
